# tum-vision/mem

Measured on AMD Instinct MI355X. Metric: pretrain samples/sec (ViT-B, 224^2 event voxels), higher is better.
Workload: dtype bf16; 1 GPU; MEM pretrain ViT-Base/16, 224^2 2-bin event voxels, bf16, batch 256 per GPU (BASELINE configs[1]); step = rasterize 256x30k events + event_norm + masks + ViT fwd/CE/bwd + clip + AdamW; global_batch=256, parallelism=dp1, stochastic_depth=work skipping, optimizer=AdamW as one launch in front of the next forward, last_block_mlp_rows=rows that reach the head

## Files before the change

### include/memhip.h

```cpp
#ifndef MEMHIP_H
#define MEMHIP_H

#include <stddef.h>
#include <stdint.h>

#ifdef __cplusplus
extern "C" {
#endif

#define MEMHIP_ABI_VERSION 10

#define MEMHIP_OK 0
#define MEMHIP_EINVAL (-1)
#define MEMHIP_EWORKSPACE (-2)
#define MEMHIP_ELAUNCH (-3)
#define MEMHIP_EUNSUPPORTED (-4)

typedef void* memhip_stream_t;

int memhip_abi_version(void);
const char* memhip_last_error(void);
const char* memhip_arch(void);
const char* memhip_build_flags(void);
int memhip_set_option(const char* name, int value);
int memhip_get_option(const char* name, int* value);
int memhip_stream_reserve_cus(memhip_stream_t stream, int cus);


typedef struct memhip_event_aug {
  double scale_x, scale_y;
  int32_t time_flip;
  int32_t flip_x;
  int64_t flip_w;
  int32_t shift_x, shift_y;
  int32_t do_filter;
  int32_t filt_w, filt_h;
  int32_t infer;
} memhip_event_aug_t;
#define MEMHIP_AUG_INFER_FLIP_W 1
#define MEMHIP_AUG_INFER_FILT_W 2
#define MEMHIP_AUG_INFER_FILT_H 4

enum { MEMHIP_RASTER_AUTO = 0, MEMHIP_RASTER_SINGLE = 1, MEMHIP_RASTER_BINNED = 2,
       MEMHIP_RASTER_LDS = 3, MEMHIP_RASTER_GLOBAL = 4, MEMHIP_RASTER_GLOBAL_VAR = 5 };
typedef struct memhip_raster_args {
  const double* ev;
  const int64_t* offsets;
  const memhip_event_aug_t* aug;
  const int32_t* dims;
  int32_t B, H, W, time_surface;
  int32_t form;
  int32_t reserved0;
  int64_t n_events;
  uint8_t* out;
  int32_t* status;
  void* workspace;
  size_t workspace_bytes;
} memhip_raster_args_t;
int memhip_rasterize(const memhip_raster_args_t* args, memhip_stream_t stream);

enum { MEMHIP_RASTER_K_COUNT,
       MEMHIP_RASTER_K_FINALIZE,
       MEMHIP_RASTER_K_LDS,
       MEMHIP_RASTER_K_BIN_KEYS,
       MEMHIP_RASTER_K_BIN_ACCUM };
typedef struct memhip_raster_launch {
  int32_t kernel;
  int32_t grid_x, grid_y;
  int32_t block;
  int32_t lds;
} memhip_raster_launch_t;
typedef struct memhip_raster_plan {
  int32_t family;
  int32_t rows_per_band, bands;
  int32_t band_px, nb;
  int32_t bx;
  uint64_t ws_bytes;
  uint64_t off_bins, off_tstat;
  uint64_t off_keys, off_hdr, off_bad_slots;
  uint64_t clear_ws_bytes, clear_status_bytes, clear_out_bytes;
  int32_t count;
  memhip_raster_launch_t l[2];
} memhip_raster_plan_t;
int memhip_rasterize_plan(const memhip_raster_args_t* args, int device_cus, memhip_raster_plan_t* out);

int memhip_aug_resolve(const double* extent, memhip_event_aug_t* aug, int B, int stage, int fixed_h, int fixed_w,
                       int hmax, int wmax, int32_t* dims, int32_t* status, memhip_stream_t stream);

int memhip_events_extent(const double* ev, const int64_t* offsets, const memhip_event_aug_t* aug,
                         int B, double* extent, memhip_stream_t stream);

#define MEMHIP_DT_U8 0
#define MEMHIP_DT_I8 1
#define MEMHIP_DT_U16 2
#define MEMHIP_DT_I16 3
#define MEMHIP_DT_U32 4
#define MEMHIP_DT_I32 5
#define MEMHIP_DT_U64 6
#define MEMHIP_DT_I64 7
#define MEMHIP_DT_F32 8
#define MEMHIP_DT_F64 9
#define MEMHIP_DT_BOOL 10
int memhip_decode_ncaltech101(const uint8_t* raw, int64_t n_bytes, double* ev, memhip_stream_t stream);
int memhip_events_from_columns(const void* x, int x_dtype, const void* y, int y_dtype, const void* t, int t_dtype,
                               const void* p, int p_dtype, int64_t n, double* ev, memhip_stream_t stream);
size_t memhip_events_dsec_workspace(int64_t n);
int memhip_events_dsec(const void* in, int dtype, int64_t n, double y_limit, double* out, int64_t* n_out,
                       void* workspace, size_t workspace_bytes, memhip_stream_t stream);

int memhip_resample_to_f32(const uint8_t* in, const int32_t* dims, int64_t slot_bytes, int fixed_h, int fixed_w, int mode,
                           const int32_t* offs, int B, int OH, int OW, float* out, memhip_stream_t stream);
int memhip_to_uint8(const float* x, int64_t n, uint8_t* y, memhip_stream_t stream);
int memhip_rand_augment_u8(const uint8_t* in, uint8_t* out, const void* ops, int B, int H, int W, memhip_stream_t stream);
int memhip_color_jitter(const void* in, int in_is_u8, int B, int H, int W, const void* params, float* out, int out_chans,
                        memhip_stream_t stream);

#define MEMHIP_EV_RM_TS 1
#define MEMHIP_EV_HOTPIX 2
#define MEMHIP_EV_LOG 4
#define MEMHIP_EV_GAMMA 8
#define MEMHIP_EV_NORMALIZE 16
int memhip_event_norm(const void* in, int in_is_u8, int B, int H, int W, int flags,
                      float num_stds, float gamma, float* out, int out_chans,
                      memhip_stream_t stream);
int memhip_event_norm_topk(const void* in, int in_is_u8, int B, int H, int W, int flags,
                           int num_hot_pixels, float gamma, float* out, int out_chans,
                           uint64_t* hot_keys, memhip_stream_t stream);

int memhip_mt_seed(uint32_t* mt_state, const uint32_t* key, int key_len);
double memhip_mt_random(uint32_t* mt_state);
int memhip_mask_blockwise(uint32_t* mt_state, int H, int W, int num_masking_patches,
                          int min_num_patches, int max_num_patches, double log_aspect_lo,
                          double log_aspect_hi, int n_masks, uint8_t* out);
int memhip_mask_random_location(uint32_t* mt_state, int H, int W, int num_masking_patches,
                                int n_masks, uint8_t* out);

#define MEMHIP_EPI_BIAS_BF16 0
#define MEMHIP_EPI_BIAS_GELU 1
#define MEMHIP_EPI_RESIDUAL 2
#define MEMHIP_EPI_DGELU 3
#define MEMHIP_EPI_F32 4
#define MEMHIP_EPI_PATCH_EMBED 5
#define MEMHIP_EPI_BIAS_GELU_DG 6
#define MEMHIP_EPI_MUL_AUX 7
#define MEMHIP_EPI_RESIDUAL_DROP 8

typedef struct memhip_dropout {
  uint32_t key0, key1;
  uint32_t site;
  uint32_t thr;
  float scale;
  int32_t row0;
} memhip_dropout_t;
int memhip_dropout_mask(const memhip_dropout_t* d, int row0, int rows, int cols, uint8_t* out, memhip_stream_t stream);
int memhip_dropout_rows_f32(const memhip_dropout_t* d, float* x, int64_t ldx, int rows, int D, memhip_stream_t stream);

typedef struct memhip_gemm_args {
  const void* A; const void* B;
  int64_t lda, ldb;
  int32_t M, N, K, epilogue;
  void* out0; int64_t ldo0;
  void* out1; int64_t ldo1;
  const float* bias;
  const float* vec1;
  float* resid; int64_t ldr;
  const void* aux; int64_t ldaux;
  const float* rowmask;
  float keep_prob;
  float colscale; int32_t colscale_n;
  int32_t rows_per_sample;
  int32_t accumulate;
  float* colsum;
  const int32_t* sample_map;
  int32_t colsum_copies;
  int32_t reserved0;
  const memhip_dropout_t* dropout;
} memhip_gemm_args_t;
int memhip_gemm_bf16_nt(const memhip_gemm_args_t* args, memhip_stream_t stream);

#define MEMHIP_NT_128 0
#define MEMHIP_NT_G256 1
#define MEMHIP_NT_P8_256 2
#define MEMHIP_NT_P8_128 3
#define MEMHIP_NT_P8_PAIR 4
typedef struct memhip_nt_launch {
  int32_t kind;
  int32_t row0, rows;
  int32_t tail_rows;
  int32_t guard;
  int32_t copy;
  int32_t grid, tail_grid;
} memhip_nt_launch_t;
typedef struct memhip_nt_plan { int32_t count; memhip_nt_launch_t l[2]; } memhip_nt_plan_t;
int memhip_gemm_bf16_nt_plan(const memhip_gemm_args_t* args, int stream_cus, int device_cus, memhip_nt_plan_t* out);

size_t memhip_gemm_bf16_tn_workspace(int R, int N, int K);
int memhip_gemm_bf16_tn(const void* A, int64_t lda, const void* B, int64_t ldb, int R, int N, int K,
                        float* out, int64_t ldo, int accumulate, void* workspace, size_t workspace_bytes,
                        memhip_stream_t stream);
typedef struct memhip_tn_problem {
  const void* A; int64_t lda;
  const void* B; int64_t ldb;
  float* out; int64_t ldo;
  int32_t R, N, K;
  int32_t reserved0;
} memhip_tn_problem_t;
size_t memhip_gemm_bf16_tn_group_workspace(const memhip_tn_problem_t* problems, int count);
int memhip_gemm_bf16_tn_group(const memhip_tn_problem_t* problems, int count, int accumulate, void* workspace,
                              size_t workspace_bytes, memhip_stream_t stream);

#define MEMHIP_TN_128 0
#define MEMHIP_TN_P8_ATOMIC 1
#define MEMHIP_TN_P8_WS 2
#define MEMHIP_TN_P8_GROUP 3
typedef struct memhip_tn_part {
  int32_t problem;
  int32_t tiles, splits, rows_per_split;
  int32_t wg_begin, quad_begin;
  int64_t ws_offset;
} memhip_tn_part_t;
typedef struct memhip_tn_launch {
  int32_t kind;
  int32_t count;
  int32_t grid, reduce_grid;
  int32_t memset_first;
  int32_t use_atomics;
  int64_t ws_bytes;
  memhip_tn_part_t p[4];
} memhip_tn_launch_t;
typedef struct memhip_tn_plan { int32_t count; int32_t reserved0; memhip_tn_launch_t l[4]; } memhip_tn_plan_t;
int memhip_gemm_bf16_tn_plan(const memhip_tn_problem_t* problems, int count, int accumulate, const void* workspace,
                             size_t workspace_bytes, int stream_cus, memhip_tn_plan_t* out_plan);
size_t memhip_gemm_bf16_tn_plan_workspace(const memhip_tn_problem_t* problems, int count, int device_cus);
int memhip_colsum_bf16(const void* in, int64_t ld, int R, int C, float* out, memhip_stream_t stream);
int memhip_colsum_fold(float* ws, int copies, int N, float* out, memhip_stream_t stream);

int memhip_residual_rows(const float* x, int64_t ldx, const int32_t* rows, const void* y, int64_t ldy, const float* gamma,
                         const float* rowkeep, float keep_prob, int R, int D, float* out, int64_t ldo,
                         memhip_stream_t stream);
int memhip_scatter_rows_f32(const float* src, int64_t lds, const int32_t* rows, int R, int D, float* dst, int64_t ldd,
                            memhip_stream_t stream);

int memhip_layernorm_fwd(const float* x, int64_t ldx, const int32_t* row_idx, int R, int D,
                         const float* gamma, const float* beta, float eps, void* y_bf16, int64_t ldy,
                         float* mean, float* rstd, memhip_stream_t stream);
int memhip_layernorm_bwd(const void* dy_bf16, int64_t lddy, const float* x, int64_t ldx,
                         const int32_t* row_idx, int R, int D, const float* gamma, const float* mean,
                         const float* rstd, float* dres, int64_t lddres, int accumulate, float* dgamma,
                         float* dbeta, memhip_stream_t stream);

int memhip_layerscale_grad(const void* W_bf16, int64_t ldw, const float* dW, int64_t lddw, const float* bias,
                           const float* dbias, const float* gamma, int N, int K, float* dgamma,
                           memhip_stream_t stream);

typedef struct memhip_branch {
  const void* y; int64_t ldy;
  const float* gamma;
  const float* rowmask;
  float keep_prob;
  int32_t rows_per_sample;
  void* dy; int64_t lddy;
  float* dgamma; float* dbias;
  const int32_t* out_map;
  const memhip_dropout_t* dropout;
} memhip_branch_t;
typedef struct memhip_branch_bwd_args {
  const float* dx; int64_t lddx;
  int32_t M, D;
  memhip_branch_t branch;
} memhip_branch_bwd_args_t;
int memhip_branch_bwd(const memhip_branch_bwd_args_t* args, memhip_stream_t stream);
typedef struct memhip_ln_bwd_branch_args {
  const void* dy; int64_t lddy;
  const float* x; int64_t ldx;
  int32_t R, D;
  const float* gamma; const float* mean; const float* rstd;
  float* dres; int64_t lddres;
  float* dgamma; float* dbeta;
  const int32_t* in_map;
  memhip_branch_t branch;
} memhip_ln_bwd_branch_args_t;
int memhip_layernorm_bwd_branch(const memhip_ln_bwd_branch_args_t* args, memhip_stream_t stream);

int memhip_embed_bwd(const float* dx, int64_t lddx, const uint8_t* mask, int B, int L, int D,
                     void* dy_bf16, int64_t lddy, float* dcls, float* dmask_token, memhip_stream_t stream);

int memhip_cross_entropy(void* logits_bf16, int64_t ld, const int64_t* labels, int M, int V,
                         float grad_scale, float* row_loss, int32_t* row_correct, int write_grad,
                         float* out2, memhip_stream_t stream);

int memhip_attn_tokens_padded(int T);
int memhip_relpos_gather(const float* table, const int32_t* index , int T, int TP, int heads,
                         float* bias_pad, float* biasT_pad ,
                         memhip_stream_t stream);
int memhip_attn_fwd(const void* qkv, int64_t ldqkv, int B, int T, int D, int heads, const float* table,
                    int window_h, int window_w, void* out, int64_t ldo, float* lse, memhip_stream_t stream);
int memhip_attn_delta(const void* dout, const void* out, int64_t ldo, int64_t rows, int heads, float* delta,
                      memhip_stream_t stream);
typedef struct memhip_attn_bwd_args {
  const void* qkv; int64_t ldqkv;
  const void* dout; int64_t ldo;
  const void* out; int64_t ldout;
  const float* lse;
  float* delta;
  const float* table;
  int32_t window_h, window_w, B, T, D, heads;
  float scale;
  int32_t reserved0;
  void* dqkv; int64_t lddqkv;
  float* dtable; float* dq_bias; float* dv_bias;
  void* ws; int64_t ws_bytes;
} memhip_attn_bwd_args_t;
int memhip_attn_bwd(const memhip_attn_bwd_args_t* args, memhip_stream_t stream);
int64_t memhip_attn_bwd_workspace(int B, int T, int heads, int window_h, int window_w);

#define MEMHIP_ATTN_16 1
#define MEMHIP_ATTN_SMALL 2
#define MEMHIP_ATTN_WIN 3
#define MEMHIP_ATTN_WIN_DS 4
#define MEMHIP_ATTN_STREAM 5
enum { MEMHIP_ATTN_K_STATS_ZERO, MEMHIP_ATTN_K_DELTA, MEMHIP_ATTN_K_FWD, MEMHIP_ATTN_K_BWD_KV, MEMHIP_ATTN_K_BWD_Q,
       MEMHIP_ATTN_K_FWD16, MEMHIP_ATTN_K_BWD16,
       MEMHIP_ATTN_K_WIN_STATS, MEMHIP_ATTN_K_FWD_WIN, MEMHIP_ATTN_K_BWD_KV_WIN, MEMHIP_ATTN_K_BWD_Q_WIN,
       MEMHIP_ATTN_K_BWD_KVS_WIN, MEMHIP_ATTN_K_BWD_QS_WIN,
       MEMHIP_ATTN_K_FWD_STREAM, MEMHIP_ATTN_K_BWD_KV_STREAM, MEMHIP_ATTN_K_BWD_Q_STREAM };
typedef struct memhip_attn_launch {
  int32_t kernel;
  int32_t grid_x, grid_y, grid_z;
  int32_t block;
  int32_t lds;
} memhip_attn_launch_t;
typedef struct memhip_attn_plan {
  int32_t family;
  int32_t n;
  int32_t ww;
  int32_t vb, dt, fd;
  int32_t spb;
  int32_t nwg;
  int32_t groups;
  int32_t nbz, nbq, nbs;
  int32_t qgroups, qs;
  int32_t stream_spb;
  int32_t lds_over;
  int32_t count;
  memhip_attn_launch_t l[5];
} memhip_attn_plan_t;
int memhip_attn_plan_fwd(int B, int T, int D, int heads, int window_h, int window_w, int stream_cus, memhip_attn_plan_t* out);
int memhip_attn_plan_bwd(int B, int T, int D, int heads, int window_h, int window_w, int has_dtable, int has_dv_bias,
                         int has_out, const void* ws, int64_t ws_bytes, int stream_cus, memhip_attn_plan_t* out);

int memhip_f32_gemm_nt(const memhip_gemm_args_t* args, memhip_stream_t stream);
int memhip_f32_transpose(const float* in, int64_t ldin, int R, int C, float* out, int64_t ldout, memhip_stream_t stream);
int memhip_f32_layernorm_fwd(const float* x, int64_t ldx, const int32_t* row_idx, int R, int D, const float* gamma,
                             const float* beta, float eps, float* y, int64_t ldy, float* mean, float* rstd,
                             memhip_stream_t stream);
int memhip_f32_layernorm_bwd(const float* dy, int64_t lddy, const float* x, int64_t ldx, const int32_t* row_idx, int R, int D,
                             const float* gamma, const float* mean, const float* rstd, float* dres, int64_t lddres,
                             int accumulate, float* dgamma, float* dbeta, memhip_stream_t stream);
int memhip_f32_branch_bwd(const float* dx, int64_t lddx, const float* y, int64_t ldy, const float* gamma, const float* rowmask,
                          float keep_prob, int rows_per_sample, int M, int D, float* dy, int64_t lddy, float* dgamma,
                          float* dbias, memhip_stream_t stream);
int memhip_f32_embed_bwd(const float* dx, int64_t lddx, const uint8_t* mask, int B, int L, int D, float* dy, int64_t lddy,
                         float* dcls, float* dmask_token, memhip_stream_t stream);
int memhip_f32_cross_entropy(float* logits, int64_t ld, const int64_t* labels, int M, int V, float grad_scale,
                             float* row_loss, int32_t* row_correct, int write_grad, float* out2, memhip_stream_t stream);
int memhip_f32_colsum(const float* in, int64_t ld, int R, int C, float* out, memhip_stream_t stream);
int memhip_f32_im2col(const float* x, int B, int C, int H, int W, int ph, int pw, float* out, memhip_stream_t stream);
int memhip_f32_attn_fwd(const float* qkv, int64_t ldqkv, int B, int T, int D, int heads, const float* table,
                        const int32_t* index, float* out, int64_t ldo, float* lse, memhip_stream_t stream);
int memhip_f32_attn_bwd(const float* qkv, int64_t ldqkv, const float* dout, int64_t ldo, int B, int T, int D, int heads,
                        float scale, const float* table, const int32_t* index, float* dqkv, int64_t lddqkv, float* dtable,
                        memhip_stream_t stream);

int memhip_mae_enc_assemble(const float* xe, const float* pos, const float* cls, const int64_t* ids_keep, int B, int L, int K,
                            int D, float* out, memhip_stream_t stream);
int memhip_mae_enc_assemble_bwd(const float* dx, const int64_t* ids_keep, int B, int L, int K, int D, float* dxe, float* dcls,
                                memhip_stream_t stream);
int memhip_mae_dec_assemble(const float* y, const float* mask_token, const float* dpos, const int64_t* ids_restore, int B, int L,
                            int K, int D, float* out, memhip_stream_t stream);
int memhip_mae_dec_assemble_bwd(const float* dxd, const int64_t* ids_restore, int B, int L, int K, int D, float* dy,
                                float* dmask_token, memhip_stream_t stream);
int memhip_mae_loss(const float* pred, const float* img, const float* mask, int B, int C, int H, int W, int patch,
                    int only_masked, float* row_loss, float* dpred, float* scratch2, memhip_stream_t stream);

enum { MEMHIP_CONV_BF16, MEMHIP_CONV_F32, MEMHIP_CONV_F16X2 };
typedef struct memhip_conv_args {
  int32_t mode;
  int32_t reserved0;
  const void* in;
  int64_t in_plane;
  const void* weight;
  int64_t w_plane;
  const float* bias;
  const void* add;
  int64_t add_plane;
  void* out;
  int64_t out_plane;
  int32_t B, H, W, Cin, Cout, ksize, stride, pad;
  int32_t relu;
  int32_t out_padded;
  int32_t out_f32;
  int32_t reserved1;
  const int32_t* n_active;
} memhip_conv_args_t;
int memhip_conv2d_nhwc(const memhip_conv_args_t* args, memhip_stream_t stream);
int memhip_nchw_to_padded_nhwc4(const float* x, int B, int C, int H, int W, const float* mean, const float* stdv, void* out,
                                int64_t out_plane, int mode, memhip_stream_t stream);
int memhip_argmax_rows(const void* logits, int mode, int64_t ld, int M, int N, int64_t* ids, float* top2_gap, float* row_rms,
                       const int32_t* n_samples, int rows_per_sample, memhip_stream_t stream);

int memhip_tok_flag_samples(const float* top2_gap, const float* row_rms, int B, int tokens_per_sample, float kappa,
                            int32_t* list, int32_t* count, int64_t* stats, memhip_stream_t stream);
int memhip_tok_gather_images_f32(const float* x, int C, int H, int W, const float* mean, const float* stdv,
                                 const int32_t* list, const int32_t* count, int offset, int R, float* out, int32_t* n_round,
                                 memhip_stream_t stream);
int memhip_tok_scatter_ids(const int64_t* ids_in, const int32_t* list, const int32_t* n_round, int offset, int R,
                           int tokens_per_sample, int64_t* ids_out, memhip_stream_t stream);

enum { MEMHIP_CONV_K_BF16,
       MEMHIP_CONV_K_F32,
       MEMHIP_CONV_K_F32_M32,
       MEMHIP_CONV_K_F16X2_W4,
       MEMHIP_CONV_K_F16X2_W8,
       MEMHIP_CONV_K_F16X2_WIDE,
       MEMHIP_CONV_K_F16X2_FIRST,
       MEMHIP_CONV_K_BF16_T };
typedef struct memhip_conv_launch {
  int32_t kernel;
  int32_t grid;
  int32_t block;
  int32_t lds;
  int32_t dyn_lo, dyn_hi;
} memhip_conv_launch_t;
typedef struct memhip_conv_plan {
  int32_t Hp, Wp, Ho, Wo;
  int32_t K, off;
  int64_t M;
  int32_t count;
  memhip_conv_launch_t l[2];
} memhip_conv_plan_t;
int memhip_conv_plan(const memhip_conv_args_t* args, int device_cus, memhip_conv_plan_t* out);

int memhip_convt2d_nhwc(const void* in, const void* weight, const float* bias, void* out, int B, int H, int W, int Cin, int Cout,
                        int relu, memhip_stream_t stream);
int memhip_convt_plan(int B, int H, int W, int Cin, int Cout, int device_cus, memhip_conv_plan_t* out);
int memhip_kl_uniform_rows(const void* logits, int mode, int64_t ld, int M, int N, float* row_kl, memhip_stream_t stream);

struct memhip_conv_wgrad_args {
  const void* small;
  const void* big;
  float* grad;
  void* workspace;
  size_t workspace_bytes;
  int32_t B, Hs, Ws;
  int32_t C, N;
  int32_t ksize, stride, pad;
  int32_t small_padded;
  int32_t accumulate;
};
typedef struct memhip_conv_wgrad_args memhip_conv_wgrad_args_t;
struct memhip_conv_wgrad_plan {
  int64_t M;
  int64_t ws_bytes;
  int32_t K;
  int32_t Hbp, Wbp;
  int32_t tiles_n, tiles_k;
  int32_t splits, rows_per_split;
  int32_t grid, block, lds_bytes;
  int32_t fold_grid;
  int32_t reserved;
};
typedef struct memhip_conv_wgrad_plan memhip_conv_wgrad_plan_t;
int memhip_conv_wgrad_nhwc(const memhip_conv_wgrad_args_t* args, memhip_stream_t stream);
int memhip_conv_wgrad_plan(const memhip_conv_wgrad_args_t* args, int device_cus, memhip_conv_wgrad_plan_t* out);
size_t memhip_conv_wgrad_workspace(const memhip_conv_wgrad_args_t* args, int device_cus);
int memhip_relu_bwd_colsum(void* g, const void* y, int padded, int B, int H, int W, int C, float* colsum, int accumulate,
                           void* workspace, size_t workspace_bytes, memhip_stream_t stream);
size_t memhip_relu_bwd_colsum_workspace(int B, int H, int W, int C);

int memhip_cast_f32_bf16(const float* in, void* out_bf16, int64_t n, memhip_stream_t stream);
int memhip_zero(void* p, int64_t bytes, memhip_stream_t stream);
int memhip_zero_ranges(void* base, const int64_t* ranges, int n, int64_t total_bytes, memhip_stream_t stream);
int memhip_copy_samples_f32(const float* src, float* dst, const int32_t* ids, int n, int64_t n_per_sample,
                            memhip_stream_t stream);
int memhip_transpose_cast_f32_bf16(const float* in, int64_t ldin, int R, int Cc, void* out_bf16,
                                   int64_t ldout, memhip_stream_t stream);
int memhip_transpose_cast_batched(const void* desc, const int32_t* tile_prefix, int n, int total_tiles,
                                  memhip_stream_t stream);

int memhip_transpose_bf16(const void* in, int64_t ldin, int R, int Cc, void* out, int64_t ldout, int R_pad,
                          float* colsum0, int c0_begin, int c0_end, float* colsum1, int c1_begin,
                          int c1_end, memhip_stream_t stream);
int memhip_im2col_bf16(const float* x, int B, int C, int H, int W, int ph, int pw, void* out_bf16,
                       memhip_stream_t stream);
int memhip_fill_cls(float* x, int64_t ldx, int B, int T, int D, const float* cls, memhip_stream_t stream);
int memhip_gemv_bf16_acc(const void* W, int64_t ldw, int N, int K, const float* x, float* y, float* x_acc,
                         float* zero, memhip_stream_t stream);

size_t memhip_grad_norm_workspace(void);
int memhip_grad_norm(const float* g, int64_t n, float* norm_out, void* workspace, size_t workspace_bytes,
                     memhip_stream_t stream);
int memhip_adamw(float* p, const float* g, float* m, float* v, int64_t n, const uint8_t* wd_flag_per_chunk,
                 double lr, double beta1, double beta2, double eps, double weight_decay, int step,
                 const float* gnorm, double max_norm, memhip_stream_t stream);

int memhip_adamw_groups(float* p, const float* g, float* m, float* v, int64_t n, const uint8_t* group_of_chunk,
                        const float* group_table, int n_groups, double beta1, double beta2, double eps, int step,
                        const float* gnorm, double max_norm, memhip_stream_t stream);

int memhip_mixup(float* x, int B, int C, int H, int W, const float* lam, const int32_t* box, const float* lam_host,
                 const int32_t* box_host, memhip_stream_t stream);
int memhip_mix_targets(const int64_t* labels, const float* lam, int B, int V, double smoothing, float* t, int64_t ldt,
                       memhip_stream_t stream);
int memhip_ce_soft(const void* logits, int logits_f32, int64_t ld, const float* target, int64_t ldt, const int64_t* labels,
                   float smoothing, int M, int V, float grad_scale, void* dlogits, int64_t lddl, float* row_loss,
                   int32_t* row_correct, int write_grad, float* out2, memhip_stream_t stream);
int memhip_ema_update(float* ema, const float* p, int64_t n, double decay, memhip_stream_t stream);

int memhip_pool_tokens(const float* x, int64_t ldx, int B, int T, int D, float* out, memhip_stream_t stream);
int memhip_pool_tokens_bwd(const float* dout, int B, int T, int D, float* dx, memhip_stream_t stream);

int memhip_tokens_to_maps(const float* x, int64_t ldx, int b0, int b1, int T, int D, float* out, memhip_stream_t stream);
int memhip_maps_to_tokens_add(const float* dmap, int b0, int b1, int T, int D, float* dx, int64_t lddx, memhip_stream_t stream);

int memhip_neck_maps_to_rows(const float* map, int B, int D, int Hp, int Wp, int level, void* rows_bf16, memhip_stream_t stream);
int memhip_neck_rows_to_maps(const void* rows_bf16, int B, int D, int Hp, int Wp, int level, float* map, memhip_stream_t stream);
#define MEMHIP_NECK_GROUPS 128
size_t memhip_neck_sums_workspace(int D);
int memhip_neck_colstats(const void* y_bf16, int64_t R, int D, const float* shift, float* workspace, size_t workspace_bytes,
                         float* out, memhip_stream_t stream);
int memhip_neck_bn_gelu_fwd(const void* y_bf16, int64_t R, int D, const float* mean, const float* rstd, const float* gamma,
                            const float* beta, void* z_bf16, memhip_stream_t stream);
int memhip_neck_bn_gelu_bwd_sums(const void* da_bf16, const void* y_bf16, int64_t R, int D, const float* mean, const float* rstd,
                                 const float* gamma, const float* beta, float* workspace, size_t workspace_bytes, float* out,
                                 memhip_stream_t stream);
int memhip_neck_bn_gelu_bwd_apply(const void* da_bf16, const void* y_bf16, int64_t R, int D, const float* mean, const float* rstd,
                                  const float* gamma, const float* beta, const float* sums, float inv_n, void* dy_bf16,
                                  memhip_stream_t stream);

int memhip_seg_axis_table(int in, int out, int align_corners, int32_t* i0, float* w1, int32_t* lo, int32_t* hi);

struct memhip_seg_args {
  const float* logits;
  int64_t sb, sc, sy, sx;
  const uint8_t* labels;
  int32_t B, C, h, w, H, W;
  int32_t ignore_index;
  int32_t align_corners;
  int32_t avg_non_ignore;
  float loss_weight;
  const int32_t* y_i0; const float* y_w1; const int32_t* y_lo; const int32_t* y_hi;
  const int32_t* x_i0; const float* x_w1; const int32_t* x_lo; const int32_t* x_hi;
  float* dz;
  int64_t db, dc, dy, dx;
  float* loss;
  int64_t* stats;
  void* workspace;
  size_t workspace_bytes;
  int64_t* confusion;
};
typedef struct memhip_seg_args memhip_seg_args_t;

int memhip_seg_ce(const memhip_seg_args_t* args, memhip_stream_t stream);
int memhip_seg_confusion(const memhip_seg_args_t* args, memhip_stream_t stream);

struct memhip_seg_plan {
  int32_t tile_h, tile_w;
  int32_t tiles_y, tiles_x;
  int32_t grid, block;
  int32_t chunk;
  int32_t max_fh, max_fw;
  int32_t tables_in_lds;
  int32_t lds_bytes;
  int32_t slot_bytes;
  int32_t conf_grid, conf_block, conf_lds_bytes;
  int32_t reserved;
  uint64_t ws_bytes;
};
typedef struct memhip_seg_plan memhip_seg_plan_t;
int memhip_seg_plan(const memhip_seg_args_t* args, memhip_seg_plan_t* out);

int memhip_map_to_nhwc_pad(const float* map, int B, int D, int h, int w, void* out_bf16, memhip_stream_t stream);
int memhip_nhwc_pad_to_map(const void* in_bf16, int B, int D, int h, int w, float* map, memhip_stream_t stream);
#define MEMHIP_BN_GROUPS 128
size_t memhip_bn_stats_workspace(int C);
// ... 102 lines not shown
```

### mem_amd/csrc/rowops.hip

```cpp
#include "common.h"
#include "dropout.hpp"

#include <type_traits>

namespace {

using namespace memhip;

typedef __attribute__((ext_vector_type(4))) __bf16 bf16x4;
typedef __attribute__((ext_vector_type(8))) __bf16 bf16x8;

__device__ __forceinline__ float wsum(float v) {
  for (int o = 32; o > 0; o >>= 1) v += __shfl_xor(v, o);
  return v;
}
__device__ __forceinline__ float wmax(float v) {
  for (int o = 32; o > 0; o >>= 1) v = fmaxf(v, __shfl_xor(v, o));
  return v;
}

__device__ __forceinline__ float div_newton(float a, float b, float r) {
  const float q0 = a * r;
  return fmaf(fmaf(-q0, b, a), r, q0);
}

constexpr int kMaxChunks = 8;

template <bool FULL>
__device__ __forceinline__ bool chunk_ok(int i, int nch) {
  if constexpr (FULL) return true;
  else return i < nch;
}

__device__ __forceinline__ int wave_id() { return __builtin_amdgcn_readfirstlane((int)(threadIdx.x >> 6)); }

struct RowWalk {
  int r, smp, off, stride, q, rem, rps;
  __device__ __forceinline__ RowWalk(int r0, int stride_, int rps_) : r(r0), stride(stride_), rps(rps_) {
    smp = r0 / rps; off = r0 - smp * rps;
    q = stride / rps; rem = stride - q * rps;
  }
  __device__ __forceinline__ void next() {
    r += stride; smp += q; off += rem;
    if (off >= rps) { off -= rps; ++smp; }
  }
};

__device__ __forceinline__ void stage_columns(float4* dst, const float* a, const float* b, int nch) {
  for (int i = threadIdx.x; i < nch; i += 256) {
    dst[i] = reinterpret_cast<const float4*>(a)[i];
    dst[nch + i] = b ? reinterpret_cast<const float4*>(b)[i] : float4{1.f, 1.f, 1.f, 1.f};
  }
  __syncthreads();
}

__device__ __forceinline__ int opaque(int v) {
  asm volatile("" : "+v"(v));
  return v;
}

__device__ __forceinline__ float mul_rn(float a, float b) {
#pragma clang fp contract(off)
  return a * b;
}
__device__ __forceinline__ float sub_rn(float a, float b) {
#pragma clang fp contract(off)
  return a - b;
}
__device__ __forceinline__ float ln_dx(float gg, float xh, float m1, float m2) { return __fmaf_rn(-xh, m2, sub_rn(gg, m1)); }
__device__ __forceinline__ float sq2(float a, float b) { return __fmaf_rn(a, a, mul_rn(b, b)); }

template <int NCH, bool FULL>
__global__ __launch_bounds__(256) void ln_fwd_kernel(const float* __restrict__ x, long long ldx,
                                                     const int* __restrict__ row_idx, int R, int D,
                                                     const float* __restrict__ gamma,
                                                     const float* __restrict__ beta, float eps,
                                                     __bf16* __restrict__ y, long long ldy,
                                                     float* __restrict__ mean, float* __restrict__ rstd) {
  extern __shared__ float red[];
  const int lane = threadIdx.x & 63;
  const int r0 = blockIdx.x * 4 + wave_id();
  const bool act = r0 < R;
  const int r = act ? r0 : R - 1;
  const long long src = row_idx ? row_idx[r] : r;
  const float4* xr = reinterpret_cast<const float4*>(x + src * ldx);
  const int nch = D >> 2;
  float4 v[NCH];
#pragma unroll
  for (int c = 0; c < NCH; ++c) {
    const int i = lane + c * 64;
    if (chunk_ok<FULL>(i, nch)) v[c] = xr[i];
  }
  constexpr int NST = (64 * NCH + 255) / 256;
  float4 sg[NST], sb[NST];
#pragma unroll
  for (int k = 0; k < NST; ++k) {
    const int i = min((int)threadIdx.x + k * 256, nch - 1);
    sg[k] = reinterpret_cast<const float4*>(gamma)[i];
    sb[k] = reinterpret_cast<const float4*>(beta)[i];
  }
  __builtin_amdgcn_sched_barrier(0);
  float s = 0.f;
#pragma unroll
  for (int c = 0; c < NCH; ++c)
    if (chunk_ok<FULL>(lane + c * 64, nch)) s += (v[c].x + v[c].y) + (v[c].z + v[c].w);
  const float mu = wsum(s) / (float)D;
  float4* lgb = reinterpret_cast<float4*>(red);
#pragma unroll
  for (int k = 0; k < NST; ++k) {
    const int i = min((int)threadIdx.x + k * 256, nch - 1);
    lgb[i] = sg[k];
    lgb[nch + i] = sb[k];
  }
  float q = 0.f;
#pragma unroll
  for (int c = 0; c < NCH; ++c) {
    if (chunk_ok<FULL>(lane + c * 64, nch)) {
      const float a = v[c].x - mu, b = v[c].y - mu, cc = v[c].z - mu, d = v[c].w - mu;
      q += sq2(a, b) + sq2(cc, d);
    }
  }
  const float var = wsum(q) / (float)D;
  const float rs = 1.0f / sqrtf(var + eps);
  __syncthreads();
  if (!act) return;
  if (lane == 0) { mean[r] = mu; rstd[r] = rs; }
  bf16x4* yr = reinterpret_cast<bf16x4*>(y + (long long)r * ldy);
#pragma unroll
  for (int c = 0; c < NCH; ++c) {
    const int i = lane + c * 64;
    if (chunk_ok<FULL>(i, nch)) {
      const float4 g = lgb[i], b = lgb[nch + i];
      bf16x4 o;
      o[0] = (__bf16)__fmaf_rn(mul_rn(v[c].x - mu, rs), g.x, b.x);
      o[1] = (__bf16)__fmaf_rn(mul_rn(v[c].y - mu, rs), g.y, b.y);
      o[2] = (__bf16)__fmaf_rn(mul_rn(v[c].z - mu, rs), g.z, b.z);
      o[3] = (__bf16)__fmaf_rn(mul_rn(v[c].w - mu, rs), g.w, b.w);
      yr[i] = o;
    }
  }
}

__device__ __forceinline__ void vm_drain() { __builtin_amdgcn_s_waitcnt(0x0F70); }

template <int NCH, bool FULL, bool ACC>
__global__ __launch_bounds__(256) void ln_bwd_kernel(const __bf16* __restrict__ dy, long long lddy,
                                                     const float* __restrict__ x, long long ldx,
                                                     const int* __restrict__ row_idx, int R, int D,
                                                     const float* __restrict__ gamma,
                                                     const float* __restrict__ mean,
                                                     const float* __restrict__ rstd,
                                                     float* __restrict__ dres, long long lddres,
                                                     float* __restrict__ dgamma, float* __restrict__ dbeta) {
  extern __shared__ float red[];
  const int lane = threadIdx.x & 63, wave = wave_id();
  const int nch = D >> 2;
  float4 ag[NCH], ab[NCH];
#pragma unroll
  for (int c = 0; c < NCH; ++c) {
    ag[c] = float4{0, 0, 0, 0};
    ab[c] = float4{0, 0, 0, 0};
  }
  const int rstride = gridDim.x * 4;
  float4 xn[NCH], prev[NCH];
  bf16x4 dn[NCH];
  auto issue = [&](int r, long long src, int lane) {
    const float4* xr = reinterpret_cast<const float4*>(x + src * ldx);
    const bf16x4* dyr = reinterpret_cast<const bf16x4*>(dy + (long long)r * lddy);
#pragma unroll
    for (int c = 0; c < NCH; ++c) {
      const int i = lane + c * 64;
      if (chunk_ok<FULL>(i, nch)) {
        xn[c] = xr[i];
        dn[c] = dyr[i];
      }
    }
  };
  auto issue_prev = [&](long long src, int lane) {
    const float4* o = reinterpret_cast<const float4*>(dres + src * lddres);
#pragma unroll
    for (int c = 0; c < NCH; ++c) {
      const int i = lane + c * 64;
      if (chunk_ok<FULL>(i, nch)) prev[c] = o[i];
    }
  };
  int r = blockIdx.x * 4 + wave;
  long long src = 0;
  float mu = 0.f, rs = 0.f;
  if (r < R) {
    src = row_idx ? row_idx[r] : r;
    issue(r, src, lane);
    if constexpr (ACC) issue_prev(src, lane);
    mu = mean[r]; rs = rstd[r];
  }
  float4* lg = reinterpret_cast<float4*>(red);
  for (int i = threadIdx.x; i < nch; i += 256) lg[i] = reinterpret_cast<const float4*>(gamma)[i];
  __syncthreads();
  int r1 = r + rstride;
  long long src1 = 0;
  if (r1 < R) src1 = row_idx ? row_idx[r1] : r1;
  int r2 = r1 + rstride;
  vm_drain();
  while (r < R) {
    float4 xh[NCH], gg[NCH];
    float s1 = 0.f, s2 = 0.f;
    const int ol = opaque(lane);
    const float4* lgl = lg + ol;
#pragma unroll
    for (int c = 0; c < NCH; ++c) {
      const int i = lane + c * 64;
      if (chunk_ok<FULL>(i, nch)) {
        const float4 xv = xn[c];
        const bf16x4 d4 = dn[c];
        const float4 g = lgl[c * 64];
        const float d0 = (float)d4[0], d1 = (float)d4[1], d2 = (float)d4[2], d3 = (float)d4[3];
        xh[c] = float4{mul_rn(xv.x - mu, rs), mul_rn(xv.y - mu, rs), mul_rn(xv.z - mu, rs), mul_rn(xv.w - mu, rs)};
        gg[c] = float4{mul_rn(d0, g.x), mul_rn(d1, g.y), mul_rn(d2, g.z), mul_rn(d3, g.w)};
        s1 += (gg[c].x + gg[c].y) + (gg[c].z + gg[c].w);
        s2 += (mul_rn(gg[c].x, xh[c].x) + mul_rn(gg[c].y, xh[c].y)) + (mul_rn(gg[c].z, xh[c].z) + mul_rn(gg[c].w, xh[c].w));
        ag[c].x += d0 * xh[c].x; ag[c].y += d1 * xh[c].y; ag[c].z += d2 * xh[c].z; ag[c].w += d3 * xh[c].w;
        ab[c].x += d0; ab[c].y += d1; ab[c].z += d2; ab[c].w += d3;
      }
    }
    float mu1 = 0.f, rs1 = 0.f;
    long long src2 = 0;
    const bool next = r1 < R;
    const int rl = next ? r1 : r;
    const long long srcl = next ? src1 : src;
    issue(rl, srcl, ol);
    if (next) {
      mu1 = mean[r1]; rs1 = rstd[r1];
      if (r2 < R) src2 = row_idx ? row_idx[r2] : r2;
    }
    const float m1 = wsum(s1) / (float)D, m2 = wsum(s2) / (float)D;
    float4* o = reinterpret_cast<float4*>(dres + src * lddres);
#pragma unroll
    for (int c = 0; c < NCH; ++c) {
      const int i = ol + c * 64;
      if (chunk_ok<FULL>(i, nch)) {
        const float4 t{ln_dx(gg[c].x, xh[c].x, m1, m2), ln_dx(gg[c].y, xh[c].y, m1, m2),
                       ln_dx(gg[c].z, xh[c].z, m1, m2), ln_dx(gg[c].w, xh[c].w, m1, m2)};
        float4 d;
        if constexpr (ACC) {
          const float4 p = prev[c];
          d = float4{__fmaf_rn(rs, t.x, p.x), __fmaf_rn(rs, t.y, p.y), __fmaf_rn(rs, t.z, p.z), __fmaf_rn(rs, t.w, p.w)};
        } else {
          d = float4{mul_rn(rs, t.x), mul_rn(rs, t.y), mul_rn(rs, t.z), mul_rn(rs, t.w)};
        }
        o[i] = d;
      }
    }
    if constexpr (ACC) {
      __builtin_amdgcn_sched_barrier(0);
      issue_prev(srcl, ol);
    }
    r = r1; src = src1; mu = mu1; rs = rs1;
    r1 = r2; src1 = src2;
    r2 += rstride;
  }
  __syncthreads();
  float4* rg = reinterpret_cast<float4*>(red + (size_t)wave * 2 * D);
  float4* rb = reinterpret_cast<float4*>(red + (size_t)wave * 2 * D + D);
#pragma unroll
  for (int c = 0; c < NCH; ++c) {
    const int i = lane + c * 64;
    if (chunk_ok<FULL>(i, nch)) { rg[i] = ag[c]; rb[i] = ab[c]; }
  }
  __syncthreads();
  for (int n = threadIdx.x; n < D; n += 256) {
    float a = 0.f, b = 0.f;
#pragma unroll
    for (int w = 0; w < 4; ++w) { a += red[(size_t)w * 2 * D + n]; b += red[(size_t)w * 2 * D + D + n]; }
    atomicAdd(dgamma + n, a);
    atomicAdd(dbeta + n, b);
  }
}

constexpr int kBrMaxChunks = 8;

template <int NCH, bool FULL, bool HAS_Y, class... Drop>
__global__ __launch_bounds__(256) void branch_bwd_kernel(const float* __restrict__ dx, long long lddx,
                                                         const __bf16* __restrict__ y, long long ldy,
                                                         const float* __restrict__ gamma,
                                                         const float* __restrict__ rowmask, float keep,
                                                         int rps, int M, int D, __bf16* __restrict__ dyo,
                                                         long long lddy, float* __restrict__ dgamma,
                                                         float* __restrict__ dbias, const int* __restrict__ out_map,
                                                         Drop... drop) {
  extern __shared__ float red[];
  const int lane = threadIdx.x & 63, wave = wave_id();
  const int nch = D >> 2;
  float4 ag[NCH], ab[NCH];
  const float rk = __frcp_rn(keep);
#pragma unroll
  for (int c = 0; c < NCH; ++c) {
    ag[c] = float4{0, 0, 0, 0};
    ab[c] = float4{0, 0, 0, 0};
  }
  float4 dn[NCH];
  bf16x4 yn[HAS_Y ? NCH : 1];
  auto issue = [&](int m, int lane) {
    const float4* dr = reinterpret_cast<const float4*>(dx + (long long)m * lddx);
#pragma unroll
    for (int c = 0; c < NCH; ++c) {
      const int i = lane + c * 64;
      if (chunk_ok<FULL>(i, nch)) {
        dn[c] = dr[i];
        if constexpr (HAS_Y) yn[c] = reinterpret_cast<const bf16x4*>(y + (long long)m * ldy)[i];
      }
    }
  };
  RowWalk w(blockIdx.x * 4 + wave, gridDim.x * 4, rps);
  auto find = [&](int& m, int& mo, int& smp) {
    for (;;) {
      m = w.r; smp = w.smp; mo = -1;
      if (m >= M) return;
      mo = w.r;
      if (out_map) { const int co = out_map[w.smp]; mo = co < 0 ? -1 : co * w.rps + w.off; }
      w.next();
      if (mo >= 0) return;
    }
  };
  int m, mo, smp;
  float k = 1.f;
  find(m, mo, smp);
  if (m < M) {
    issue(m, lane);
    if (rowmask) k = rowmask[smp];
  }
  float4* lg = reinterpret_cast<float4*>(red);
  for (int i = threadIdx.x; i < nch; i += 256)
    lg[i] = gamma ? reinterpret_cast<const float4*>(gamma)[i] : float4{1.f, 1.f, 1.f, 1.f};
  __syncthreads();
  int m1, mo1, smp1;
  find(m1, mo1, smp1);
  vm_drain();
  while (m < M) {
    const int ol = opaque(lane);
    float4 dv[NCH];
    bf16x4 yv[HAS_Y ? NCH : 1];
#pragma unroll
    for (int c = 0; c < NCH; ++c) {
      if (chunk_ok<FULL>(lane + c * 64, nch)) {
        dv[c] = dn[c];
        if constexpr (HAS_Y) yv[c] = yn[c];
      }
    }
    float k1 = 1.f;
    const bool next = m1 < M;
    issue(next ? m1 : m, ol);
    if (next && rowmask) k1 = rowmask[smp1];
    int m2, mo2, smp2;
    find(m2, mo2, smp2);
    bf16x4* orow = reinterpret_cast<bf16x4*>(dyo + (long long)mo * lddy);
    const float4* lgl = lg + ol;
#pragma unroll
    for (int c = 0; c < NCH; ++c) {
      const int i = ol + c * 64;
      if (chunk_ok<FULL>(i, nch)) {
        float4 d = dv[c];
        if (rowmask || out_map) {
          d.x = div_newton(d.x * k, keep, rk); d.y = div_newton(d.y * k, keep, rk);
          d.z = div_newton(d.z * k, keep, rk); d.w = div_newton(d.w * k, keep, rk);
        }
        if constexpr (sizeof...(Drop) > 0) {
          const DropParams dp = (drop, ...);
          const unsigned kb = dropout_keep8(dp, (unsigned)(dp.row0 + m), (unsigned)(i >> 1)) >> ((i & 1) * 4);
          d.x = __fmul_rn(d.x, dropout_mul(dp, kb, 0)); d.y = __fmul_rn(d.y, dropout_mul(dp, kb, 1));
          d.z = __fmul_rn(d.z, dropout_mul(dp, kb, 2)); d.w = __fmul_rn(d.w, dropout_mul(dp, kb, 3));
        }
        if constexpr (HAS_Y) {
          const bf16x4 yy = yv[c];
          ag[c].x += d.x * (float)yy[0]; ag[c].y += d.y * (float)yy[1];
          ag[c].z += d.z * (float)yy[2]; ag[c].w += d.w * (float)yy[3];
        }
        const float4 g = lgl[c * 64];
        bf16x4 o;
        o[0] = (__bf16)(d.x * g.x); o[1] = (__bf16)(d.y * g.y);
        o[2] = (__bf16)(d.z * g.z); o[3] = (__bf16)(d.w * g.w);
        orow[i] = o;
        ab[c].x += (float)o[0]; ab[c].y += (float)o[1]; ab[c].z += (float)o[2]; ab[c].w += (float)o[3];
      }
    }
    m = m1; mo = mo1; k = k1;
    m1 = m2; mo1 = mo2; smp1 = smp2;
  }
  __syncthreads();
  float4* rg = reinterpret_cast<float4*>(red + (size_t)wave * 2 * D);
  float4* rb = reinterpret_cast<float4*>(red + (size_t)wave * 2 * D + D);
#pragma unroll
  for (int c = 0; c < NCH; ++c) {
    const int i = lane + c * 64;
    if (chunk_ok<FULL>(i, nch)) { rg[i] = ag[c]; rb[i] = ab[c]; }
  }
  __syncthreads();
  for (int n = threadIdx.x; n < D; n += 256) {
    float a = 0.f, b = 0.f;
#pragma unroll
    for (int w2 = 0; w2 < 4; ++w2) { a += red[(size_t)w2 * 2 * D + n]; b += red[(size_t)w2 * 2 * D + D + n]; }
    if (dgamma) atomicAdd(dgamma + n, a);
    if (dbias) atomicAdd(dbias + n, b);
  }
}

template <int NCH, bool FULL, bool HAS_Y, class... Drop>
__global__ __launch_bounds__(256) void ln_bwd_branch_kernel(const __bf16* __restrict__ dy, long long lddy,
                                                            const float* __restrict__ x, long long ldx, int R, int D,
                                                            const float* __restrict__ gamma,
                                                            const float* __restrict__ mean, const float* __restrict__ rstd,
                                                            float* __restrict__ dres, long long lddres,
                                                            float* __restrict__ dgamma, float* __restrict__ dbeta,
                                                            const __bf16* __restrict__ yb, long long ldyb,
                                                            const float* __restrict__ gb, const float* __restrict__ rowmask,
                                                            float keep, int rps, __bf16* __restrict__ dyo, long long lddyo,
                                                            float* __restrict__ dgb, float* __restrict__ dbiasb,
                                                            const int* __restrict__ in_map, const int* __restrict__ out_map,
                                                            Drop... drop) {
  extern __shared__ float red[];
  const int lane = threadIdx.x & 63, wave = wave_id();
  const int nch = D >> 2;
  float4 ag[NCH], ab[NCH], bg[HAS_Y ? NCH : 1], bb[NCH];
  const float rk = __frcp_rn(keep);
#pragma unroll
  for (int c = 0; c < NCH; ++c) {
    ag[c] = ab[c] = bb[c] = float4{0, 0, 0, 0};
    if (HAS_Y) bg[c] = float4{0, 0, 0, 0};
  }
  float4 xn[NCH], prev[NCH];
  bf16x4 dn[NCH], yn[HAS_Y ? NCH : 1];
  auto issue_x = [&](int r, int rin, int lane) {
    const float4* xr = reinterpret_cast<const float4*>(x + (long long)r * ldx);
    const bf16x4* dyr = reinterpret_cast<const bf16x4*>(dy + (long long)rin * lddy);
#pragma unroll
    for (int c = 0; c < NCH; ++c) {
      const int i = lane + c * 64;
      if (chunk_ok<FULL>(i, nch)) {
        xn[c] = xr[i];
        dn[c] = dyr[i];
      }
    }
  };
  auto issue_y = [&](int r, int lane) {
    if constexpr (HAS_Y) {
#pragma unroll
      for (int c = 0; c < NCH; ++c) {
        const int i = lane + c * 64;
        if (chunk_ok<FULL>(i, nch)) yn[c] = reinterpret_cast<const bf16x4*>(yb + (long long)r * ldyb)[i];
      }
    }
  };
  auto issue_prev = [&](int r, int lane) {
    const float4* o = reinterpret_cast<const float4*>(dres + (long long)r * lddres);
#pragma unroll
    for (int c = 0; c < NCH; ++c) {
      const int i = lane + c * 64;
      if (chunk_ok<FULL>(i, nch)) prev[c] = o[i];
    }
  };
  const int row0 = blockIdx.x * 4 + wave, rstride = gridDim.x * 4;
  auto resolve = [&](const RowWalk& t, int& rin, int& rout) {
    rin = rout = t.r;
    if (in_map) { const int ci = in_map[t.smp]; rin = ci < 0 ? -1 : ci * t.rps + t.off; }
    if (out_map) { const int co = out_map[t.smp]; rout = co < 0 ? -1 : co * t.rps + t.off; }
  };
  int r, rin, rout;
  float mu = 0.f, rs = 0.f, km = 1.f;
  float4 xh[NCH], gg[NCH];
  bf16x4 yv[HAS_Y ? NCH : 1];
  float s1, s2;
  float4 *lg = reinterpret_cast<float4*>(red), *lgb = lg + nch;
  auto reduce_row = [&](bool has_in, int ol) {
    s1 = s2 = 0.f;
    const float4* lgl = lg + ol;
    if (has_in) {
#pragma unroll
      for (int c = 0; c < NCH; ++c) {
        if (chunk_ok<FULL>(lane + c * 64, nch)) {
          if constexpr (HAS_Y) yv[c] = yn[c];
          const float4 xv = xn[c];
          const bf16x4 d4 = dn[c];
          const float d0 = (float)d4[0], d1 = (float)d4[1], d2 = (float)d4[2], d3 = (float)d4[3];
          xh[c] = float4{mul_rn(xv.x - mu, rs), mul_rn(xv.y - mu, rs), mul_rn(xv.z - mu, rs), mul_rn(xv.w - mu, rs)};
          const float4 gmc = lgl[c * 64];
          gg[c] = float4{mul_rn(d0, gmc.x), mul_rn(d1, gmc.y), mul_rn(d2, gmc.z), mul_rn(d3, gmc.w)};
          s1 += (gg[c].x + gg[c].y) + (gg[c].z + gg[c].w);
          s2 += (mul_rn(gg[c].x, xh[c].x) + mul_rn(gg[c].y, xh[c].y)) + (mul_rn(gg[c].z, xh[c].z) + mul_rn(gg[c].w, xh[c].w));
          ag[c].x += d0 * xh[c].x; ag[c].y += d1 * xh[c].y; ag[c].z += d2 * xh[c].z; ag[c].w += d3 * xh[c].w;
          ab[c].x += d0; ab[c].y += d1; ab[c].z += d2; ab[c].w += d3;
        }
      }
    } else {
#pragma unroll
      for (int c = 0; c < NCH; ++c) {
        if (chunk_ok<FULL>(lane + c * 64, nch)) {
          if constexpr (HAS_Y) yv[c] = yn[c];
          xh[c] = gg[c] = float4{0.f, 0.f, 0.f, 0.f};
        }
      }
    }
  };
  auto store_row = [&](bool has_in, bool has_out, int ol) {
    const float m1 = wsum(s1) / (float)D, m2 = wsum(s2) / (float)D;
    float4* o = reinterpret_cast<float4*>(dres + (long long)r * lddres);
    bf16x4* orow = reinterpret_cast<bf16x4*>(dyo + (long long)(has_out ? rout : 0) * lddyo);
    const float4* lgbl = lgb + ol;
#pragma unroll
    for (int c = 0; c < NCH; ++c) {
      const int i = ol + c * 64;
      if (chunk_ok<FULL>(i, nch)) {
        float4 d{__fmaf_rn(rs, ln_dx(gg[c].x, xh[c].x, m1, m2), prev[c].x), __fmaf_rn(rs, ln_dx(gg[c].y, xh[c].y, m1, m2), prev[c].y),
                 __fmaf_rn(rs, ln_dx(gg[c].z, xh[c].z, m1, m2), prev[c].z), __fmaf_rn(rs, ln_dx(gg[c].w, xh[c].w, m1, m2), prev[c].w)};
        if (has_in) o[i] = d;
        if (!has_out) continue;
        if (rowmask || out_map) {
          d.x = div_newton(d.x * km, keep, rk); d.y = div_newton(d.y * km, keep, rk);
          d.z = div_newton(d.z * km, keep, rk); d.w = div_newton(d.w * km, keep, rk);
        }
        if constexpr (sizeof...(Drop) > 0) {
          const DropParams dp = (drop, ...);
          const unsigned kb = dropout_keep8(dp, (unsigned)(dp.row0 + r), (unsigned)(i >> 1)) >> ((i & 1) * 4);
          d.x = __fmul_rn(d.x, dropout_mul(dp, kb, 0)); d.y = __fmul_rn(d.y, dropout_mul(dp, kb, 1));
          d.z = __fmul_rn(d.z, dropout_mul(dp, kb, 2)); d.w = __fmul_rn(d.w, dropout_mul(dp, kb, 3));
        }
        if constexpr (HAS_Y) {
          bg[c].x += d.x * (float)yv[c][0]; bg[c].y += d.y * (float)yv[c][1];
          bg[c].z += d.z * (float)yv[c][2]; bg[c].w += d.w * (float)yv[c][3];
        }
        const float4 gbc = lgbl[c * 64];
        bf16x4 q;
        q[0] = (__bf16)(d.x * gbc.x); q[1] = (__bf16)(d.y * gbc.y);
        q[2] = (__bf16)(d.z * gbc.z); q[3] = (__bf16)(d.w * gbc.w);
        orow[i] = q;
        bb[c].x += (float)q[0]; bb[c].y += (float)q[1]; bb[c].z += (float)q[2]; bb[c].w += (float)q[3];
      }
    }
  };
  RowWalk w(row0, rstride, rps);
  auto find = [&](int& fr, int& frin, int& frout, int& fsmp) {
    for (;;) {
      fr = w.r; fsmp = w.smp; frin = frout = -1;
      if (fr >= R) return;
      resolve(w, frin, frout);
      w.next();
      if ((frin | frout) >= 0) return;
    }
  };
  int smp;
  find(r, rin, rout, smp);
  if (r < R) {
    issue_x(r, rin, lane); issue_y(r, lane); issue_prev(r, lane);
    mu = mean[rin]; rs = rstd[rin];
    if (rowmask) km = rowmask[smp];
  }
  stage_columns(lg, gamma, gb, nch);
  int r1, rin1, rout1, smp1;
  find(r1, rin1, rout1, smp1);
  vm_drain();
  while (r < R) {
    const int ol = opaque(lane);
    reduce_row(true, ol);
    float mu1 = 0.f, rs1 = 0.f, km1 = 1.f;
    const bool next = r1 < R;
    const int rl = next ? r1 : r, rinl = next ? rin1 : rin;
    issue_x(rl, rinl, ol); issue_y(rl, ol);
    if (next) {
      mu1 = mean[rin1]; rs1 = rstd[rin1];
      if (rowmask) km1 = rowmask[smp1];
    }
    int r2, rin2, rout2, smp2;
    find(r2, rin2, rout2, smp2);
    store_row(true, true, ol);
    __builtin_amdgcn_sched_barrier(0);
    issue_prev(rl, ol);
    r = r1; rin = rin1; rout = rout1; mu = mu1; rs = rs1; km = km1;
    r1 = r2; rin1 = rin2; rout1 = rout2; smp1 = smp2;
  }
  if (in_map || out_map) {
    for (RowWalk v(row0, rstride, rps); v.r < R; v.next()) {
      resolve(v, rin, rout);
      if ((rin >= 0) == (rout >= 0)) continue;
      r = v.r;
      const int ol = opaque(lane);
      issue_prev(r, ol); issue_y(r, ol);
      mu = rs = 0.f;
      if (rin >= 0) {
        issue_x(r, rin, ol);
        mu = mean[rin]; rs = rstd[rin];
      }
      km = rowmask ? rowmask[v.smp] : 1.f;
      reduce_row(rin >= 0, ol);
      store_row(rin >= 0, rout >= 0, ol);
    }
  }
  __syncthreads();
  float4* r0 = reinterpret_cast<float4*>(red + (size_t)wave * 4 * D);
#pragma unroll
  for (int c = 0; c < NCH; ++c) {
    const int i = lane + c * 64;
    if (chunk_ok<FULL>(i, nch)) { r0[i] = ag[c]; r0[nch + i] = ab[c]; r0[2 * nch + i] = HAS_Y ? bg[HAS_Y ? c : 0] : float4{0, 0, 0, 0}; r0[3 * nch + i] = bb[c]; }
  }
  __syncthreads();
  for (int n = threadIdx.x; n < D; n += 256) {
    float a = 0.f, b = 0.f, c2 = 0.f, d2 = 0.f;
#pragma unroll
    for (int w2 = 0; w2 < 4; ++w2) {
      const float* rw = red + (size_t)w2 * 4 * D;
      a += rw[n]; b += rw[D + n]; c2 += rw[2 * D + n]; d2 += rw[3 * D + n];
    }
    atomicAdd(dgamma + n, a);
    atomicAdd(dbeta + n, b);
    if (dgb) atomicAdd(dgb + n, c2);
    if (dbiasb) atomicAdd(dbiasb + n, d2);
  }
}


__global__ __launch_bounds__(256) void layerscale_grad_kernel(const __bf16* __restrict__ W, long long ldw,
                                                              const float* __restrict__ dW, long long lddw,
                                                              const float* __restrict__ b, const float* __restrict__ db,
                                                              const float* __restrict__ gamma, int N, int K,
                                                              float* __restrict__ dgamma) {
  __shared__ float red[4][4];
  const int lane = threadIdx.x & 63, wave = threadIdx.x >> 6;
  const int n0 = blockIdx.x * 4;
  float s[4] = {0.f, 0.f, 0.f, 0.f};
  for (int k0 = 0; k0 < K; k0 += 4096) {
#pragma unroll
    for (int c = 0; c < 4; ++c) {
      const int n = n0 + c < N ? n0 + c : N - 1;
      const __bf16* wr = W + (long long)n * ldw;
      const float* gr = dW + (long long)n * lddw;
#pragma unroll
      for (int u = 0; u < 4; ++u) {
        const int k = k0 + u * 1024 + (int)threadIdx.x * 4;
        if (k < K) {
          const bf16x4 w = *reinterpret_cast<const bf16x4*>(wr + k);
          const float4 g = *reinterpret_cast<const float4*>(gr + k);
          s[c] += (float)w[0] * g.x + (float)w[1] * g.y + (float)w[2] * g.z + (float)w[3] * g.w;
        }
      }
    }
  }
#pragma unroll
  for (int c = 0; c < 4; ++c) {
    const float t = wsum(s[c]);
    if (lane == 0) red[wave][c] = t;
  }
  __syncthreads();
  if (threadIdx.x < 4 && n0 + (int)threadIdx.x < N) {
    const int n = n0 + threadIdx.x;
    float t = (red[0][threadIdx.x] + red[1][threadIdx.x]) + (red[2][threadIdx.x] + red[3][threadIdx.x]);
    if (b && db) t += b[n] * db[n];
    const float g = gamma[n];
    dgamma[n] = g != 0.f ? t / g : 0.f;
  }
}

__global__ __launch_bounds__(256) void embed_bwd_kernel(const float* __restrict__ dx, long long lddx,
                                                        const unsigned char* __restrict__ mask, int B,
                                                        int L, int D, __bf16* __restrict__ dy,
                                                        long long lddy, float* __restrict__ dcls,
                                                        float* __restrict__ dmask) {
  constexpr int U = 7;
  for (int c = threadIdx.x * 4; c < D; c += 256 * 4) {
    float4 cls{0, 0, 0, 0}, am{0, 0, 0, 0};
    for (int b = blockIdx.x; b < B; b += gridDim.x) {
      const float* row0 = dx + (long long)b * (L + 1) * lddx + c;
      const float4 dc = *reinterpret_cast<const float4*>(row0);
      cls.x += dc.x; cls.y += dc.y; cls.z += dc.z; cls.w += dc.w;
      const unsigned char* mk = mask + (long long)b * L;
      __bf16* out = dy + (long long)b * L * lddy + c;
      int p = 0;
      for (; p + U <= L; p += U) {
        float4 d[U];
#pragma unroll
        for (int u = 0; u < U; ++u) d[u] = *reinterpret_cast<const float4*>(row0 + (long long)(1 + p + u) * lddx);
#pragma unroll
        for (int u = 0; u < U; ++u) {
          const float w = (float)mk[p + u], q = 1.0f - w;
          am.x += d[u].x * w; am.y += d[u].y * w; am.z += d[u].z * w; am.w += d[u].w * w;
          bf16x4 o;
          o[0] = (__bf16)(d[u].x * q); o[1] = (__bf16)(d[u].y * q); o[2] = (__bf16)(d[u].z * q); o[3] = (__bf16)(d[u].w * q);
          *reinterpret_cast<bf16x4*>(out + (long long)(p + u) * lddy) = o;
        }
      }
      for (; p < L; ++p) {
        const float4 d = *reinterpret_cast<const float4*>(row0 + (long long)(1 + p) * lddx);
        const float w = (float)mk[p], q = 1.0f - w;
        am.x += d.x * w; am.y += d.y * w; am.z += d.z * w; am.w += d.w * w;
        bf16x4 o;
        o[0] = (__bf16)(d.x * q); o[1] = (__bf16)(d.y * q); o[2] = (__bf16)(d.z * q); o[3] = (__bf16)(d.w * q);
        *reinterpret_cast<bf16x4*>(out + (long long)p * lddy) = o;
      }
    }
    atomicAdd(dcls + c, cls.x); atomicAdd(dcls + c + 1, cls.y);
    atomicAdd(dcls + c + 2, cls.z); atomicAdd(dcls + c + 3, cls.w);
    atomicAdd(dmask + c, am.x); atomicAdd(dmask + c + 1, am.y);
    atomicAdd(dmask + c + 2, am.z); atomicAdd(dmask + c + 3, am.w);
  }
}

template <int VPT>
__global__ __launch_bounds__(256) void ce_kernel(__bf16* __restrict__ logits, long long ld,
                                                 const long long* __restrict__ labels, int V,
                                                 float grad_scale, float* __restrict__ row_loss,
                                                 int* __restrict__ row_correct, int write_grad) {
  __shared__ float sm[4];
  __shared__ int si[4];
  __shared__ float bc[2];
  const int r = blockIdx.x, tid = threadIdx.x, lane = tid & 63, wave = tid >> 6;
  bf16x8* row = reinterpret_cast<bf16x8*>(logits + (long long)r * ld);
  const int nch = V >> 3;
  float v[VPT][8];
  float mx = -INFINITY;
  int amax = 0x7fffffff;
#pragma unroll
  for (int c = 0; c < VPT; ++c) {
    const int i = tid + c * 256;
    if (i < nch) {
      const bf16x8 t = row[i];
#pragma unroll
      for (int k = 0; k < 8; ++k) {
        v[c][k] = (float)t[k];
        if (v[c][k] > mx) { mx = v[c][k]; amax = i * 8 + k; }
      }
    }
  }
  for (int o = 32; o > 0; o >>= 1) {
    const float om = __shfl_xor(mx, o);
    const int oi = __shfl_xor(amax, o);
    if (om > mx || (om == mx && oi < amax)) { mx = om; amax = oi; }
  }
  if (lane == 0) { sm[wave] = mx; si[wave] = amax; }
  __syncthreads();
  if (tid == 0) {
    float m = sm[0]; int a = si[0];
    for (int w = 1; w < 4; ++w) if (sm[w] > m || (sm[w] == m && si[w] < a)) { m = sm[w]; a = si[w]; }
    bc[0] = m; si[0] = a;
  }
  __syncthreads();
  mx = bc[0];
  amax = si[0];
  float s = 0.f;
#pragma unroll
  for (int c = 0; c < VPT; ++c) {
    const int i = tid + c * 256;
    if (i < nch) {
#pragma unroll
      for (int k = 0; k < 8; ++k) { v[c][k] = __expf(v[c][k] - mx); s += v[c][k]; }
    }
  }
  s = wsum(s);
  __syncthreads();
  if (lane == 0) sm[wave] = s;
  __syncthreads();
  if (tid == 0) bc[1] = (sm[0] + sm[1]) + (sm[2] + sm[3]);
  __syncthreads();
  const float sum = bc[1];
  const long long lab = labels[r];
  if (tid == 0) {
    const bool lab_ok = lab >= 0 && lab < V;
    const float zl = lab_ok ? (float)logits[(long long)r * ld + lab] : __builtin_nanf("");
    row_loss[r] = (mx + __logf(sum)) - zl;
    row_correct[r] = (amax == (int)lab) ? 1 : 0;
  }
  if (write_grad) {
    const float inv = 1.0f / sum;
    __syncthreads();
#pragma unroll
    for (int c = 0; c < VPT; ++c) {
      const int i = tid + c * 256;
      if (i < nch) {
        bf16x8 o;
#pragma unroll
        for (int k = 0; k < 8; ++k) {
          float p = v[c][k] * inv;
          if ((long long)(i * 8 + k) == lab) p -= 1.0f;
          o[k] = (__bf16)(p * grad_scale);
        }
        row[i] = o;
      }
    }
  }
}

__global__ __launch_bounds__(256) void ce_reduce_kernel(const float* __restrict__ row_loss,
                                                        const int* __restrict__ row_correct, int M,
                                                        float* __restrict__ out) {
  __shared__ double sd[4];
  __shared__ int sc[4];
  double s = 0.0;
  int c = 0;
  for (int i = threadIdx.x; i < M; i += 256) { s += (double)row_loss[i]; c += row_correct[i]; }
  for (int o = 32; o > 0; o >>= 1) { s += __shfl_xor(s, o); c += __shfl_xor(c, o); }
  if ((threadIdx.x & 63) == 0) { sd[threadIdx.x >> 6] = s; sc[threadIdx.x >> 6] = c; }
  __syncthreads();
  if (threadIdx.x == 0) {
    const double t = (sd[0] + sd[1]) + (sd[2] + sd[3]);
    const int k = sc[0] + sc[1] + sc[2] + sc[3];
    out[0] = (float)(t / (double)M);
    out[1] = (float)k / (float)M;
  }
}

}

template <int MAXN, class F>
void dispatch_width(int D, F&& f) {
  const int nch = cdiv(D / 4, 64);
  const bool full = D % 256 == 0;
  const auto either = [&](auto N) { if (full) f(N, std::true_type{}); else f(N, std::false_type{}); };
  if (nch <= 1) either(std::integral_constant<int, 1>{});
  else if (nch <= 2) either(std::integral_constant<int, 2>{});
  else if (nch <= 3) either(std::integral_constant<int, 3>{});
  else if (MAXN == 4 || nch <= 4) either(std::integral_constant<int, 4>{});
  else if constexpr (MAXN == 8) {
    if (nch == 5 && full) f(std::integral_constant<int, 5>{}, std::true_type{});
    else if (nch == 8 && full) f(std::integral_constant<int, 8>{}, std::true_type{});
    else f(std::integral_constant<int, 8>{}, std::false_type{});
  }
}

extern "C" int memhip_layernorm_fwd(const float* x, int64_t ldx, const int32_t* row_idx, int R, int D,
                                    const float* gamma, const float* beta, float eps, void* y,
                                    int64_t ldy, float* mean, float* rstd, memhip_stream_t stream) {
  MEMHIP_REQUIRE(R >= 0 && D > 0 && D % 4 == 0 && D <= 64 * 4 * kMaxChunks, "layernorm_fwd: bad R=%d D=%d", R, D);
  if (R == 0) return MEMHIP_OK;
  MEMHIP_REQUIRE(x && gamma && beta && y && mean && rstd, "layernorm_fwd: null pointer");
  MEMHIP_REQUIRE(ldx % 4 == 0 && ldy % 4 == 0, "layernorm_fwd: ld must be a multiple of 4");
  dispatch_width<kMaxChunks>(D, [&](auto N, auto F) {
    hipLaunchKernelGGL((ln_fwd_kernel<decltype(N)::value, decltype(F)::value>), dim3(cdiv(R, 4)), dim3(256), (size_t)2 * D * sizeof(float), as_stream(stream),
                       x, (long long)ldx, row_idx, R, D, gamma, beta, eps, (__bf16*)y, (long long)ldy, mean, rstd);
  });
  return check_launch("layernorm_fwd");
}

extern "C" int memhip_layernorm_bwd(const void* dy, int64_t lddy, const float* x, int64_t ldx,
                                    const int32_t* row_idx, int R, int D, const float* gamma,
                                    const float* mean, const float* rstd, float* dres, int64_t lddres,
                                    int accumulate, float* dgamma, float* dbeta, memhip_stream_t stream) {
  MEMHIP_REQUIRE(R >= 0 && D > 0 && D % 4 == 0 && D <= 64 * 4 * kMaxChunks, "layernorm_bwd: bad R=%d D=%d", R, D);
  if (R == 0) return MEMHIP_OK;
  MEMHIP_REQUIRE(dy && x && gamma && mean && rstd && dres && dgamma && dbeta, "layernorm_bwd: null pointer");
  MEMHIP_REQUIRE(ldx % 4 == 0 && lddy % 4 == 0 && lddres % 4 == 0, "layernorm_bwd: ld must be a multiple of 4");
  int grid = cdiv(R, 4);
  const int cap = opt(OPT_LN_BWD_GRID) * 4 / 3;
  if (grid > cap) grid = cap;
  dispatch_width<kMaxChunks>(D, [&](auto N, auto F) {
    dispatch_bool(accumulate, [&](auto A) {
      hipLaunchKernelGGL((ln_bwd_kernel<decltype(N)::value, decltype(F)::value, decltype(A)::value>), dim3(grid), dim3(256), (size_t)8 * D * sizeof(float), as_stream(stream),
                         (const __bf16*)dy, (long long)lddy, x, (long long)ldx, row_idx, R, D, gamma, mean, rstd, dres,
                         (long long)lddres, dgamma, dbeta);
      return 0;
    });
  });
  return check_launch("layernorm_bwd");
}

template <int NCH, bool FULL, bool HAS_Y, class... Drop>
static void branch_bwd_launch(const memhip_branch_bwd_args_t& a, int grid, memhip_stream_t stream, Drop... drop) {
  const memhip_branch_t& b = a.branch;
  hipLaunchKernelGGL((branch_bwd_kernel<NCH, FULL, HAS_Y, Drop...>), dim3(grid), dim3(256), (size_t)8 * a.D * sizeof(float),
                     as_stream(stream), a.dx, (long long)a.lddx, (const __bf16*)b.y, (long long)b.ldy, b.gamma, b.rowmask,
                     b.keep_prob, b.rows_per_sample > 0 ? b.rows_per_sample : 1, a.M, a.D, (__bf16*)b.dy, (long long)b.lddy,
                     b.dgamma, b.dbias, (const int*)b.out_map, drop...);
}

extern "C" int memhip_branch_bwd(const memhip_branch_bwd_args_t* args, memhip_stream_t stream) {
  MEMHIP_REQUIRE(args, "branch_bwd: null args");
  const memhip_branch_t& b = args->branch;
  const int M = args->M, D = args->D;
  MEMHIP_REQUIRE(M >= 0 && D > 0 && D % 4 == 0, "branch_bwd: bad M=%d D=%d", M, D);
  MEMHIP_REQUIRE(!b.dropout || D % 8 == 0, "branch_bwd_drop: D=%d must be a multiple of 8", D);
  MEMHIP_REQUIRE(!b.out_map || (!b.rowmask && !b.y && b.rows_per_sample > 0), "branch_bwd: out_map excludes rowmask / y");
  if (M == 0) return MEMHIP_OK;
  MEMHIP_REQUIRE(args->dx && b.dy, "branch_bwd: null pointer");
  MEMHIP_REQUIRE(b.y || !b.dgamma, "branch_bwd: dgamma needs y (or use memhip_layerscale_grad)");
  MEMHIP_REQUIRE(args->lddx % 4 == 0 && b.ldy % 4 == 0 && b.lddy % 4 == 0, "branch_bwd: ld must be a multiple of 4");
  MEMHIP_REQUIRE(D <= 64 * 4 * kBrMaxChunks, "branch_bwd: D=%d too large", D);
  int grid = cdiv(M, 4);
  if (grid > 1024) grid = 1024;
  dispatch_width<kBrMaxChunks>(D, [&](auto N, auto F) {
    dispatch_bool(b.y, [&](auto Y) {
      if (b.dropout) branch_bwd_launch<decltype(N)::value, decltype(F)::value, decltype(Y)::value>(*args, grid, stream, drop_params(*b.dropout));
      else branch_bwd_launch<decltype(N)::value, decltype(F)::value, decltype(Y)::value>(*args, grid, stream);
      return 0;
    });
  });
  return check_launch("branch_bwd");
}

extern "C" int memhip_embed_bwd(const float* dx, int64_t lddx, const uint8_t* mask, int B, int L, int D,
                                void* dy, int64_t lddy, float* dcls, float* dmask_token,
                                memhip_stream_t stream) {
  MEMHIP_REQUIRE(B >= 0 && L > 0 && D > 0 && D % 4 == 0, "embed_bwd: bad shape");
  if (B == 0) return MEMHIP_OK;
  MEMHIP_REQUIRE(dx && mask && dy && dcls && dmask_token, "embed_bwd: null pointer");
  hipLaunchKernelGGL(embed_bwd_kernel, dim3(B < 128 ? B : 128), dim3(256), 0, as_stream(stream), dx, (long long)lddx, mask, B,
                     L, D, (__bf16*)dy, (long long)lddy, dcls, dmask_token);
  return check_launch("embed_bwd");
}

extern "C" int memhip_cross_entropy(void* logits, int64_t ld, const int64_t* labels, int M, int V,
                                    float grad_scale, float* row_loss, int32_t* row_correct,
                                    int write_grad, float* out2, memhip_stream_t stream) {
  MEMHIP_REQUIRE(M >= 0 && V > 0 && V % 8 == 0 && V <= 256 * 8 * 8, "cross_entropy: V=%d unsupported", V);
  if (M == 0) return MEMHIP_OK;
  MEMHIP_REQUIRE(logits && labels && row_loss && row_correct && out2, "cross_entropy: null pointer");
  MEMHIP_REQUIRE(ld % 8 == 0, "cross_entropy: ld must be a multiple of 8");
  hipStream_t s = as_stream(stream);
  const int nch = V / 8, vpt = cdiv(nch, 256);
  __bf16* lg = (__bf16*)logits;
  const long long* lab = (const long long*)labels;
#define CE_LAUNCH(N) hipLaunchKernelGGL(ce_kernel<N>, dim3(M), dim3(256), 0, s, lg, (long long)ld, lab, V, \
                                        grad_scale, row_loss, row_correct, write_grad)
  if (vpt <= 1) CE_LAUNCH(1);
  else if (vpt <= 2) CE_LAUNCH(2);
  else if (vpt <= 4) CE_LAUNCH(4);
  else CE_LAUNCH(8);
#undef CE_LAUNCH
  hipLaunchKernelGGL(ce_reduce_kernel, dim3(1), dim3(256), 0, s, row_loss, row_correct, M, out2);
  return check_launch("cross_entropy");
}

template <int NCH, bool FULL, bool HAS_Y, class... Drop>
static void ln_bwd_branch_launch(const memhip_ln_bwd_branch_args_t& a, int grid, memhip_stream_t stream, Drop... drop) {
  const memhip_branch_t& b = a.branch;
  hipLaunchKernelGGL((ln_bwd_branch_kernel<NCH, FULL, HAS_Y, Drop...>), dim3(grid), dim3(256), (size_t)16 * a.D * sizeof(float),
                     as_stream(stream), (const __bf16*)a.dy, (long long)a.lddy, a.x, (long long)a.ldx, a.R, a.D, a.gamma, a.mean,
                     a.rstd, a.dres, (long long)a.lddres, a.dgamma, a.dbeta, (const __bf16*)b.y, (long long)b.ldy, b.gamma,
                     b.rowmask, b.keep_prob, b.rows_per_sample > 0 ? b.rows_per_sample : 1, (__bf16*)b.dy, (long long)b.lddy,
                     b.dgamma, b.dbias, (const int*)a.in_map, (const int*)b.out_map, drop...);
}

extern "C" int memhip_layernorm_bwd_branch(const memhip_ln_bwd_branch_args_t* args, memhip_stream_t stream) {
  MEMHIP_REQUIRE(args, "layernorm_bwd_branch: null args");
  const memhip_ln_bwd_branch_args_t& a = *args;
  const memhip_branch_t& b = a.branch;
  const int R = a.R, D = a.D;
  MEMHIP_REQUIRE(R >= 0 && D > 0 && D % 4 == 0 && D <= 64 * 4 * 4, "layernorm_bwd_branch: D=%d unsupported (<= 1024)", D);
  MEMHIP_REQUIRE(!b.dropout || D % 8 == 0, "layernorm_bwd_branch_drop: D=%d must be a multiple of 8", D);
  MEMHIP_REQUIRE(!(a.in_map || b.out_map) || (!b.rowmask && !b.y && b.rows_per_sample > 0),
                 "layernorm_bwd_branch: sample maps exclude rowmask / y_branch");
  if (R == 0) return MEMHIP_OK;
  MEMHIP_REQUIRE(a.dy && a.x && a.gamma && a.mean && a.rstd && a.dres && a.dgamma && a.dbeta && b.dy,
                 "layernorm_bwd_branch: null pointer");
  MEMHIP_REQUIRE(b.y || !b.dgamma, "layernorm_bwd_branch: dgamma_branch needs y_branch");
  MEMHIP_REQUIRE(a.ldx % 4 == 0 && a.lddy % 4 == 0 && a.lddres % 4 == 0 && b.ldy % 4 == 0 && b.lddy % 4 == 0,
                 "layernorm_bwd_branch: ld must be a multiple of 4");
  int grid = cdiv(R, 4);
  int cap = opt(OPT_LN_BWD_GRID);
  if (D > 768 && cap > 512) cap = 512;
  if (grid > cap) grid = cap;
  dispatch_width<4>(D, [&](auto N, auto F) {
    if (b.dropout)
      dispatch_bool(b.y, [&](auto Y) {
        ln_bwd_branch_launch<decltype(N)::value, decltype(F)::value, decltype(Y)::value>(a, grid, stream, drop_params(*b.dropout));
        return 0;
      });
    else
      dispatch_bool(b.y, [&](auto Y) {
        ln_bwd_branch_launch<decltype(N)::value, decltype(F)::value, decltype(Y)::value>(a, grid, stream);
        return 0;
      });
  });
  return check_launch("layernorm_bwd_branch");
}

extern "C" int memhip_layerscale_grad(const void* W_bf16, int64_t ldw, const float* dW, int64_t lddw, const float* bias,
                                      const float* dbias, const float* gamma, int N, int K, float* dgamma,
                                      memhip_stream_t stream) {
  MEMHIP_REQUIRE(N >= 0 && K > 0 && K % 4 == 0 && ldw % 4 == 0 && lddw % 4 == 0, "layerscale_grad: bad shape");
  if (N == 0) return MEMHIP_OK;
  MEMHIP_REQUIRE(W_bf16 && dW && gamma && dgamma && (!bias == !dbias), "layerscale_grad: null pointer");
  hipLaunchKernelGGL(layerscale_grad_kernel, dim3((N + 3) / 4), dim3(256), 0, as_stream(stream), (const __bf16*)W_bf16,
                     (long long)ldw, dW, (long long)lddw, bias, dbias, gamma, N, K, dgamma);
  return check_launch("layerscale_grad");
}
```

### mem_amd/ops.py

```python
import ctypes as C

import torch

from ._lib import check, declare, f32, f64, i32, i64, lib, ptr, stream_ptr, sz, vp
from .vae_model import pack_convt_weight

EPI_BIAS_BF16, EPI_BIAS_GELU, EPI_RESIDUAL, EPI_DGELU, EPI_F32, EPI_PATCH_EMBED, EPI_BIAS_GELU_DG, EPI_MUL_AUX = range(8)
EPI_RESIDUAL_DROP = 8


class Dropout(C.Structure):
    _fields_ = [("key0", C.c_uint32), ("key1", C.c_uint32), ("site", C.c_uint32), ("thr", C.c_uint32), ("scale", f32),
                ("row0", i32)]


def dropout_params(key0, key1, site, p, row0=0):
    assert 0.0 <= p < 1.0, p
    return Dropout(int(key0) & 0xFFFFFFFF, int(key1) & 0xFFFFFFFF, int(site), int(round(p * 65536)), 1.0 / (1.0 - p), int(row0))


def with_row0(d, row0):
    return None if d is None else Dropout(d.key0, d.key1, d.site, d.thr, d.scale, int(row0))


class GemmArgs(C.Structure):
    _fields_ = [("A", vp), ("B", vp), ("lda", i64), ("ldb", i64),
                ("M", i32), ("N", i32), ("K", i32), ("epilogue", i32),
                ("out0", vp), ("ldo0", i64), ("out1", vp), ("ldo1", i64),
                ("bias", vp), ("vec1", vp), ("resid", vp), ("ldr", i64),
                ("aux", vp), ("ldaux", i64), ("rowmask", vp), ("keep_prob", f32),
                ("colscale", f32), ("colscale_n", i32), ("rows_per_sample", i32), ("accumulate", i32),
                ("colsum", vp), ("sample_map", vp), ("colsum_copies", i32), ("reserved0", i32),
                ("dropout", vp)]


class Branch(C.Structure):
    _fields_ = [("y", vp), ("ldy", i64), ("gamma", vp), ("rowmask", vp), ("keep_prob", f32), ("rows_per_sample", i32),
                ("dy", vp), ("lddy", i64), ("dgamma", vp), ("dbias", vp), ("out_map", vp), ("dropout", vp)]


class BranchBwdArgs(C.Structure):
    _fields_ = [("dx", vp), ("lddx", i64), ("M", i32), ("D", i32), ("branch", Branch)]


class LnBwdBranchArgs(C.Structure):
    _fields_ = [("dy", vp), ("lddy", i64), ("x", vp), ("ldx", i64), ("R", i32), ("D", i32), ("gamma", vp), ("mean", vp),
                ("rstd", vp), ("dres", vp), ("lddres", i64), ("dgamma", vp), ("dbeta", vp), ("in_map", vp), ("branch", Branch)]


class AttnBwdArgs(C.Structure):
    _fields_ = [("qkv", vp), ("ldqkv", i64), ("dout", vp), ("ldo", i64), ("out", vp), ("ldout", i64), ("lse", vp), ("delta", vp),
                ("table", vp), ("window_h", i32), ("window_w", i32), ("B", i32), ("T", i32), ("D", i32), ("heads", i32),
                ("scale", f32), ("reserved0", i32), ("dqkv", vp), ("lddqkv", i64), ("dtable", vp), ("dq_bias", vp),
                ("dv_bias", vp), ("ws", vp), ("ws_bytes", i64)]


class NtLaunch(C.Structure):
    _fields_ = [(n, i32) for n in ("kind", "row0", "rows", "tail_rows", "guard", "copy", "grid", "tail_grid")]


class NtPlan(C.Structure):
    _fields_ = [("count", i32), ("l", NtLaunch * 2)]


declare({"memhip_gemm_bf16_nt": (i32, [C.POINTER(GemmArgs), vp]),
         "memhip_branch_bwd": (i32, [C.POINTER(BranchBwdArgs), vp]),
         "memhip_layernorm_bwd_branch": (i32, [C.POINTER(LnBwdBranchArgs), vp]),
         "memhip_attn_bwd": (i32, [C.POINTER(AttnBwdArgs), vp]),
         "memhip_gemm_bf16_nt_plan": (i32, [C.POINTER(GemmArgs), i32, i32, C.POINTER(NtPlan)])})


def _p(t):
    return None if t is None else t.data_ptr()


GEMM_TIMER = None
GEMM_EVENT_POOL = []


def _timer_event():
    return GEMM_EVENT_POOL.pop() if GEMM_EVENT_POOL else torch.cuda.Event(enable_timing=True)


def _timed(code, flops, fn):
    if GEMM_TIMER is None:
        fn()
        return
    e0, e1 = _timer_event(), _timer_event()
    e0.record()
    fn()
    e1.record()
    GEMM_TIMER.append((e0, e1, flops, code))


def gemm_args(A, B, M, N, K, epi, out0=None, out1=None, bias=None, vec1=None, resid=None, aux=None,
              rowmask=None, keep_prob=1.0, colscale=1.0, colscale_n=0, rows_per_sample=1, accumulate=False, colsum=None,
              lda=None, ldb=None, ldo0=None, ldo1=None, ldr=None, ldaux=None, sample_map=None, colsum_copies=0, dropout=None):
    a = GemmArgs()
    a.A, a.B = _p(A), _p(B)
    a.lda = A.stride(0) if lda is None else lda
    a.ldb = B.stride(0) if ldb is None else ldb
    a.M, a.N, a.K, a.epilogue = M, N, K, epi
    a.out0 = _p(out0)
    a.ldo0 = (out0.stride(0) if out0 is not None else 0) if ldo0 is None else ldo0
    a.out1 = _p(out1)
    a.ldo1 = (out1.stride(0) if out1 is not None else 0) if ldo1 is None else ldo1
    a.bias, a.vec1, a.resid = _p(bias), _p(vec1), _p(resid)
    a.ldr = (resid.stride(0) if resid is not None else 0) if ldr is None else ldr
    a.aux = _p(aux)
    a.ldaux = (aux.stride(0) if (aux is not None and aux.dim() > 1) else 0) if ldaux is None else ldaux
    a.rowmask = _p(rowmask)
    a.keep_prob, a.colscale, a.colscale_n = keep_prob, colscale, colscale_n
    a.rows_per_sample, a.accumulate = rows_per_sample, int(accumulate)
    a.colsum = _p(colsum)
    a.sample_map = _p(sample_map)
    a.colsum_copies = colsum_copies
    a.dropout = None if dropout is None else C.addressof(dropout)
    return a


def gemm_nt(A, B, M, N, K, epi, *args, **kw):
    a = gemm_args(A, B, M, N, K, epi, *args, **kw)
    _timed(epi, 2.0 * M * N * K, lambda: check(lib.memhip_gemm_bf16_nt(C.byref(a), stream_ptr()), "gemm_bf16_nt"))


NT_128, NT_G256, NT_P8_256, NT_P8_128, NT_P8_PAIR = range(5)


def gemm_nt_plan(a, stream_cus=None, device_cus=None):
    if stream_cus is None or device_cus is None:
        cus = torch.cuda.get_device_properties(torch.cuda.current_device()).multi_processor_count
        stream_cus = cus if stream_cus is None else stream_cus
        device_cus = cus if device_cus is None else device_cus
    plan = NtPlan()
    check(lib.memhip_gemm_bf16_nt_plan(C.byref(a), stream_cus, device_cus, C.byref(plan)), "gemm_bf16_nt_plan")
    return [plan.l[i] for i in range(plan.count)]


declare({
    "memhip_layernorm_fwd": (i32, [vp, i64, vp, i32, i32, vp, vp, f32, vp, i64, vp, vp, vp]),
    "memhip_layernorm_bwd": (i32, [vp, i64, vp, i64, vp, i32, i32, vp, vp, vp, vp, i64, i32, vp, vp, vp]),
    "memhip_layerscale_grad": (i32, [vp, i64, vp, i64, vp, vp, vp, i32, i32, vp, vp]),
    "memhip_embed_bwd": (i32, [vp, i64, vp, i32, i32, i32, vp, i64, vp, vp, vp]),
    "memhip_cross_entropy": (i32, [vp, i64, vp, i32, i32, f32, vp, vp, i32, vp, vp]),
    "memhip_attn_tokens_padded": (i32, [i32]),
    "memhip_relpos_gather": (i32, [vp, vp, i32, i32, i32, vp, vp, vp]),
    "memhip_attn_fwd": (i32, [vp, i64, i32, i32, i32, i32, vp, i32, i32, vp, i64, vp, vp]),
    "memhip_attn_delta": (i32, [vp, vp, i64, i64, i32, vp, vp]),
    "memhip_attn_bwd_workspace": (i64, [i32, i32, i32, i32, i32]),
    "memhip_cast_f32_bf16": (i32, [vp, vp, i64, vp]),
    "memhip_copy_samples_f32": (i32, [vp, vp, vp, i32, i64, vp]),
    "memhip_zero": (i32, [vp, i64, vp]),
    "memhip_stream_reserve_cus": (i32, [vp, i32]),
    "memhip_zero_ranges": (i32, [vp, vp, i32, i64, vp]),
    "memhip_transpose_cast_f32_bf16": (i32, [vp, i64, i32, i32, vp, i64, vp]),
    "memhip_transpose_bf16": (i32, [vp, i64, i32, i32, vp, i64, i32, vp, i32, i32, vp, i32, i32, vp]),
    "memhip_im2col_bf16": (i32, [vp, i32, i32, i32, i32, i32, i32, vp, vp]),
    "memhip_fill_cls": (i32, [vp, i64, i32, i32, i32, vp, vp]),
    "memhip_gemv_bf16_acc": (i32, [vp, i64, i32, i32, vp, vp, vp, vp, vp]),
    "memhip_nchw_to_padded_nhwc4": (i32, [vp, i32, i32, i32, i32, vp, vp, vp, i64, i32, vp]),
    "memhip_argmax_rows": (i32, [vp, i32, i64, i32, i32, vp, vp, vp, vp, i32, vp]),
    "memhip_tok_flag_samples": (i32, [vp, vp, i32, i32, f32, vp, vp, vp, vp]),
    "memhip_tok_gather_images_f32": (i32, [vp, i32, i32, i32, vp, vp, vp, vp, i32, i32, vp, vp, vp]),
    "memhip_tok_scatter_ids": (i32, [vp, vp, vp, i32, i32, i32, vp, vp]),
    "memhip_grad_norm_workspace": (sz, []),
    "memhip_grad_norm": (i32, [vp, i64, vp, vp, sz, vp]),
    "memhip_adamw": (i32, [vp, vp, vp, vp, i64, vp, f64, f64, f64, f64, f64, i32, vp, f64, vp]),
    "memhip_transpose_cast_batched": (i32, [vp, vp, i32, i32, vp]),
    "memhip_adamw_groups": (i32, [vp, vp, vp, vp, i64, vp, vp, i32, f64, f64, f64, i32, vp, f64, vp]),
    "memhip_dropout_mask": (i32, [C.POINTER(Dropout), i32, i32, i32, vp, vp]),
    "memhip_dropout_rows_f32": (i32, [C.POINTER(Dropout), vp, i64, i32, i32, vp]),
})


def dropout_mask(d, row0, rows, cols, out):
    check(lib.memhip_dropout_mask(C.byref(d), row0, rows, cols, ptr(out), stream_ptr()), "dropout_mask")


def dropout_rows(d, x, rows, D):
    check(lib.memhip_dropout_rows_f32(C.byref(d), ptr(x), x.stride(0), rows, D, stream_ptr()), "dropout_rows_f32")


def layernorm_fwd(x, gamma, beta, y, mean, rstd, R, D, eps=1e-6, row_idx=None):
    check(lib.memhip_layernorm_fwd(ptr(x), x.stride(0), ptr(row_idx), R, D, ptr(gamma), ptr(beta), eps,
                                   ptr(y), y.stride(0), ptr(mean), ptr(rstd), stream_ptr()), "layernorm_fwd")


def layernorm_bwd(dy, x, gamma, mean, rstd, dres, dgamma, dbeta, R, D, accumulate=True, row_idx=None):
    check(lib.memhip_layernorm_bwd(ptr(dy), dy.stride(0), ptr(x), x.stride(0), ptr(row_idx), R, D, ptr(gamma),
                                   ptr(mean), ptr(rstd), ptr(dres), dres.stride(0), int(accumulate),
                                   ptr(dgamma), ptr(dbeta), stream_ptr()), "layernorm_bwd")


def _branch(y, gamma, rowmask, keep_prob, rows_per_sample, dy, dgamma, dbias, out_map, dropout):
    return Branch(_p(y), y.stride(0) if y is not None else 0, _p(gamma), _p(rowmask), keep_prob, rows_per_sample, _p(dy),
                  dy.stride(0), _p(dgamma), _p(dbias), _p(out_map), None if dropout is None else C.addressof(dropout))


def layernorm_bwd_branch(dy, x, gamma, mean, rstd, dres, dgamma, dbeta, R, D, y_b, gamma_b, dy_b, dgamma_b, dbias_b,
                         rowmask=None, keep_prob=1.0, rows_per_sample=1, in_map=None, out_map=None, dropout=None):
    a = LnBwdBranchArgs(_p(dy), dy.stride(0), _p(x), x.stride(0), R, D, _p(gamma), _p(mean), _p(rstd), _p(dres), dres.stride(0),
                        _p(dgamma), _p(dbeta), _p(in_map),
                        _branch(y_b, gamma_b, rowmask, keep_prob, rows_per_sample, dy_b, dgamma_b, dbias_b, out_map, dropout))
    check(lib.memhip_layernorm_bwd_branch(C.byref(a), stream_ptr()), "layernorm_bwd_branch")


def layerscale_grad(W16, dW, bias, dbias, gamma, N, K, dgamma):
    check(lib.memhip_layerscale_grad(ptr(W16), W16.stride(0), ptr(dW), dW.stride(0), ptr(bias), ptr(dbias), ptr(gamma),
                                     N, K, ptr(dgamma), stream_ptr()), "layerscale_grad")


def branch_bwd(dx, y, gamma, dy, dgamma, dbias, M, D, rowmask=None, keep_prob=1.0, rows_per_sample=1, out_map=None, dropout=None):
    a = BranchBwdArgs(_p(dx), dx.stride(0), M, D,
                      _branch(y, gamma, rowmask, keep_prob, rows_per_sample, dy, dgamma, dbias, out_map, dropout))
    check(lib.memhip_branch_bwd(C.byref(a), stream_ptr()), "branch_bwd")


def gemv_acc(W, N, K, x, y, x_acc=None, zero=None):
    check(lib.memhip_gemv_bf16_acc(ptr(W), W.stride(0), N, K, ptr(x), ptr(y), ptr(x_acc), ptr(zero), stream_ptr()),
          "gemv_bf16_acc")


CONV_MODES = ("bf16", "fp32", "fp16x2")
_CONV_MODE = {torch.bfloat16: 0, torch.float32: 1, torch.float16: 2}
_F16X2 = 2


class ConvArgs(C.Structure):
    _fields_ = [("mode", i32), ("reserved0", i32), ("in", vp), ("in_plane", i64), ("weight", vp), ("w_plane", i64),
                ("bias", vp), ("add", vp), ("add_plane", i64), ("out", vp), ("out_plane", i64)] + \
               [(n, i32) for n in ("B", "H", "W", "Cin", "Cout", "ksize", "stride", "pad", "relu", "out_padded", "out_f32",
                                   "reserved1")] + [("n_active", vp)]


declare({"memhip_conv2d_nhwc": (i32, [C.POINTER(ConvArgs), vp])})


def conv_args(mode, B, H, W, Cin, Cout, ksize, stride, pad, x=None, weight=None, bias=None, out=None, relu=False, add=None,
              out_padded=True, out_f32=False, n_active=None, planes=(0, 0, 0, 0)):
    return ConvArgs(mode, 0, x, planes[0], weight, planes[1], bias, add, planes[2], out, planes[3], B, H, W, Cin, Cout, ksize,
                    stride, pad, int(relu), int(out_padded), int(out_f32), 0, n_active)


def conv2d_nhwc(x_pad, weight, bias, out, B, H, W, Cin, Cout, ksize, stride, pad, relu=False, add=None, out_padded=True,
                n_active=None):
    mode = _CONV_MODE[x_pad.dtype]
    out_f32 = mode == _F16X2 and out.dtype == torch.float32
    assert weight.dtype == x_pad.dtype and (out_f32 or out.dtype == x_pad.dtype) and (add is None or add.dtype == x_pad.dtype)
    planes = (0, 0, 0, 0) if mode != _F16X2 else (x_pad.stride(0), weight.stride(0), 0 if add is None else add.stride(0),
                                             0 if out_f32 else out.stride(0))
    a = conv_args(mode, B, H, W, Cin, Cout, ksize, stride, pad, _p(x_pad), _p(weight), _p(bias), _p(out), relu, _p(add),
                  out_padded and not out_f32, out_f32, _p(n_active), planes)
    check(lib.memhip_conv2d_nhwc(C.byref(a), stream_ptr()), "conv2d_nhwc")


def nchw_to_padded_nhwc4(x, out, mean=None, std=None):
    B, Cc, H, W = x.shape
    mode = _CONV_MODE[out.dtype]
    check(lib.memhip_nchw_to_padded_nhwc4(ptr(x), B, Cc, H, W, ptr(mean), ptr(std), ptr(out), out.stride(0) if mode == _F16X2 else 0,
                                          mode, stream_ptr()), "nchw_to_padded_nhwc4")


def argmax_rows(logits, M, N, ids, gap=None, rms=None, n_samples=None, rows_per_sample=0):
    check(lib.memhip_argmax_rows(ptr(logits), _CONV_MODE[logits.dtype], logits.stride(0), M, N, ptr(ids), ptr(gap), ptr(rms),
                                 ptr(n_samples), rows_per_sample, stream_ptr()), "argmax_rows")


declare({
    "memhip_convt2d_nhwc": (i32, [vp, vp, vp, vp, i32, i32, i32, i32, i32, i32, vp]),
    "memhip_kl_uniform_rows": (i32, [vp, i32, i64, i32, i32, vp, vp]),
})


def convt2d_nhwc(x_pad, weight, bias, out, B, H, W, Cin, Cout, relu=False):
    assert x_pad.dtype == torch.bfloat16 and weight.dtype == torch.bfloat16 and out.dtype == torch.bfloat16
    assert B == 0 or (x_pad.numel() >= B * (H + 2) * (W + 2) * Cin and weight.numel() == 16 * Cin * Cout and
                      out.numel() >= B * (2 * H + 2) * (2 * W + 2) * Cout and (bias is None or bias.numel() == Cout))
    check(lib.memhip_convt2d_nhwc(_p(x_pad), _p(weight), _p(bias), _p(out), B, H, W, Cin, Cout, int(relu), stream_ptr()),
          "convt2d_nhwc")


def kl_uniform_rows(logits, M, N, out=None):
    assert logits.dim() == 2 and logits.stride(1) == 1 and logits.shape[0] >= M and logits.shape[1] >= N
    if out is None:
        out = torch.empty((M,), dtype=torch.float32, device=logits.device)
    assert out.dtype == torch.float32 and out.numel() >= M
    check(lib.memhip_kl_uniform_rows(ptr(logits), _CONV_MODE[logits.dtype], logits.stride(0), M, N, ptr(out), stream_ptr()),
          "kl_uniform_rows")
    return out[:M]


def tok_flag_samples(gap, rms, B, hw, kappa, lst, count, stats=None):
    check(lib.memhip_tok_flag_samples(ptr(gap), ptr(rms), B, hw, float(kappa), ptr(lst), ptr(count), ptr(stats), stream_ptr()),
          "tok_flag_samples")


def tok_gather_images(x, mean, std, lst, count, offset, R, out, n_round):
    _, Cc, H, W = x.shape
    check(lib.memhip_tok_gather_images_f32(ptr(x), Cc, H, W, ptr(mean), ptr(std), ptr(lst), ptr(count), offset, R, ptr(out),
                                           ptr(n_round), stream_ptr()), "tok_gather_images_f32")


def tok_scatter_ids(ids_in, lst, n_round, offset, R, hw, ids_out):
    check(lib.memhip_tok_scatter_ids(ptr(ids_in), ptr(lst), ptr(n_round), offset, R, hw, ptr(ids_out), stream_ptr()),
          "tok_scatter_ids")


def embed_bwd(dx, mask_u8, B, L, D, dy, dcls, dmask_token):
    check(lib.memhip_embed_bwd(ptr(dx), dx.stride(0), ptr(mask_u8), B, L, D, ptr(dy), dy.stride(0), ptr(dcls),
                               ptr(dmask_token), stream_ptr()), "embed_bwd")


def cross_entropy(logits, labels, M, V, grad_scale, row_loss, row_correct, out2, write_grad=True):
    check(lib.memhip_cross_entropy(ptr(logits), logits.stride(0), ptr(labels), M, V, grad_scale, ptr(row_loss),
                                   ptr(row_correct), int(write_grad), ptr(out2), stream_ptr()), "cross_entropy")


def attn_tokens_padded(T):
    return lib.memhip_attn_tokens_padded(T)


def relpos_gather(table, index_i32, T, TP, heads, bias_pad, biasT_pad=None):
    check(lib.memhip_relpos_gather(ptr(table), ptr(index_i32), T, TP, heads, ptr(bias_pad), ptr(biasT_pad),
                                   stream_ptr()), "relpos_gather")


def attn_fwd(qkv, B, T, D, heads, table, window, out, lse):
    _timed(200, 4.0 * B * T * T * D, lambda: check(
        lib.memhip_attn_fwd(ptr(qkv), qkv.stride(0), B, T, D, heads, ptr(table), window[0], window[1], ptr(out),
                            out.stride(0), ptr(lse), stream_ptr()), "attn_fwd"))


def attn_delta(dout, out, rows, heads, delta):
    check(lib.memhip_attn_delta(ptr(dout), ptr(out), out.stride(0), rows, heads, ptr(delta), stream_ptr()),
          "attn_delta")


def attn_bwd_workspace(B, T, heads, window):
    return int(lib.memhip_attn_bwd_workspace(B, T, heads, window[0], window[1]))


ATTN_16, ATTN_SMALL, ATTN_WIN, ATTN_WIN_DS, ATTN_STREAM = range(1, 6)
ATTN_KERNELS = ("attn_stats_zero_kernel", "attn_delta_kernel", "attn_fwd_kernel", "attn_bwd_kv_kernel", "attn_bwd_q_kernel",
                "attn16_fwd_kernel", "attn16_bwd_kernel", "attn_win_stats_kernel", "attn_fwd_win_kernel", "attn_bwd_kv_win_kernel",
                "attn_bwd_q_win_kernel", "attn_bwd_kvs_win_kernel", "attn_bwd_qs_win_kernel", "attn_fwd_stream_kernel",
                "attn_bwd_kv_stream_kernel", "attn_bwd_q_stream_kernel")


class AttnLaunch(C.Structure):
    _fields_ = [(n, i32) for n in ("kernel", "grid_x", "grid_y", "grid_z", "block", "lds")]


class AttnPlan(C.Structure):
    _fields_ = [(n, i32) for n in ("family", "n", "ww", "vb", "dt", "fd", "spb", "nwg", "groups", "nbz", "nbq", "nbs", "qgroups",
                                   "qs", "stream_spb", "lds_over", "count")] + [("l", AttnLaunch * 5)]

    @property
    def launches(self):
        return [(ATTN_KERNELS[l.kernel], (l.grid_x, l.grid_y, l.grid_z), l.block, l.lds) for l in self.l[:self.count]]


declare({"memhip_attn_plan_fwd": (i32, [i32, i32, i32, i32, i32, i32, i32, C.POINTER(AttnPlan)]),
         "memhip_attn_plan_bwd": (i32, [i32, i32, i32, i32, i32, i32, i32, i32, i32, vp, i64, i32, C.POINTER(AttnPlan)])})


def attn_plan(B, T, heads, window, backward=False, dtable=True, dv_bias=False, out=False, ws=None, ws_bytes=0, stream_cus=None):
    if stream_cus is None:
        stream_cus = torch.cuda.get_device_properties(torch.cuda.current_device()).multi_processor_count
    plan = AttnPlan()
    if not backward:
        check(lib.memhip_attn_plan_fwd(B, T, 64 * heads, heads, window[0], window[1], stream_cus, C.byref(plan)), "attn_plan_fwd")
        return plan
    if ws is not None and not isinstance(ws, int):
        ws, ws_bytes = ptr(ws), ws.numel() * ws.element_size()
    check(lib.memhip_attn_plan_bwd(B, T, 64 * heads, heads, window[0], window[1], int(dtable), int(dv_bias), int(out), ws, ws_bytes,
                                   stream_cus, C.byref(plan)), "attn_plan_bwd")
    return plan


def attn_bwd(qkv, dout, lse, delta, table, window, B, T, D, heads, scale, dqkv, dtable, dq_bias=None, dv_bias=None, out=None, ws=None):
    a = AttnBwdArgs(_p(qkv), qkv.stride(0), _p(dout), dout.stride(0), _p(out), out.stride(0) if out is not None else 0, _p(lse),
                    _p(delta), _p(table), window[0], window[1], B, T, D, heads, scale, 0, _p(dqkv), dqkv.stride(0), _p(dtable),
                    _p(dq_bias), _p(dv_bias), _p(ws), ws.numel() * ws.element_size() if ws is not None else 0)
    _timed(201, 10.0 * B * T * T * D, lambda: check(lib.memhip_attn_bwd(C.byref(a), stream_ptr()), "attn_bwd"))


def residual_rows(x, rows_i32, y, gamma, rowkeep, keep_prob, R, D, out):
    check(lib.memhip_residual_rows(ptr(x), x.stride(0), ptr(rows_i32), ptr(y), y.stride(0), ptr(gamma), ptr(rowkeep), keep_prob,
                                   R, D, ptr(out), out.stride(0), stream_ptr()), "residual_rows")


def scatter_rows(src, rows_i32, R, D, dst):
    check(lib.memhip_scatter_rows_f32(ptr(src), src.stride(0), ptr(rows_i32), R, D, ptr(dst), dst.stride(0), stream_ptr()),
          "scatter_rows")


def copy_samples(src, dst, ids_i32, n, n_per_sample):
    check(lib.memhip_copy_samples_f32(ptr(src), ptr(dst), ptr(ids_i32), n, n_per_sample, stream_ptr()), "copy_samples")


def stream_reserve_cus(stream, cus):
    check(lib.memhip_stream_reserve_cus(C.c_void_p(stream.cuda_stream), int(cus)), "stream_reserve_cus")


def zero_(t):
    nb = t.numel() * t.element_size()
    assert t.is_contiguous() and nb % 16 == 0
    check(lib.memhip_zero(ptr(t), nb, stream_ptr()), "zero")


def zero_ranges(base, ranges_dev, n, total_bytes):
    check(lib.memhip_zero_ranges(ptr(base), ptr(ranges_dev), n, total_bytes, stream_ptr()), "zero_ranges")


def cast_f32_bf16(src, dst, n):
    check(lib.memhip_cast_f32_bf16(ptr(src), ptr(dst), n, stream_ptr()), "cast")


def transpose_cast(src_f32, R, Cc, dst_bf16, ldout=None):
    check(lib.memhip_transpose_cast_f32_bf16(ptr(src_f32), src_f32.stride(0), R, Cc, ptr(dst_bf16),
                                             dst_bf16.stride(0) if ldout is None else ldout, stream_ptr()),
          "transpose_cast")


def transpose_cast_batched(desc_dev, prefix_dev, n, total_tiles):
    check(lib.memhip_transpose_cast_batched(ptr(desc_dev), ptr(prefix_dev), n, total_tiles, stream_ptr()),
          "transpose_cast_batched")


def transpose_bf16(src, R, Cc, dst, R_pad, colsum0=None, c0=(0, 0), colsum1=None, c1=(0, 0)):
    check(lib.memhip_transpose_bf16(ptr(src), src.stride(0), R, Cc, ptr(dst), dst.stride(0), R_pad, ptr(colsum0),
                                    c0[0], c0[1], ptr(colsum1), c1[0], c1[1], stream_ptr()), "transpose_bf16")


def im2col(x, B, Cc, H, W, ph, pw, out):
    check(lib.memhip_im2col_bf16(ptr(x), B, Cc, H, W, ph, pw, ptr(out), stream_ptr()), "im2col")


def fill_cls(x, B, T, D, cls):
    check(lib.memhip_fill_cls(ptr(x), x.stride(0), B, T, D, ptr(cls), stream_ptr()), "fill_cls")


def grad_norm(g, n, norm_out, ws):
    check(lib.memhip_grad_norm(ptr(g), n, ptr(norm_out), ptr(ws), ws.numel() * ws.element_size(), stream_ptr()),
          "grad_norm")


def adamw(p, g, m, v, n, wd_flags, lr, beta1, beta2, eps, wd, step, gnorm=None, max_norm=0.0):
    check(lib.memhip_adamw(ptr(p), ptr(g), ptr(m), ptr(v), n, ptr(wd_flags), lr, beta1, beta2, eps, wd, step,
                           ptr(gnorm), max_norm if max_norm else 0.0, stream_ptr()), "adamw")


def adamw_groups(p, g, m, v, n, group_of_chunk, group_table, n_groups, beta1, beta2, eps, step, gnorm=None, max_norm=0.0):
    check(lib.memhip_adamw_groups(ptr(p), ptr(g), ptr(m), ptr(v), n, ptr(group_of_chunk), ptr(group_table), n_groups, beta1,
                                  beta2, eps, step, ptr(gnorm), max_norm if max_norm else 0.0, stream_ptr()), "adamw_groups")


declare({
    "memhip_gemm_bf16_tn": (i32, [vp, i64, vp, i64, i32, i32, i32, vp, i64, i32, vp, sz, vp]),
    "memhip_gemm_bf16_tn_workspace": (sz, [i32, i32, i32]),
    "memhip_gemm_bf16_tn_group_workspace": (sz, [vp, i32]),
    "memhip_gemm_bf16_tn_group": (i32, [vp, i32, i32, vp, sz, vp]),
    "memhip_colsum_bf16": (i32, [vp, i64, i32, i32, vp, vp]),
    "memhip_colsum_fold": (i32, [vp, i32, i32, vp, vp]),
    "memhip_residual_rows": (i32, [vp, i64, vp, vp, i64, vp, vp, f32, i32, i32, vp, i64, vp]),
    "memhip_scatter_rows_f32": (i32, [vp, i64, vp, i32, i32, vp, i64, vp]),
})


_TN_WS_CACHE = {}


def gemm_tn_workspace(R, N, K):
    key = (R, N, K)
    v = _TN_WS_CACHE.get(key)
    if v is None:
        v = _TN_WS_CACHE[key] = int(lib.memhip_gemm_bf16_tn_workspace(R, N, K))
    return v


def _ws_arg(workspace):
    return (None, 0) if workspace is None else (ptr(workspace), workspace.numel() * workspace.element_size())


def gemm_tn(A, B, R, N, K, out, accumulate=True, workspace=None):
    ws, wsb = _ws_arg(workspace)
    _timed(100, 2.0 * R * N * K, lambda: check(
        lib.memhip_gemm_bf16_tn(ptr(A), A.stride(0), ptr(B), B.stride(0), R, N, K, ptr(out), out.stride(0),
                                int(accumulate), ws, wsb, stream_ptr()), "gemm_bf16_tn"))


class TnProblem(C.Structure):
    _fields_ = [("A", C.c_void_p), ("lda", C.c_int64), ("B", C.c_void_p), ("ldb", C.c_int64), ("out", C.c_void_p),
                ("ldo", C.c_int64), ("R", C.c_int32), ("N", C.c_int32), ("K", C.c_int32), ("reserved0", C.c_int32)]


def _tn_problems(problems):
    arr = (TnProblem * len(problems))()
    for q, (A, B, R, N, K, out) in zip(arr, problems):
        q.A, q.lda, q.B, q.ldb, q.out, q.ldo = A.data_ptr(), A.stride(0), B.data_ptr(), B.stride(0), out.data_ptr(), out.stride(0)
        q.R, q.N, q.K, q.reserved0 = R, N, K, 0
    return arr


def _tn_shapes(shapes):
    arr = (TnProblem * len(shapes))()
    for q, (R, N, K) in zip(arr, shapes):
# ... 835 lines not shown
```

### mem_amd/vit_engine.py

```python
import math
from collections import namedtuple

import torch

from . import ops

ALIGN = 1024

Branch = namedtuple("Branch", "n rows gemm_rows ridx smap cmap rowmask keep_prob")


def _pad(n, a):
    return (n + a - 1) // a * a


def flat_layout(shapes, skip, order, aliases=()):
    decays = lambda n: not (len(shapes[n]) == 1 or n.endswith(".bias") or n in skip)
    segs, buckets, flags, off = {}, [], [], 0
    for bname, entries in order:
        b0 = off
        for e in entries:
            if isinstance(e, tuple):
                (n, k), flag = e, 0
            elif e in shapes:
                n, k, flag = e, math.prod(shapes[e]), int(decays(e))
            else:
                continue
            segs[n] = (off, k)
            size = _pad(k, ALIGN)
            flags += [flag] * (size // ALIGN)
            off += size
        buckets.append((bname, b0, off))
    for alias, seg, o, k in aliases:
        segs[alias] = (segs[seg][0] + o, k)
    missing = [n for n in shapes if n not in segs]
    assert not missing, f"parameters not placed in the flat buffer: {missing}"
    return segs, buckets, off, flags, [n for n in shapes if decays(n)]


def check_export(export, depth, what="export"):
    if export is None:
        return ()
    export = tuple(int(i) for i in export)
    for k, i in enumerate(export):
        if not 0 <= i < depth:
            raise ValueError(f"{what}: block index {i} outside [0, {depth})")
        if i in export[:k]:
            raise ValueError(f"{what}: block index {i} given twice")
        if k and i < export[k - 1]:
            raise ValueError(f"{what}: block indices must ascend, {i} follows {export[k - 1]}")
    return export


class FlatParams:

    def _pack_flat(self, named, skip, order, aliases=()):
        self.segs, self.buckets, self.nflat, flags, self.decay_names = flat_layout(
            {n: tuple(p.shape) for n, p in named.items()}, skip, order, aliases)
        self.flat_p = torch.zeros(self.nflat, dtype=torch.float32, device=self.dev)
        self.flat_g = torch.zeros(self.nflat, dtype=torch.float32, device=self.dev)
        self.wd_flags = torch.tensor(flags, dtype=torch.uint8, device=self.dev)
        self.named = named
        for n, p in named.items():
            o, k = self.segs[n]
            view = self.flat_p[o:o + k].view(p.shape)
            view.copy_(p.data)
            p.data = view
        self.attach_grads()

    def attach_grads(self):
        for n, p in self.named.items():
            o, k = self.segs[n]
            g = p.grad
            if g is None or g.data_ptr() != self.flat_g.data_ptr() + 4 * o:
                p.grad = self.flat_g[o:o + k].view(p.shape)

    def P(self, name):
        o, k = self.segs[name]
        return self.flat_p[o:o + k]

    def G(self, name):
        o, k = self.segs[name]
        return self.flat_g[o:o + k]


class ViTEngine(FlatParams):
    def __init__(self, model):
        self.model = model
        p0 = next(model.parameters())
        assert p0.is_cuda, "mem_amd runs on the GPU only: move the model to cuda first (no CPU fallback)"
        self.dev = p0.device
        pe = model.patch_embed
        self.C = pe.proj.weight.shape[1]
        self.ph, self.pw = pe.patch_size
        self.H, self.W = pe.img_size
        self.L = pe.num_patches
        self.T = self.L + 1
        self.D = model.embed_dim
        self.depth = len(model.blocks)
        self.heads = model.blocks[0].attn.num_heads
        self.scale = float(model.blocks[0].attn.scale)
        self.hidden = model.blocks[0].mlp.fc1.weight.shape[0]
        self.head_kind = "mlm" if hasattr(model, "lm_head") else "cls"
        self.V = model.lm_head.weight.shape[0] if self.head_kind == "mlm" else 0
        self.Kpe = self.C * self.ph * self.pw
        assert self.D % 64 == 0 and self.hidden % 64 == 0 and self.Kpe % 64 == 0, "GEMM K dims must be multiples of 64"
        self.has_pos = model.pos_embed is not None
        self.drop_rate = float(getattr(model, "drop_rate", 0.0))
        self.window = tuple(pe.patch_shape)
        self.nrd = (2 * self.window[0] - 1) * (2 * self.window[1] - 1) + 3
        if model.rel_pos_bias is not None:
            self.rel = "shared"
        elif getattr(model.blocks[0].attn, "relative_position_bias_table", None) is not None:
            self.rel = "block"
        else:
            self.rel = "none"
        self.TP = ops.attn_tokens_padded(self.T)
        self._pack_parameters()
        self._build_static()
        if hasattr(model, "register_state_dict_pre_hook"):
            model.register_state_dict_pre_hook(lambda *_a, **_k: self.wait_optimizer())
        self.B = 0
        self.Mm_cap = 0
        self.cur = None
        self.B_stash = 0
        self.step_masks = None
        self.weights_dirty = True
        self.w16_version = 0
        self._zero_plans = {}
        self.grad_hook = None
        self.hook_on_side = True
        self.accumulate_grads = False
        self.overlap_optimizer = False
        self._opt_stream = None
        self._opt_ev = None
        self._opt_done = None
        self.wgrad_side_stream = True
        self.wgrad_group = 2
        self.fwd_two_streams = False
        self._side = None
        self._ev_pool, self._ev_i = [], 0
        self.dp_skip = True
        self.tail_rows = True
        self._dp_stage = None

    def _pack_parameters(self):
        m, D = self.model, self.D
        order, aliases = [], []
        head = ["lm_head.weight", "lm_head.bias", "head.weight", "head.bias", "fc_norm.weight", "fc_norm.bias", "norm.weight",
                "norm.bias"]
        head += [n for n, _ in m.named_parameters() if n.startswith(tuple(getattr(m, "_TAIL_PREFIXES", ()))) and n not in head]
        order.append(("head", head))
        for i in reversed(range(self.depth)):
            pre = f"blocks.{i}."
            qkvb = pre + "attn.qkvbias3"
            aliases += [(pre + "attn.q_bias", qkvb, 0, D), (pre + "attn.v_bias", qkvb, 2 * D, D)]
            names = [pre + n for n in ("mlp.fc2.weight", "mlp.fc2.bias", "gamma_2", "mlp.fc1.weight", "mlp.fc1.bias",
                                       "norm2.weight", "norm2.bias", "attn.proj.weight", "attn.proj.bias", "gamma_1",
                                       "attn.qkv.weight")]
            names += [(qkvb, 3 * D)] + [pre + n for n in ("attn.relative_position_bias_table", "norm1.weight", "norm1.bias")]
            order.append((f"block{i}", names))
        order.append(("embed", ["rel_pos_bias.relative_position_bias_table", "patch_embed.proj.weight",
                                "patch_embed.proj.bias", "mask_token", "cls_token", "pos_embed"]))
        self._pack_flat(dict(m.named_parameters()), m.no_weight_decay(), order, aliases)
        self.flat_w16 = torch.zeros(self.nflat, dtype=torch.bfloat16, device=self.dev)
        self.no_decay_names = [n for n in self.named if n not in set(self.decay_names)]

    def W16(self, name, rows, cols):
        o, k = self.segs[name]
        return self.flat_w16[o:o + k].view(rows, cols)

    def _build_static(self):
        D, Hd, V, dev = self.D, self.hidden, self.V, self.dev
        bf = torch.bfloat16
        self.wT = {}
        for i in range(self.depth):
            self.wT[i] = dict(qkv=torch.empty((D, 3 * D), dtype=bf, device=dev),
                              proj=torch.empty((D, D), dtype=bf, device=dev),
                              fc1=torch.empty((D, Hd), dtype=bf, device=dev),
                              fc2=torch.empty((Hd, D), dtype=bf, device=dev))
        self.wT_lm = torch.empty((D, V), dtype=bf, device=dev) if self.head_kind == "mlm" else None
        self.zero_table = torch.zeros((self.nrd, self.heads), dtype=torch.float32, device=dev)
        self.zero_vec = torch.zeros(D, dtype=torch.float32, device=dev)
        self.head_end = self.buckets[0][2]
        self._tdesc = None
        self.set_gelu_dg(True)
        self.fuse_ln_branch = True
        self.gn_ws = torch.zeros(1024, dtype=torch.float64, device=dev)
        self.gnorm = torch.zeros(1, dtype=torch.float32, device=dev)
        self.loss_acc = torch.zeros(2, dtype=torch.float32, device=dev)

    def _matrix_grad_names(self):
        names = [f"blocks.{i}.{n}" for i in range(self.depth) for n in ("attn.qkv.weight", "attn.proj.weight", "mlp.fc1.weight",
                                                                       "mlp.fc2.weight")]
        names.append("patch_embed.proj.weight")
        if self.head_kind == "mlm":
            names.append("lm_head.weight")
        return names

    def _zero_small_grads(self, start=0):
        key = ("zr", start)
        if key not in self._zero_plans:
            import numpy as np
            mats = sorted(self.segs[n] for n in self._matrix_grad_names())
            ranges, pos = [], start
            for o, k in mats:
                end = o + _pad(k, ALIGN)
                if end <= start:
                    continue
                if o > pos:
                    ranges.append((pos * 4, (o - pos) * 4))
                pos = max(pos, end)
            if pos < self.nflat:
                ranges.append((pos * 4, (self.nflat - pos) * 4))
            arr = np.asarray(ranges, dtype=np.int64).reshape(-1, 2)
            self._zero_plans[key] = (torch.from_numpy(arr).to(self.dev), len(ranges), int(arr[:, 1].sum()) if len(ranges) else 0)
        dev, n, total = self._zero_plans[key]
        ops.zero_ranges(self.flat_g, dev, n, total)

    def _zero_grad_of(self, name):
        o, k = self.segs[name]
        ops.zero_(self.flat_g[o:o + _pad(k, ALIGN)])

    def set_gelu_dg(self, on):
        self.epi_gelu, self.epi_dgelu = (ops.EPI_BIAS_GELU_DG, ops.EPI_MUL_AUX) if on else (ops.EPI_BIAS_GELU, ops.EPI_DGELU)

    def ensure_batch(self, B, Mm_max, keep=True):
        if B > self.B:
            self._alloc_forward(B)
        if keep and self.B_stash < self.B:
            self._alloc_stash()
        if Mm_max > self.Mm_cap or (self.head_kind == "mlm" and not hasattr(self, "hN")):
            self._alloc_head(min(self.B * self.L, _pad(Mm_max + Mm_max // 16 + 1, 256)))

    def _alloc_head(self, Mm_cap):
        dev, bf, f32 = self.dev, torch.bfloat16, torch.float32
        D, V = self.D, self.V
        e = lambda *s, dt=bf: torch.empty(s, dtype=dt, device=dev)
        if self.head_kind == "mlm":
            self.hN = e(Mm_cap, D)
            self.meanN, self.rstdN = e(Mm_cap, dt=f32), e(Mm_cap, dt=f32)
            self.logits = e(Mm_cap, V)
            self.row_loss, self.row_ok = e(Mm_cap, dt=f32), torch.empty(Mm_cap, dtype=torch.int32, device=dev)
            self.dhN = e(Mm_cap, D)
            self.x_tail, self.dxc = e(max(Mm_cap, 1), D, dt=f32), e(max(Mm_cap, 1), D, dt=f32)
            self.y_tail = torch.zeros((_pad(max(Mm_cap, 1), 256), D), dtype=bf, device=dev)
        self.Mm_cap = Mm_cap

    def _act_set(self, B):
        dev, bf, f32 = self.dev, torch.bfloat16, torch.float32
        D, Hd, M = self.D, self.hidden, B * self.T
        Ma = M + 256
        e = lambda *s, dt=bf: torch.empty(s, dtype=dt, device=dev)
        z = lambda *s, dt=bf: torch.zeros(s, dtype=dt, device=dev)
        return dict(h1=z(Ma, D), qkv=z(Ma, 3 * D), ao=z(Ma, D), h2=z(Ma, D), hpre=z(Ma, Hd),
                    a=z(Ma, Hd), lse=e(B, self.heads, self.TP, dt=f32),
                    mean1=e(M, dt=f32), rstd1=e(M, dt=f32), mean2=e(M, dt=f32), rstd2=e(M, dt=f32))

    def _alloc_forward(self, B):
        dev, f32 = self.dev, torch.float32
        D, T = self.D, self.T
        M = B * T
        self.patches = torch.empty((B * self.L, self.Kpe), dtype=torch.bfloat16, device=dev)
        self.x = [torch.zeros((M + T, D), dtype=f32, device=dev) for _ in range(3)]
        self.act = [self._act_set(B)]
        if self.head_kind != "mlm":
            self.zero_mask = torch.zeros(B * self.L, dtype=torch.uint8, device=dev)
        for name in ("dx", "dY", "dh_small", "dY2", "dbig", "dqkv", "dao", "delta_ws", "_tn_ws", "bias_scr", "cs_ws", "dYpe"):
            if hasattr(self, name):
                delattr(self, name)
        self._maps = []
        self.B, self.B_stash = B, 0

    def _map_buffers(self, n, B):
        D, L = self.D, self.L
        while len(self._maps) < n:
            self._maps.append(torch.empty(self.B * D * L, dtype=torch.float32, device=self.dev))
        return [m[: B * D * L].view(B, D, *self.window) for m in self._maps[:n]]

    def _alloc_stash(self):
        dev, bf, f32 = self.dev, torch.bfloat16, torch.float32
        D, Hd, T, B = self.D, self.hidden, self.T, self.B
        M = B * T
        Ma = M + 256
        e = lambda *s, dt=bf: torch.empty(s, dtype=dt, device=dev)
        z = lambda *s, dt=bf: torch.zeros(s, dtype=dt, device=dev)
        self.x += [torch.zeros((M + T, D), dtype=f32, device=dev) for _ in range(2 * self.depth + 1 - len(self.x))]
        self.act += [self._act_set(B) for _ in range(self.depth - len(self.act))]
        self.dx = torch.zeros((M, D), dtype=f32, device=dev)
        self.dY, self.dh_small = z(Ma, D), z(Ma, D)
        self.dY2 = z(Ma, D)
        self.dbig = z(Ma, Hd)
        self.dqkv = z(Ma, 3 * D)
        self.dao = z(Ma, D)
        self.delta_ws = e(2 * M + 4, self.heads, dt=f32)
        self._tn_ws = torch.empty(0, dtype=torch.uint8, device=dev)
        self.bias_scr = torch.zeros(2, D, dtype=f32, device=dev)
        self.cs_ws = torch.zeros(self.CS_COPIES, self.hidden, dtype=f32, device=dev)
        self.dYpe = e(B * self.L, D)
        self.B_stash = B

    def sync_weights(self):
        self.wait_optimizer()
        ops.cast_f32_bf16(self.flat_p, self.flat_w16, self.nflat)
        if self._tdesc is None:
            self._build_transpose_descs()
        ops.transpose_cast_batched(self._tdesc, self._tprefix, self._tn, self._ttiles)
        self.weights_dirty = False
        self.w16_version += 1

    def _build_transpose_descs(self):
        import numpy as np
        D, Hd = self.D, self.hidden
        items = []
        for i in range(self.depth):
            pre = f"blocks.{i}."
            items += [(self.P(pre + "attn.qkv.weight"), 3 * D, D, self.wT[i]["qkv"]),
                      (self.P(pre + "attn.proj.weight"), D, D, self.wT[i]["proj"]),
                      (self.P(pre + "mlp.fc1.weight"), Hd, D, self.wT[i]["fc1"]),
                      (self.P(pre + "mlp.fc2.weight"), D, Hd, self.wT[i]["fc2"])]
        if self.head_kind == "mlm":
            items.append((self.P("lm_head.weight"), self.V, D, self.wT_lm))
        desc = np.zeros((len(items), 6), dtype=np.int64)
        prefix = np.zeros(len(items) + 1, dtype=np.int32)
        for k, (src, R, Cc, dst) in enumerate(items):
            desc[k] = (src.data_ptr(), Cc, R, Cc, dst.data_ptr(), dst.stride(0))
            prefix[k + 1] = prefix[k] + ((R + 63) // 64) * ((Cc + 63) // 64)
        self._tdesc = torch.from_numpy(desc).to(self.dev)
        self._tprefix = torch.from_numpy(prefix).to(self.dev)
        self._tn, self._ttiles = len(items), int(prefix[-1])
        self._tbucket = {}
        locs = []
        for i in range(self.depth):
            locs.append((f"block{i}", 4 * i, 4))
        if self.head_kind == "mlm":
            locs.append(("head", 4 * self.depth, 1))
        loc_prefix = []
        for name, k0, n in locs:
            pl = (prefix[k0:k0 + n + 1] - prefix[k0]).astype(np.int32)
            self._tbucket[name] = (k0, n, len(loc_prefix), int(pl[-1]))
            loc_prefix += list(pl)
        self._tprefix_loc = torch.from_numpy(np.asarray(loc_prefix, dtype=np.int32)).to(self.dev)

    def table(self, i):
        if self.rel == "shared":
            return self.P("rel_pos_bias.relative_position_bias_table")
        if self.rel == "block":
            return self.P(f"blocks.{i}.attn.relative_position_bias_table")
        return self.zero_table

    def dtable(self, i):
        if self.rel == "shared":
            return self.G("rel_pos_bias.relative_position_bias_table")
        if self.rel == "block":
            return self.G(f"blocks.{i}.attn.relative_position_bias_table")
        return None

    CS_COPIES = 8

    def _dp_plan(self, dp_masks, B):
        import numpy as np
        if dp_masks is None or not self.dp_skip:
            return None
        probs = [float(b.drop_prob) for b in self.model.blocks for _ in range(2)]
        if max(probs) == 0.0:
            return None
        mk = dp_masks.detach().cpu().numpy() if isinstance(dp_masks, torch.Tensor) else np.asarray(dp_masks)
        mk = mk.reshape(2 * self.depth, B) != 0
        J, T = 2 * self.depth, self.T
        W = 3 * B + 256
        host = np.zeros((J, W), dtype=np.int32)
        host[:, B + 256:2 * B + 256] = -1
        kept_n = []
        for j in range(J):
            if probs[j] == 0.0:
                kept_n.append(None)
                continue
            k = np.flatnonzero(mk[j]).astype(np.int32)
            d = np.flatnonzero(~mk[j]).astype(np.int32)
            host[j, :len(k)] = k
            host[j, len(k):B + 256] = B
            host[j, B + 256 + k] = np.arange(len(k), dtype=np.int32)
            host[j, 2 * B + 256:2 * B + 256 + len(d)] = d
            kept_n.append(len(k))
        if self._dp_stage is None or self._dp_stage_w != J * W:
            from .utils import HostStager
            self._dp_stage, self._dp_stage_w = HostStager(J * W * 4, self.dev), J * W
            self._dp_ar = torch.arange(T, dtype=torch.int32, device=self.dev)
        dev = self._dp_stage.put(host).view(torch.int32).view(J, W)
        ridx = (dev[:, :B, None] * T + self._dp_ar[None, None, :]).view(J, B * T)
        return dict(n=kept_n, kidx=dev[:, :B + 256], cmap=dev[:, B + 256:2 * B + 256], drop=dev[:, 2 * B + 256:], ridx=ridx, B=B)

    def _branches(self, B, plan, dp_masks):
        T, out = self.T, []
        for j in range(2 * self.depth):
            drop_prob = self.model.blocks[j // 2].drop_prob
            if plan is not None and plan["n"][j] is not None:
                n = plan["n"][j]
                out.append(Branch(n, n * T, _pad(n * T, 256), plan["ridx"][j], plan["kidx"][j], plan["cmap"][j], None,
                                  1.0 - drop_prob))
            else:
                rowmask = dp_masks[j] if (dp_masks is not None and drop_prob > 0.0) else None
                out.append(Branch(B, B * T, B * T, None, None, None, rowmask, 1.0 - drop_prob))
        return out

    def _drop(self, site, row0=0):
        key = self.cur["drop_key"] if self.cur else None
        if key is None:
            return None
        return ops.dropout_params(key[0], key[1], site, self.drop_rate, row0)

    def _copy_dropped(self, plan, j, src, dst, B):
        nd = B - plan["n"][j]
        if nd > 0:
            ops.copy_samples(src, dst, plan["drop"][j], nd, self.T * self.D)

    def forward(self, x, mask_u8, rows_idx, labels=None, dp_masks=None, all_tokens=False, labels_event=None):
        assert x.is_cuda and x.dtype == torch.float32 and x.is_contiguous()
        B = x.shape[0]
        assert tuple(x.shape[1:]) == (self.C, self.H, self.W), \
            f"Input image size ({x.shape[2]}*{x.shape[3]}) doesn't match model ({self.H}*{self.W})."
        Mm = rows_idx.numel()
        self.ensure_batch(B, Mm)
        use_tail = (self.tail_rows and not all_tokens and self.depth >= 1 and 0 < Mm and 4 * Mm <= 3 * B * self.T)
        xl = self.forward_trunk(x, mask_u8, dp_masks, tail_rows=rows_idx if use_tail else None)
        D, Hd, T, L, V = self.D, self.hidden, self.T, self.L, self.V
        M = B * T
        self.cur.update(Mm=Mm, rows=rows_idx, labels=labels)
        self._wait_params("head")
        if self.cur.get("tail") is not None:
            ops.layernorm_fwd(self.x_tail, self.P("norm.weight"), self.P("norm.bias"), self.hN, self.meanN, self.rstdN, Mm, D)
        else:
            ops.layernorm_fwd(xl, self.P("norm.weight"), self.P("norm.bias"), self.hN, self.meanN, self.rstdN, Mm, D,
                              row_idx=rows_idx)
        ops.gemm_nt(self.hN, self.W16("lm_head.weight", V, D), Mm, V, D, ops.EPI_BIAS_BF16, out0=self.logits,
                    bias=self.P("lm_head.bias"))
        if labels is not None:
            if labels_event is not None:
                torch.cuda.current_stream().wait_event(labels_event)
            ops.cross_entropy(self.logits, labels, Mm, V, 1.0 / Mm, self.row_loss, self.row_ok, self.loss_acc,
                              write_grad=True)
        return self.logits[:Mm]

    def _split_point(self, B, num_cu=256):
        ntn = max(1, self.D // 256)
        tile_rows = -(-B * self.T // 256)
        rounds = tile_rows * ntn // num_cu
        if rounds < 1:
            return 0
        bs = (rounds * num_cu // ntn) * 256 // self.T
        return bs if 0 < bs < B and (B - bs) * self.T >= 4096 else 0

    def _branch(self, j, b0, b1):
        br = self.cur["branch"][j]
        if b0 == 0 and b1 == self.cur["B"]:
            return br
        assert br.smap is None, "stochastic-depth work skipping runs the whole batch on one stream"
        rows = (b1 - b0) * self.T
        return br._replace(n=b1 - b0, rows=rows, gemm_rows=rows, rowmask=None if br.rowmask is None else br.rowmask[b0:b1])

    def _block_fwd(self, i, b0, b1):
        D, Hd, T = self.D, self.hidden, self.T
        r0, r1 = b0 * T, b1 * T
        pre = f"blocks.{i}."
        xs = self.cur["x"]
        a = self.cur["act"][i]
        B, plan = self.cur["B"], self.cur["plan"]
        ba, bm = self._branch(2 * i, b0, b1), self._branch(2 * i + 1, b0, b1)
        xin, xmid, xout = xs[2 * i][r0:r1], xs[2 * i + 1][r0:r1], xs[2 * i + 2][r0:r1]
        g1 = self.P(pre + "gamma_1") if (pre + "gamma_1") in self.segs else None
        g2 = self.P(pre + "gamma_2") if (pre + "gamma_2") in self.segs else None
        tail = self.cur["tail"] if (i == self.depth - 1 and b0 == 0 and b1 == B) else None
        if ba.smap is not None:
            self._copy_dropped(plan, 2 * i, xin, xmid, B)
        if ba.n > 0:
            rs = slice(r0, r1) if ba.smap is None else slice(None)
            h1, qkv, ao = a["h1"][rs], a["qkv"][rs], a["ao"][rs]
            ops.layernorm_fwd(xin, self.P(pre + "norm1.weight"), self.P(pre + "norm1.bias"), h1, a["mean1"][r0:r1],
                              a["rstd1"][r0:r1], ba.rows, D, row_idx=ba.ridx)
            ops.gemm_nt(h1, self.W16(pre + "attn.qkv.weight", 3 * D, D), ba.gemm_rows, 3 * D, D, ops.EPI_BIAS_BF16,
                        out0=qkv, bias=self.P(pre + "attn.qkvbias3"), colscale=self.scale, colscale_n=D)
            ops.attn_fwd(qkv, ba.n, T, D, self.heads, self.table(i), self.window, ao, a["lse"][b0:b1])
            da = self._drop(2 * i, r0)
            ops.gemm_nt(ao, self.W16(pre + "attn.proj.weight", D, D), ba.gemm_rows, D, D,
                        ops.EPI_RESIDUAL if da is None else ops.EPI_RESIDUAL_DROP, out0=None,
                        bias=self.P(pre + "attn.proj.bias"), vec1=g1, resid=xmid, aux=xin, ldaux=D, rowmask=ba.rowmask,
                        keep_prob=ba.keep_prob, rows_per_sample=T, sample_map=ba.smap, dropout=da)
        if tail is not None:
            self._mlp_fwd_tail(i, a, xs[2 * i + 1], g2, bm.keep_prob, tail)
            return
        if bm.smap is not None:
            self._copy_dropped(plan, 2 * i + 1, xmid, xout, B)
        if bm.n > 0:
            rs = slice(r0, r1) if bm.smap is None else slice(None)
            h2, hpre, aa = a["h2"][rs], a["hpre"][rs], a["a"][rs]
            ops.layernorm_fwd(xmid, self.P(pre + "norm2.weight"), self.P(pre + "norm2.bias"), h2, a["mean2"][r0:r1],
                              a["rstd2"][r0:r1], bm.rows, D, row_idx=bm.ridx)
            ops.gemm_nt(h2, self.W16(pre + "mlp.fc1.weight", Hd, D), bm.gemm_rows, Hd, D, self.epi_gelu, out0=hpre,
                        out1=aa, bias=self.P(pre + "mlp.fc1.bias"))
            dm = self._drop(2 * i + 1, r0)
            ops.gemm_nt(aa, self.W16(pre + "mlp.fc2.weight", D, Hd), bm.gemm_rows, D, Hd,
                        ops.EPI_RESIDUAL if dm is None else ops.EPI_RESIDUAL_DROP, out0=None,
                        bias=self.P(pre + "mlp.fc2.bias"), vec1=g2, resid=xout, aux=xmid, ldaux=D, rowmask=bm.rowmask,
                        keep_prob=bm.keep_prob, rows_per_sample=T, sample_map=bm.smap, dropout=dm)

    def _mlp_fwd_tail(self, i, a, xmid, g2, keep, tail):
        D, Hd = self.D, self.hidden
        pre = f"blocks.{i}."
        rows, Mm = tail["rows"], tail["Mm"]
        Mp = _pad(Mm, 256)
        assert self._drop(0) is None, "the tail-row form of the last block is pretraining-only: no element-wise dropout"
        ops.layernorm_fwd(xmid, self.P(pre + "norm2.weight"), self.P(pre + "norm2.bias"), a["h2"], a["mean2"], a["rstd2"],
                          Mm, D, row_idx=rows)
        ops.gemm_nt(a["h2"], self.W16(pre + "mlp.fc1.weight", Hd, D), Mp, Hd, D, self.epi_gelu, out0=a["hpre"],
                    out1=a["a"], bias=self.P(pre + "mlp.fc1.bias"))
        ops.gemm_nt(a["a"], self.W16(pre + "mlp.fc2.weight", D, Hd), Mp, D, Hd, ops.EPI_BIAS_BF16, out0=self.y_tail,
                    bias=self.P(pre + "mlp.fc2.bias"))
        ops.residual_rows(xmid, rows, self.y_tail, g2, tail["rowkeep"], keep, Mm, D, self.x_tail)

    def forward_trunk(self, x, mask_u8=None, dp_masks=None, tail_rows=None, drop_key=None, keep=True, export=None,
                      streams=None):
        export = check_export(export, self.depth)
        assert (not export and streams is None) or (self.head_kind == "cls" and tail_rows is None), \
            "per-block exports serve the finetuning trunk: no mlm head, no tail-row form"
        assert drop_key is None or (self.drop_rate > 0.0 and tail_rows is None), "dropout: finetuning trunk only"
        assert keep or (self.head_kind == "cls" and tail_rows is None), \
            "forward-only mode (keep=False) serves the finetuning trunk: no mlm head, no tail-row form"
        assert x.is_cuda and x.dtype == torch.float32 and x.is_contiguous()
        B = x.shape[0]
        assert tuple(x.shape[1:]) == (self.C, self.H, self.W), \
            f"Input image size ({x.shape[2]}*{x.shape[3]}) doesn't match model ({self.H}*{self.W})."
        self.ensure_batch(B, self.Mm_cap, keep=keep)
        if self.weights_dirty:
            self.sync_weights()
        if self.fwd_two_streams:
            self.wait_optimizer()
        self._wait_params("embed")
        if mask_u8 is None:
            mask_u8 = self.zero_mask[: B * self.L]
        D, Hd, T, L = self.D, self.hidden, self.T, self.L
        M = B * T
        plan = self._dp_plan(dp_masks, B)
        if plan is not None:
            dp_masks = None
        nx = 2 * self.depth + 1
        self.cur = dict(B=B, M=M, Mm=0, mask=mask_u8, rows=None, dp=dp_masks, labels=None, plan=plan, tail=None, drop_key=drop_key,
                        keep=bool(keep), x=self.x if keep else [self.x[j % 3] for j in range(nx)],
                        act=self.act if keep else [self.act[0]] * self.depth, branch=self._branches(B, plan, dp_masks),
                        maps=dict(zip(export, self._map_buffers(len(export), B))) if export else None, streams=streams, dmaps=None)
        if tail_rows is not None and not self.fwd_two_streams:
            jm, lastb = 2 * self.depth - 1, self.model.blocks[self.depth - 1]
            keepvec = None
            if lastb.drop_prob > 0.0:
                if plan is not None and plan["n"][jm] is not None:
                    keepvec = (plan["cmap"][jm] >= 0).to(torch.float32)
                elif dp_masks is not None:
                    keepvec = dp_masks[jm]
            rowkeep = None
            if keepvec is not None:
                rowkeep = keepvec.index_select(0, torch.div(tail_rows, T, rounding_mode="floor").long()).contiguous()
            self.cur["tail"] = dict(rows=tail_rows, Mm=tail_rows.numel(), rowkeep=rowkeep)
        if self.head_kind == "cls" and not self.accumulate_grads and self.head_end:
            ops.zero_(self.flat_g[: self.head_end])
        ops.im2col(x, B, self.C, self.H, self.W, self.ph, self.pw, self.patches)
        x0 = self.x[0]
        if not keep and plan is not None:
            ops.zero_(x0[M:M + T])
        ops.fill_cls(x0, B, T, D, self.P("cls_token"))
        ops.gemm_nt(self.patches, self.W16("patch_embed.proj.weight", D, self.Kpe), B * L, D, self.Kpe,
                    ops.EPI_PATCH_EMBED, bias=self.P("patch_embed.proj.bias"),
                    vec1=self.P("mask_token") if "mask_token" in self.segs else self.zero_vec,
                    resid=x0, aux=mask_u8, rows_per_sample=L, ldaux=0)
        if self.has_pos:
            x0[:M].view(B, T, D).add_(self.P("pos_embed").view(1, T, D))
        dpos = self._drop(2 * self.depth)
        if dpos is not None:
            ops.dropout_rows(dpos, x0, M, D)
        bs = self._split_point(B) if (self.fwd_two_streams and ops.GEMM_TIMER is None and plan is None) else 0
        split = 0 < bs < B
        if split:
            if self._side is None:
                self._side = torch.cuda.Stream(device=self.dev)
            e0 = torch.cuda.Event()
            e0.record()
            self._side.wait_event(e0)
            for i in range(self.depth):
                self._block_fwd(i, 0, bs)
                self._export_block(i, 0, bs)
                with torch.cuda.stream(self._side):
                    self._block_fwd(i, bs, B)
                    self._export_block(i, bs, B)
            e1 = torch.cuda.Event()
            e1.record(self._side)
            torch.cuda.current_stream().wait_event(e1)
        else:
            for i in range(self.depth):
                self._wait_params(f"block{i}")
                self._block_fwd(i, 0, B)
                self._export_block(i, 0, B)
        return self.cur["x"][2 * self.depth][:M]

    def _export_block(self, i, b0, b1):
        c = self.cur
        if c["maps"] is None and c["streams"] is None:
            return
        xout, T = c["x"][2 * i + 2], self.T
        if c["maps"] is not None and i in c["maps"]:
            ops.tokens_to_maps(xout, c["B"], T, out=c["maps"][i], b0=b0, b1=b1)
        if c["streams"] is not None:
            c["streams"][i][b0 * T:b1 * T].copy_(xout[b0 * T:b1 * T])

    def _tn_ws_at_least(self, need):
        if need > self._tn_ws.numel():
            self._tn_ws = torch.empty(need, dtype=torch.uint8, device=self.dev)

    def _wgrad(self, dY, X, R, n_out, n_in, gname, bias_grads=()):
        self._tn_ws_at_least(ops.gemm_tn_workspace(R, n_out, n_in))
        ops.gemm_tn(dY, X, R, n_out, n_in, self.G(gname).view(n_out, n_in), accumulate=self.accumulate_grads,
                    workspace=self._tn_ws)
        for gv, c0, c1 in bias_grads:
            ops.colsum_bf16(dY[:, c0:c1], R, c1 - c0, gv)

    def _wg_mlp(self, pre, a, has_g, R, dY):
        D, Hd = self.D, self.hidden
        both = int(self.wgrad_group) >= 2
        if both:
            self._wgrad_group([(dY, a["a"], R, D, Hd, pre + "mlp.fc2.weight"), (self.dbig, a["h2"], R, Hd, D, pre + "mlp.fc1.weight")])
        else:
            self._wgrad(dY, a["a"], R, D, Hd, pre + "mlp.fc2.weight")
        self._side_read_done("dY")
        if has_g:
            ops.layerscale_grad(self.W16(pre + "mlp.fc2.weight", D, Hd), self.G(pre + "mlp.fc2.weight").view(D, Hd),
                                self.P(pre + "mlp.fc2.bias"), self.G(pre + "mlp.fc2.bias"),
                                self.P(pre + "gamma_2"), D, Hd, self.G(pre + "gamma_2"))
        if not both:
            self._wgrad(self.dbig, a["h2"], R, Hd, D, pre + "mlp.fc1.weight")
        self._side_read_done("dbig")

    def _wgrad_group(self, items):
        self._tn_ws_at_least(ops.gemm_tn_group_workspace([(R, n_out, n_in) for _, _, R, n_out, n_in, _ in items]))
        ops.gemm_tn_group([(dY, X, R, n_out, n_in, self.G(gname).view(n_out, n_in)) for dY, X, R, n_out, n_in, gname in items],
                          accumulate=self.accumulate_grads, workspace=self._tn_ws)

    def _event(self):
        if self._ev_i == len(self._ev_pool):
            self._ev_pool.append(torch.cuda.Event())
        e = self._ev_pool[self._ev_i]
        self._ev_i += 1
        return e

    def _side_begin(self):
        self._use_side = bool(self.wgrad_side_stream) and ops.GEMM_TIMER is None
        self._ev_i = 0
        self._side_reads = {}
        if self._use_side and self._side is None:
            self._side = torch.cuda.Stream(device=self.dev)
        if self._use_side and getattr(self, "_ws_for", None) != (self.B, self.Mm_cap):
            self._ws_for = (self.B, self.Mm_cap)
            D, Hd = self.D, self.hidden
            M = self.B * self.T
            self._tn_ws_at_least(max(
                ops.gemm_tn_group_workspace([(M, D, D), (M, 3 * D, D)]), ops.gemm_tn_group_workspace([(M, D, Hd), (M, Hd, D)]),
                ops.gemm_tn_workspace(M, 3 * D, D), ops.gemm_tn_workspace(M, Hd, D), ops.gemm_tn_workspace(M, D, Hd),
                ops.gemm_tn_workspace(M, D, D), ops.gemm_tn_workspace(self.Mm_cap or M, max(self.V, 1), D),
                ops.gemm_tn_workspace(self.B * self.L, D, self.Kpe)))

    def _on_side(self, fn):
        if not self._use_side:
            fn()
            return
        e = self._event()
        e.record()
        with torch.cuda.stream(self._side):
            self._side.wait_event(e)
            fn()

    def _side_read_done(self, name):
        if self._use_side:
            e = self._event()
            e.record(self._side)
            self._side_reads[name] = e

    def _before_overwrite(self, name):
        if self._use_side:
            e = self._side_reads.pop(name, None)
            if e is not None:
                torch.cuda.current_stream().wait_event(e)

    def _side_join(self):
        if not self._use_side:
            return
        e = self._event()
        e.record(self._side)
        torch.cuda.current_stream().wait_event(e)

    def _bucket_ready(self, k):
        if not self.grad_hook:
            return
        if not self._use_side:
            self.grad_hook(k)
            return
        if not self.hook_on_side:
            self._side_join()
            self.grad_hook(k)
            return
        e = self._event()
        e.record()
        with torch.cuda.stream(self._side):
            self._side.wait_event(e)
            self.grad_hook(k)

    attn_ds_workspace = True

    def _attn_ws(self, nb):
        if not self.attn_ds_workspace:
            return None
        need = ops.attn_bwd_workspace(nb, self.T, self.heads, self.window)
        if need == 0:
            return None
        ws = getattr(self, "_attn_ws_buf", None)
        if ws is None or ws.numel() < need:
            ws = self._attn_ws_buf = torch.empty(ops.attn_bwd_workspace(self.cur["B"], self.T, self.heads, self.window),
                                                 dtype=torch.uint8, device=self.dev)
        return ws

    def backward(self, dlogits=None):
        c = self.cur
        B, M, Mm = c["B"], c["M"], c["Mm"]
        D, Hd, T, L, V = self.D, self.hidden, self.T, self.L, self.V
        dp_masks = c["dp"]
        self.wait_optimizer()
        if dlogits is not None:
            self.logits[:Mm].copy_(dlogits)
        if not self.accumulate_grads:
            self._zero_small_grads()
        dx = self.dx
        ops.zero_(dx[:M])
        dl = self.logits
        self._side_begin()
        ops.gemm_nt(dl, self.wT_lm, Mm, D, V, ops.EPI_BIAS_BF16, out0=self.dhN)
        self._on_side(lambda: self._wgrad(dl, self.hN, Mm, V, D, "lm_head.weight", bias_grads=((self.G("lm_head.bias"), 0, V),)))
        if c.get("tail") is not None:
            ops.layernorm_bwd(self.dhN, self.x_tail, self.P("norm.weight"), self.meanN, self.rstdN, self.dxc,
                              self.G("norm.weight"), self.G("norm.bias"), Mm, D, accumulate=False)
            ops.scatter_rows(self.dxc, c["rows"], Mm, D, dx)
        else:
            ops.layernorm_bwd(self.dhN, self.x[2 * self.depth], self.P("norm.weight"), self.meanN, self.rstdN, dx,
                              self.G("norm.weight"), self.G("norm.bias"), Mm, D, accumulate=False, row_idx=c["rows"])
        self._backward_trunk()

    def backward_trunk(self, dxl, dmaps=None):
        c = self.cur
        if not c.get("keep", True):
            raise RuntimeError("backward_trunk after forward_trunk(keep=False): a forward-only pass keeps no activations "
                               "(the blocks shared one buffer set); run the forward with keep=True to train the trunk")
        M, D = c["M"], self.D
        if not self.accumulate_grads:
            self._zero_small_grads(self.head_end)
        if dxl is None:
            ops.zero_(self.dx[:M])
        else:
            self.dx[:M].copy_(dxl.reshape(M, D))
        if dmaps is not None:
            B, n = c["B"], c["B"] * D * self.L
            for i, g in dmaps.items():
                if not 0 <= i < self.depth:
                    raise ValueError(f"dmaps: block index {i} outside [0, {self.depth})")
                assert g.is_cuda and g.dtype == torch.float32 and g.is_contiguous() and g.numel() == n, \
                    f"dmaps[{i}]: contiguous fp32 [{B}, {D}, {self.window[0]}, {self.window[1]}]"
        c["dmaps"] = dmaps or None
        self._side_begin()
        self._backward_trunk()

    def _inject_dmap(self, i):
        dm = self.cur.get("dmaps")
        if dm is not None and i in dm:
            ops.maps_to_tokens_add(dm[i], self.dx, self.cur["B"], self.T)

    def _attn_branch_bwd(self, i, scr):
        pre = f"blocks.{i}."
        ba = self.cur["branch"][2 * i]
        self._before_overwrite("dY2")
        ops.branch_bwd(self.dx, None, self.P(pre + "gamma_1") if (pre + "gamma_1") in self.segs else None, self.dY2, None, scr,
                       self.cur["M"], self.D, rowmask=ba.rowmask, keep_prob=ba.keep_prob, rows_per_sample=self.T,
                       out_map=ba.cmap, dropout=self._drop(2 * i))

    def _mlp_bwd_tail(self, i, a, pre, has_g, keep, tail, scr):
        D, Hd = self.D, self.hidden
        rows, Mm, rk = tail["rows"], tail["Mm"], tail["rowkeep"]
        Mp = _pad(Mm, 256)
        assert self._drop(0) is None, "the tail-row form of the last block is pretraining-only: no element-wise dropout"
        dx, dY = self.dx, self.dY
        self._before_overwrite("dY")
        ops.branch_bwd(self.dxc, None, self.P(pre + "gamma_2") if has_g else None, dY, None, self.G(pre + "mlp.fc2.bias"),
                       Mm, D, rowmask=rk, keep_prob=keep, rows_per_sample=1)
        if Mp > Mm:
            ops.zero_(dY[Mm:Mp])
        self._before_overwrite("dbig")
        ops.gemm_nt(dY, self.wT[i]["fc2"], Mp, Hd, D, self.epi_dgelu, out0=self.dbig, aux=a["hpre"],
                    colsum=self.cs_ws, colsum_copies=self.CS_COPIES)
        ops.colsum_fold(self.cs_ws, self.CS_COPIES, Hd, self.G(pre + "mlp.fc1.bias"))
        self._on_side(lambda: self._wg_mlp(pre, a, has_g, Mm, dY))
        ops.gemm_nt(self.dbig, self.wT[i]["fc1"], Mp, D, Hd, ops.EPI_BIAS_BF16, out0=self.dh_small)
        ops.layernorm_bwd(self.dh_small, self.x[2 * i + 1], self.P(pre + "norm2.weight"), a["mean2"], a["rstd2"], dx,
                          self.G(pre + "norm2.weight"), self.G(pre + "norm2.bias"), Mm, D, accumulate=True, row_idx=rows)
        self._attn_branch_bwd(i, scr)

    def _backward_trunk(self):
        c = self.cur
        B, M, br = c["B"], c["M"], c["branch"]
        D, Hd, T = self.D, self.hidden, self.T
        dx, dY, dY2 = self.dx, self.dY, self.dY2
        self._bucket_ready(0)
        ops.zero_(self.bias_scr)
        fuse = D <= 1024 and self.fuse_ln_branch
        self._inject_dmap(self.depth - 1)
        for i in reversed(range(self.depth)):
            pre = f"blocks.{i}."
            a = self.act[i]
            ba, bm = br[2 * i], br[2 * i + 1]
            xin, xmid = self.x[2 * i], self.x[2 * i + 1]
            has_g = (pre + "gamma_1") in self.segs
            table, dtable = self.table(i), self.dtable(i)
            scr = self.bias_scr[i & 1]
            tail = c["tail"] if i == self.depth - 1 else None
            if tail is not None:
                self._mlp_bwd_tail(i, a, pre, has_g, bm.keep_prob, tail, scr)
            else:
                if i == self.depth - 1 or not fuse:
                    self._before_overwrite("dY")
                    ops.branch_bwd(dx, None, self.P(pre + "gamma_2") if has_g else None, dY, None, self.G(pre + "mlp.fc2.bias"),
                                   M, D, rowmask=bm.rowmask, keep_prob=bm.keep_prob, rows_per_sample=T, out_map=bm.cmap,
                                   dropout=self._drop(2 * i + 1))
                if bm.n == 0 and not self.accumulate_grads:
                    self._zero_grad_of(pre + "mlp.fc1.weight")
                    self._zero_grad_of(pre + "mlp.fc2.weight")
                if bm.n > 0:
                    self._before_overwrite("dbig")
                    if bm.gemm_rows > bm.rows:
                        ops.zero_(dY[bm.rows:bm.gemm_rows])
                    ops.gemm_nt(dY, self.wT[i]["fc2"], bm.gemm_rows, Hd, D, self.epi_dgelu, out0=self.dbig, aux=a["hpre"],
                                colsum=self.cs_ws, colsum_copies=self.CS_COPIES)
                    ops.colsum_fold(self.cs_ws, self.CS_COPIES, Hd, self.G(pre + "mlp.fc1.bias"))
                    self._on_side(lambda: self._wg_mlp(pre, a, has_g, bm.rows, dY))
                    ops.gemm_nt(self.dbig, self.wT[i]["fc1"], bm.gemm_rows, D, Hd, ops.EPI_BIAS_BF16, out0=self.dh_small)
                if fuse:
                    self._before_overwrite("dY2")
                    ops.layernorm_bwd_branch(self.dh_small, xmid, self.P(pre + "norm2.weight"), a["mean2"], a["rstd2"], dx,
                                             self.G(pre + "norm2.weight"), self.G(pre + "norm2.bias"), M, D, None,
                                             self.P(pre + "gamma_1") if has_g else None, dY2, None, scr,
                                             rowmask=ba.rowmask, keep_prob=ba.keep_prob, rows_per_sample=T,
                                             in_map=bm.cmap, out_map=ba.cmap, dropout=self._drop(2 * i))
                else:
                    if bm.n > 0:
                        ops.layernorm_bwd(self.dh_small, xmid, self.P(pre + "norm2.weight"), a["mean2"], a["rstd2"], dx,
                                          self.G(pre + "norm2.weight"), self.G(pre + "norm2.bias"), bm.rows, D, accumulate=True,
                                          row_idx=bm.ridx)
                    self._attn_branch_bwd(i, scr)
            if ba.n == 0 and not self.accumulate_grads:
                self._zero_grad_of(pre + "attn.proj.weight")
                self._zero_grad_of(pre + "attn.qkv.weight")
            if ba.n > 0:
                ops.gemm_nt(dY2, self.wT[i]["proj"], ba.gemm_rows, D, D, ops.EPI_BIAS_BF16, out0=self.dao)
            ops.gemv_acc(self.wT[i]["proj"], D, D, scr, self.G(pre + "attn.v_bias"),
                         x_acc=self.G(pre + "attn.proj.bias"), zero=self.bias_scr[(i & 1) ^ 1])
            if ba.n > 0:
                def wg_proj(grouped=False):
                    if not grouped:
                        self._wgrad(dY2, a["ao"], ba.rows, D, D, pre + "attn.proj.weight")
                    self._side_read_done("dY2")
                    if has_g:
                        ops.layerscale_grad(self.W16(pre + "attn.proj.weight", D, D), self.G(pre + "attn.proj.weight").view(D, D),
                                            self.P(pre + "attn.proj.bias"), self.G(pre + "attn.proj.bias"),
                                            self.P(pre + "gamma_1"), D, D, self.G(pre + "gamma_1"))
                if not self.wgrad_group:
                    self._on_side(wg_proj)
                self._before_overwrite("dqkv")
                ops.attn_bwd(a["qkv"], self.dao, a["lse"], self.delta_ws, table, self.window, ba.n, T, D, self.heads,
                             self.scale, self.dqkv, dtable, dq_bias=self.G(pre + "attn.q_bias"), out=a["ao"],
                             ws=self._attn_ws(ba.n))

                def wg_qkv():
                    if self.wgrad_group:
                        self._wgrad_group([(dY2, a["ao"], ba.rows, D, D, pre + "attn.proj.weight"),
                                           (self.dqkv, a["h1"], ba.rows, 3 * D, D, pre + "attn.qkv.weight")])
                        wg_proj(grouped=True)
                    else:
                        self._wgrad(self.dqkv, a["h1"], ba.rows, 3 * D, D, pre + "attn.qkv.weight")
                    self._side_read_done("dqkv")
                self._on_side(wg_qkv)
                ops.gemm_nt(self.dqkv, self.wT[i]["qkv"], ba.gemm_rows, D, 3 * D, ops.EPI_BIAS_BF16, out0=self.dh_small)
            if i > 0:
                self._inject_dmap(i - 1)
            if fuse and i > 0:
                pb, bb = f"blocks.{i - 1}.", br[2 * i - 1]
                self._before_overwrite("dY")
                ops.layernorm_bwd_branch(self.dh_small, xin, self.P(pre + "norm1.weight"), a["mean1"], a["rstd1"], dx,
                                         self.G(pre + "norm1.weight"), self.G(pre + "norm1.bias"), M, D, None,
                                         self.P(pb + "gamma_2") if (pb + "gamma_2") in self.segs else None, dY, None,
                                         self.G(pb + "mlp.fc2.bias"), rowmask=bb.rowmask, keep_prob=bb.keep_prob,
                                         rows_per_sample=T, in_map=ba.cmap, out_map=bb.cmap, dropout=self._drop(2 * i - 1))
            elif ba.n > 0:
                ops.layernorm_bwd(self.dh_small, xin, self.P(pre + "norm1.weight"), a["mean1"], a["rstd1"], dx,
                                  self.G(pre + "norm1.weight"), self.G(pre + "norm1.bias"), ba.rows, D, accumulate=True,
                                  row_idx=ba.ridx)
            self._bucket_ready(self.depth - i)
        self._backward_embed(c, B, M)

    def _backward_embed(self, c, B, M):
        D, T, L = self.D, self.T, self.L
        dx = self.dx
        dpos = self._drop(2 * self.depth)
        if dpos is not None:
            ops.dropout_rows(dpos, dx, M, D)
        if self.has_pos:
            if self.accumulate_grads:
                self.G("pos_embed").view(T, D).add_(dx[:M].view(B, T, D).sum(0))
            else:
                self.G("pos_embed").view(T, D).copy_(dx[:M].view(B, T, D).sum(0))
        ops.embed_bwd(dx, c["mask"], B, L, D, self.dYpe, self.G("cls_token"),
                      self.G("mask_token") if "mask_token" in self.segs else self.zero_vec)
        self._on_side(lambda: self._wgrad(self.dYpe, self.patches, B * L, D, self.Kpe, "patch_embed.proj.weight",
                                          bias_grads=((self.G("patch_embed.proj.bias"), 0, D),)))
        self._side_join()
        if self.grad_hook:
            self.grad_hook(self.depth + 1)

    def grad_norm(self, end=None):
        n = self.nflat if end is None else end
        ops.grad_norm(self.flat_g[:n], n, self.gnorm, self.gn_ws)
        return self.gnorm

    def weights_updated(self, end=None):
        if end is None or end >= self.nflat:
            self.weights_dirty = True
        elif not self.weights_dirty:
            assert end <= self.head_end, "partial weight update: the head bucket only (no transposed copies to refresh)"
            ops.cast_f32_bf16(self.flat_p[:end], self.flat_w16[:end], end)
            self.w16_version += 1

    def adamw_step(self, m, v, lr, wd, step, betas=(0.9, 0.95), eps=1e-8, max_norm=0.0):
        if not (self.overlap_optimizer and self.head_kind == "mlm" and not self.fwd_two_streams):
            self.wait_optimizer()
            ops.adamw(self.flat_p, self.flat_g, m, v, self.nflat, self.wd_flags, lr, betas[0], betas[1], eps, wd, step,
                      gnorm=self.gnorm, max_norm=max_norm or 0.0)
            self.weights_dirty = True
            return
        self.wait_optimizer()
        if self._tdesc is None:
            self._build_transpose_descs()
        if self._opt_stream is None:
            self._opt_stream = torch.cuda.Stream(device=self.dev)
            self._opt_events = {b[0]: torch.cuda.Event() for b in self.buckets}
            self._opt_events["__done__"] = torch.cuda.Event()
            self._opt_start = torch.cuda.Event()
        main, st = torch.cuda.current_stream(), self._opt_stream
        self._opt_start.record(main)
        with torch.cuda.stream(st):
            st.wait_event(self._opt_start)
            for name, b0, b1 in reversed(self.buckets):
                if b1 == b0:
                    self._opt_events[name].record(st)
                    continue
                ops.adamw(self.flat_p[b0:b1], self.flat_g[b0:b1], m[b0:b1], v[b0:b1], b1 - b0,
                          self.wd_flags[b0 // ALIGN: b1 // ALIGN], lr, betas[0], betas[1], eps, wd, step,
                          gnorm=self.gnorm, max_norm=max_norm or 0.0)
                ops.cast_f32_bf16(self.flat_p[b0:b1], self.flat_w16[b0:b1], b1 - b0)
                self._opt_events[name].record(st)
            for name, (k0, n, p0, tiles) in self._tbucket.items():
                ops.transpose_cast_batched(self._tdesc[k0:k0 + n], self._tprefix_loc[p0:p0 + n + 1], n, tiles)
            self._opt_events["__done__"].record(st)
        self._opt_ev = self._opt_events
        self._opt_done = self._opt_events["__done__"]
        self.weights_dirty = False
        self.w16_version += 1

    def _wait_params(self, bucket):
        if self._opt_ev is not None:
            torch.cuda.current_stream().wait_event(self._opt_ev[bucket])

    def wait_optimizer(self):
        if self._opt_done is not None:
            torch.cuda.current_stream().wait_event(self._opt_done)
            self._opt_ev = None
            self._opt_done = None
```

Baseline: 7730 samples/sec.

## Fold dropped-sample copies into LN forward and colsum fold into LN backward

```diff
diff --git a/include/memhip.h b/include/memhip.h
--- a/include/memhip.h
+++ b/include/memhip.h
@@ -248,6 +248,15 @@
                          const int32_t* row_idx, int R, int D, const float* gamma, const float* mean,
                          const float* rstd, float* dres, int64_t lddres, int accumulate, float* dgamma,
                          float* dbeta, memhip_stream_t stream);
+int memhip_layernorm_fwd_copy(const float* x, int64_t ldx, const int32_t* row_idx, int R, int D,
+                              const float* gamma, const float* beta, float eps, void* y_bf16, int64_t ldy,
+                              float* mean, float* rstd, const int32_t* dropped, int n_dropped, int rows_per_sample,
+                              float* x_out, int64_t ldxo, memhip_stream_t stream);
+int memhip_layernorm_bwd_fold(const void* dy_bf16, int64_t lddy, const float* x, int64_t ldx,
+                              const int32_t* row_idx, int R, int D, const float* gamma, const float* mean,
+                              const float* rstd, float* dres, int64_t lddres, int accumulate, float* dgamma,
+                              float* dbeta, float* fold_ws, int fold_copies, int fold_n, float* fold_dst,
+                              memhip_stream_t stream);
 
 int memhip_layerscale_grad(const void* W_bf16, int64_t ldw, const float* dW, int64_t lddw, const float* bias,
                            const float* dbias, const float* gamma, int N, int K, float* dgamma,
@@ -281,6 +290,8 @@
   memhip_branch_t branch;
 } memhip_ln_bwd_branch_args_t;
 int memhip_layernorm_bwd_branch(const memhip_ln_bwd_branch_args_t* args, memhip_stream_t stream);
+int memhip_layernorm_bwd_branch_fold(const memhip_ln_bwd_branch_args_t* args, float* fold_ws, int fold_copies, int fold_n,
+                                     float* fold_dst, memhip_stream_t stream);
 
 int memhip_embed_bwd(const float* dx, int64_t lddx, const uint8_t* mask, int B, int L, int D,
                      void* dy_bf16, int64_t lddy, float* dcls, float* dmask_token, memhip_stream_t stream);
diff --git a/mem_amd/csrc/rowops.hip b/mem_amd/csrc/rowops.hip
--- a/mem_amd/csrc/rowops.hip
+++ b/mem_amd/csrc/rowops.hip
@@ -70,13 +70,21 @@
 __device__ __forceinline__ float ln_dx(float gg, float xh, float m1, float m2) { return __fmaf_rn(-xh, m2, sub_rn(gg, m1)); }
 __device__ __forceinline__ float sq2(float a, float b) { return __fmaf_rn(a, a, mul_rn(b, b)); }
 
-template <int NCH, bool FULL>
-__global__ __launch_bounds__(256) void ln_fwd_kernel(const float* __restrict__ x, long long ldx,
-                                                     const int* __restrict__ row_idx, int R, int D,
-                                                     const float* __restrict__ gamma,
-                                                     const float* __restrict__ beta, float eps,
-                                                     __bf16* __restrict__ y, long long ldy,
-                                                     float* __restrict__ mean, float* __restrict__ rstd) {
+struct NoFold {};
+struct DroppedCopy {
+  const int* ids;
+  int n, rps;
+  float* out;
+  long long ldo;
+};
+
+template <int NCH, bool FULL, class Copy>
+__device__ __forceinline__ void ln_fwd_body(const float* __restrict__ x, long long ldx,
+                                            const int* __restrict__ row_idx, int R, int D,
+                                            const float* __restrict__ gamma,
+                                            const float* __restrict__ beta, float eps,
+                                            __bf16* __restrict__ y, long long ldy,
+                                            float* __restrict__ mean, float* __restrict__ rstd, Copy cp) {
   extern __shared__ float red[];
   const int lane = threadIdx.x & 63;
   const int r0 = blockIdx.x * 4 + wave_id();
@@ -123,36 +131,93 @@
   const float var = wsum(q) / (float)D;
   const float rs = 1.0f / sqrtf(var + eps);
   __syncthreads();
-  if (!act) return;
-  if (lane == 0) { mean[r] = mu; rstd[r] = rs; }
-  bf16x4* yr = reinterpret_cast<bf16x4*>(y + (long long)r * ldy);
-#pragma unroll
-  for (int c = 0; c < NCH; ++c) {
-    const int i = lane + c * 64;
-    if (chunk_ok<FULL>(i, nch)) {
-      const float4 g = lgb[i], b = lgb[nch + i];
-      bf16x4 o;
-      o[0] = (__bf16)__fmaf_rn(mul_rn(v[c].x - mu, rs), g.x, b.x);
-      o[1] = (__bf16)__fmaf_rn(mul_rn(v[c].y - mu, rs), g.y, b.y);
-      o[2] = (__bf16)__fmaf_rn(mul_rn(v[c].z - mu, rs), g.z, b.z);
-      o[3] = (__bf16)__fmaf_rn(mul_rn(v[c].w - mu, rs), g.w, b.w);
-      yr[i] = o;
-    }
-  }
-}
-
-__device__ __forceinline__ void vm_drain() { __builtin_amdgcn_s_waitcnt(0x0F70); }
-
-template <int NCH, bool FULL, bool ACC>
-__global__ __launch_bounds__(256) void ln_bwd_kernel(const __bf16* __restrict__ dy, long long lddy,
-                                                     const float* __restrict__ x, long long ldx,
+  const auto store = [&]() {
+    if (lane == 0) { mean[r] = mu; rstd[r] = rs; }
+    bf16x4* yr = reinterpret_cast<bf16x4*>(y + (long long)r * ldy);
+#pragma unroll
+    for (int c = 0; c < NCH; ++c) {
+      const int i = lane + c * 64;
+      if (chunk_ok<FULL>(i, nch)) {
+        const float4 g = lgb[i], b = lgb[nch + i];
+        bf16x4 o;
+        o[0] = (__bf16)__fmaf_rn(mul_rn(v[c].x - mu, rs), g.x, b.x);
+        o[1] = (__bf16)__fmaf_rn(mul_rn(v[c].y - mu, rs), g.y, b.y);
+        o[2] = (__bf16)__fmaf_rn(mul_rn(v[c].z - mu, rs), g.z, b.z);
+        o[3] = (__bf16)__fmaf_rn(mul_rn(v[c].w - mu, rs), g.w, b.w);
+        yr[i] = o;
+      }
+    }
+  };
+  if constexpr (std::is_same_v<Copy, NoFold>) {
+    if (!act) return;
+    store();
+  } else {
+    if (act) store();
+    const int total = cp.n * cp.rps;
+    RowWalk w(r0, gridDim.x * 4, cp.rps);
+    for (; w.r < total; w.next()) {
+      const long long row = (long long)cp.ids[w.smp] * cp.rps + w.off;
+      const float4* sr = reinterpret_cast<const float4*>(x + row * ldx);
+      float4* dr = reinterpret_cast<float4*>(cp.out + row * cp.ldo);
+      float4 t[NCH];
+#pragma unroll
+      for (int c = 0; c < NCH; ++c)
+        if (chunk_ok<FULL>(lane + c * 64, nch)) t[c] = sr[lane + c * 64];
+#pragma unroll
+      for (int c = 0; c < NCH; ++c)
+        if (chunk_ok<FULL>(lane + c * 64, nch)) dr[lane + c * 64] = t[c];
+    }
+  }
+}
+
+template <int NCH, bool FULL>
+__global__ __launch_bounds__(256) void ln_fwd_kernel(const float* __restrict__ x, long long ldx,
                                                      const int* __restrict__ row_idx, int R, int D,
                                                      const float* __restrict__ gamma,
-                                                     const float* __restrict__ mean,
-                                                     const float* __restrict__ rstd,
-                                                     float* __restrict__ dres, long long lddres,
-                                                     float* __restrict__ dgamma, float* __restrict__ dbeta) {
+                                                     const float* __restrict__ beta, float eps,
+                                                     __bf16* __restrict__ y, long long ldy,
+                                                     float* __restrict__ mean, float* __restrict__ rstd) {
+  ln_fwd_body<NCH, FULL>(x, ldx, row_idx, R, D, gamma, beta, eps, y, ldy, mean, rstd, NoFold{});
+}
+
+template <int NCH, bool FULL>
+__global__ __launch_bounds__(256) void ln_fwd_copy_kernel(const float* __restrict__ x, long long ldx,
+                                                          const int* __restrict__ row_idx, int R, int D,
+                                                          const float* __restrict__ gamma,
+                                                          const float* __restrict__ beta, float eps,
+                                                          __bf16* __restrict__ y, long long ldy,
+                                                          float* __restrict__ mean, float* __restrict__ rstd,
+                                                          DroppedCopy cp) {
+  ln_fwd_body<NCH, FULL>(x, ldx, row_idx, R, D, gamma, beta, eps, y, ldy, mean, rstd, cp);
+}
+
+__device__ __forceinline__ void vm_drain() { __builtin_amdgcn_s_waitcnt(0x0F70); }
+
+struct ColFold { float* ws; int copies, n; float* dst; };
+
+__device__ __forceinline__ void fold_columns(const ColFold& f) {
+  if (!f.ws) return;
+  for (int c = blockIdx.x * 256 + threadIdx.x; c < f.n; c += gridDim.x * 256) {
+    float s = 0.f;
+    for (int k = 0; k < f.copies; ++k) {
+      s += f.ws[(long long)k * f.n + c];
+      f.ws[(long long)k * f.n + c] = 0.f;
+    }
+    f.dst[c] += s;
+  }
+}
+
+template <int NCH, bool FULL, bool ACC, class Fold>
+__device__ __forceinline__ void ln_bwd_body(const __bf16* __restrict__ dy, long long lddy,
+                                            const float* __restrict__ x, long long ldx,
+                                            const int* __restrict__ row_idx, int R, int D,
+                                            const float* __restrict__ gamma,
+                                            const float* __restrict__ mean,
+                                            const float* __restrict__ rstd,
+                                            float* __restrict__ dres, long long lddres,
+                                            float* __restrict__ dgamma, float* __restrict__ dbeta, Fold fold) {
   extern __shared__ float red[];
+  if constexpr (!std::is_same_v<Fold, NoFold>) fold_columns(fold);
   const int lane = threadIdx.x & 63, wave = wave_id();
   const int nch = D >> 2;
   float4 ag[NCH], ab[NCH];
@@ -274,6 +339,31 @@
     atomicAdd(dgamma + n, a);
     atomicAdd(dbeta + n, b);
   }
+}
+
+template <int NCH, bool FULL, bool ACC>
+__global__ __launch_bounds__(256) void ln_bwd_kernel(const __bf16* __restrict__ dy, long long lddy,
+                                                     const float* __restrict__ x, long long ldx,
+                                                     const int* __restrict__ row_idx, int R, int D,
+                                                     const float* __restrict__ gamma,
+                                                     const float* __restrict__ mean,
+                                                     const float* __restrict__ rstd,
+                                                     float* __restrict__ dres, long long lddres,
+                                                     float* __restrict__ dgamma, float* __restrict__ dbeta) {
+  ln_bwd_body<NCH, FULL, ACC>(dy, lddy, x, ldx, row_idx, R, D, gamma, mean, rstd, dres, lddres, dgamma, dbeta, NoFold{});
+}
+
+template <int NCH, bool FULL, bool ACC>
+__global__ __launch_bounds__(256) void ln_bwd_fold_kernel(const __bf16* __restrict__ dy, long long lddy,
+                                                          const float* __restrict__ x, long long ldx,
+                                                          const int* __restrict__ row_idx, int R, int D,
+                                                          const float* __restrict__ gamma,
+                                                          const float* __restrict__ mean,
+                                                          const float* __restrict__ rstd,
+                                                          float* __restrict__ dres, long long lddres,
+                                                          float* __restrict__ dgamma, float* __restrict__ dbeta,
+                                                          ColFold fold) {
+  ln_bwd_body<NCH, FULL, ACC>(dy, lddy, x, ldx, row_idx, R, D, gamma, mean, rstd, dres, lddres, dgamma, dbeta, fold);
 }
 
 constexpr int kBrMaxChunks = 8;
@@ -403,20 +493,21 @@
   }
 }
 
-template <int NCH, bool FULL, bool HAS_Y, class... Drop>
-__global__ __launch_bounds__(256) void ln_bwd_branch_kernel(const __bf16* __restrict__ dy, long long lddy,
-                                                            const float* __restrict__ x, long long ldx, int R, int D,
-                                                            const float* __restrict__ gamma,
-                                                            const float* __restrict__ mean, const float* __restrict__ rstd,
-                                                            float* __restrict__ dres, long long lddres,
-                                                            float* __restrict__ dgamma, float* __restrict__ dbeta,
-                                                            const __bf16* __restrict__ yb, long long ldyb,
-                                                            const float* __restrict__ gb, const float* __restrict__ rowmask,
-                                                            float keep, int rps, __bf16* __restrict__ dyo, long long lddyo,
-                                                            float* __restrict__ dgb, float* __restrict__ dbiasb,
-                                                            const int* __restrict__ in_map, const int* __restrict__ out_map,
-                                                            Drop... drop) {
+template <int NCH, bool FULL, bool HAS_Y, class Fold, class... Drop>
+__device__ __forceinline__ void ln_bwd_branch_body(const __bf16* __restrict__ dy, long long lddy,
+                                                   const float* __restrict__ x, long long ldx, int R, int D,
+                                                   const float* __restrict__ gamma,
+                                                   const float* __restrict__ mean, const float* __restrict__ rstd,
+                                                   float* __restrict__ dres, long long lddres,
+                                                   float* __restrict__ dgamma, float* __restrict__ dbeta,
+                                                   const __bf16* __restrict__ yb, long long ldyb,
+                                                   const float* __restrict__ gb, const float* __restrict__ rowmask,
+                                                   float keep, int rps, __bf16* __restrict__ dyo, long long lddyo,
+                                                   float* __restrict__ dgb, float* __restrict__ dbiasb,
+                                                   const int* __restrict__ in_map, const int* __restrict__ out_map,
+                                                   Fold fold, Drop... drop) {
   extern __shared__ float red[];
+  if constexpr (!std::is_same_v<Fold, NoFold>) fold_columns(fold);
   const int lane = threadIdx.x & 63, wave = wave_id();
   const int nch = D >> 2;
   float4 ag[NCH], ab[NCH], bg[HAS_Y ? NCH : 1], bb[NCH];
@@ -614,6 +705,39 @@
   }
 }
 
+template <int NCH, bool FULL, bool HAS_Y, class... Drop>
+__global__ __launch_bounds__(256) void ln_bwd_branch_kernel(const __bf16* __restrict__ dy, long long lddy,
+                                                            const float* __restrict__ x, long long ldx, int R, int D,
+                                                            const float* __restrict__ gamma,
+                                                            const float* __restrict__ mean, const float* __restrict__ rstd,
+                                                            float* __restrict__ dres, long long lddres,
+                                                            float* __restrict__ dgamma, float* __restrict__ dbeta,
+                                                            const __bf16* __restrict__ yb, long long ldyb,
+                                                            const float* __restrict__ gb, const float* __restrict__ rowmask,
+                                                            float keep, int rps, __bf16* __restrict__ dyo, long long lddyo,
+                                                            float* __restrict__ dgb, float* __restrict__ dbiasb,
+                                                            const int* __restrict__ in_map, const int* __restrict__ out_map,
+                                                            Drop... drop) {
+  ln_bwd_branch_body<NCH, FULL, HAS_Y>(dy, lddy, x, ldx, R, D, gamma, mean, rstd, dres, lddres, dgamma, dbeta, yb, ldyb, gb,
+                                       rowmask, keep, rps, dyo, lddyo, dgb, dbiasb, in_map, out_map, NoFold{}, drop...);
+}
+
+template <int NCH, bool FULL, class... Drop>
+__global__ __launch_bounds__(256) void ln_bwd_branch_fold_kernel(const __bf16* __restrict__ dy, long long lddy,
+                                                                 const float* __restrict__ x, long long ldx, int R, int D,
+                                                                 const float* __restrict__ gamma,
+                                                                 const float* __restrict__ mean, const float* __restrict__ rstd,
+                                                                 float* __restrict__ dres, long long lddres,
+                                                                 float* __restrict__ dgamma, float* __restrict__ dbeta,
+                                                                 const float* __restrict__ gb, const float* __restrict__ rowmask,
+                                                                 float keep, int rps, __bf16* __restrict__ dyo, long long lddyo,
+                                                                 float* __restrict__ dbiasb,
+                                                                 const int* __restrict__ in_map, const int* __restrict__ out_map,
+                                                                 ColFold fold, Drop... drop) {
+  ln_bwd_branch_body<NCH, FULL, false>(dy, lddy, x, ldx, R, D, gamma, mean, rstd, dres, lddres, dgamma, dbeta, nullptr, 0, gb,
+                                       rowmask, keep, rps, dyo, lddyo, nullptr, dbiasb, in_map, out_map, fold, drop...);
+}
+
 
 __global__ __launch_bounds__(256) void layerscale_grad_kernel(const __bf16* __restrict__ W, long long ldw,
                                                               const float* __restrict__ dW, long long lddw,
@@ -833,6 +957,24 @@
                        x, (long long)ldx, row_idx, R, D, gamma, beta, eps, (__bf16*)y, (long long)ldy, mean, rstd);
   });
   return check_launch("layernorm_fwd");
+}
+
+extern "C" int memhip_layernorm_fwd_copy(const float* x, int64_t ldx, const int32_t* row_idx, int R, int D,
+                                         const float* gamma, const float* beta, float eps, void* y,
+                                         int64_t ldy, float* mean, float* rstd, const int32_t* dropped, int n_dropped,
+                                         int rows_per_sample, float* x_out, int64_t ldxo, memhip_stream_t stream) {
+  if (n_dropped == 0) return memhip_layernorm_fwd(x, ldx, row_idx, R, D, gamma, beta, eps, y, ldy, mean, rstd, stream);
+  MEMHIP_REQUIRE(R > 0 && D > 0 && D % 4 == 0 && D <= 64 * 4 * kMaxChunks, "layernorm_fwd_copy: bad R=%d D=%d (the copy rides on a LayerNorm launch)", R, D);
+  MEMHIP_REQUIRE(n_dropped > 0 && rows_per_sample > 0 && (long long)n_dropped * rows_per_sample <= INT32_MAX,
+                 "layernorm_fwd_copy: bad n_dropped=%d rows_per_sample=%d", n_dropped, rows_per_sample);
+  MEMHIP_REQUIRE(x && gamma && beta && y && mean && rstd && dropped && x_out, "layernorm_fwd_copy: null pointer");
+  MEMHIP_REQUIRE(ldx % 4 == 0 && ldy % 4 == 0 && ldxo % 4 == 0, "layernorm_fwd_copy: ld must be a multiple of 4");
+  const DroppedCopy cp{(const int*)dropped, n_dropped, rows_per_sample, x_out, (long long)ldxo};
+  dispatch_width<kMaxChunks>(D, [&](auto N, auto F) {
+    hipLaunchKernelGGL((ln_fwd_copy_kernel<decltype(N)::value, decltype(F)::value>), dim3(cdiv(R, 4)), dim3(256), (size_t)2 * D * sizeof(float), as_stream(stream),
+                       x, (long long)ldx, row_idx, R, D, gamma, beta, eps, (__bf16*)y, (long long)ldy, mean, rstd, cp);
+  });
+  return check_launch("layernorm_fwd_copy");
 }
 
 extern "C" int memhip_layernorm_bwd(const void* dy, int64_t lddy, const float* x, int64_t ldx,
@@ -855,6 +997,32 @@
     });
   });
   return check_launch("layernorm_bwd");
+}
+
+extern "C" int memhip_layernorm_bwd_fold(const void* dy, int64_t lddy, const float* x, int64_t ldx,
+                                         const int32_t* row_idx, int R, int D, const float* gamma,
+                                         const float* mean, const float* rstd, float* dres, int64_t lddres,
+                                         int accumulate, float* dgamma, float* dbeta, float* fold_ws, int fold_copies,
+                                         int fold_n, float* fold_dst, memhip_stream_t stream) {
+  if (!fold_ws)
+    return memhip_layernorm_bwd(dy, lddy, x, ldx, row_idx, R, D, gamma, mean, rstd, dres, lddres, accumulate, dgamma, dbeta, stream);
+  MEMHIP_REQUIRE(R > 0 && D > 0 && D % 4 == 0 && D <= 64 * 4 * kMaxChunks, "layernorm_bwd_fold: bad R=%d D=%d (the fold rides on a LayerNorm launch)", R, D);
+  MEMHIP_REQUIRE(fold_copies >= 1 && fold_n > 0 && fold_dst, "layernorm_bwd_fold: bad fold copies=%d n=%d", fold_copies, fold_n);
+  MEMHIP_REQUIRE(dy && x && gamma && mean && rstd && dres && dgamma && dbeta, "layernorm_bwd_fold: null pointer");
+  MEMHIP_REQUIRE(ldx % 4 == 0 && lddy % 4 == 0 && lddres % 4 == 0, "layernorm_bwd_fold: ld must be a multiple of 4");
+  int grid = cdiv(R, 4);
+  const int cap = opt(OPT_LN_BWD_GRID) * 4 / 3;
+  if (grid > cap) grid = cap;
+  const ColFold fold{fold_ws, fold_copies, fold_n, fold_dst};
+  dispatch_width<kMaxChunks>(D, [&](auto N, auto F) {
+    dispatch_bool(accumulate, [&](auto A) {
+      hipLaunchKernelGGL((ln_bwd_fold_kernel<decltype(N)::value, decltype(F)::value, decltype(A)::value>), dim3(grid), dim3(256), (size_t)8 * D * sizeof(float), as_stream(stream),
+                         (const __bf16*)dy, (long long)lddy, x, (long long)ldx, row_idx, R, D, gamma, mean, rstd, dres,
+                         (long long)lddres, dgamma, dbeta, fold);
+      return 0;
+    });
+  });
+  return check_launch("layernorm_bwd_fold");
 }
 
 template <int NCH, bool FULL, bool HAS_Y, class... Drop>
@@ -933,7 +1101,32 @@
                      b.dgamma, b.dbias, (const int*)a.in_map, (const int*)b.out_map, drop...);
 }
 
+template <int NCH, bool FULL, class... Drop>
+static void ln_bwd_branch_fold_launch(const memhip_ln_bwd_branch_args_t& a, ColFold fold, int grid, memhip_stream_t stream,
+                                      Drop... drop) {
+  const memhip_branch_t& b = a.branch;
+  hipLaunchKernelGGL((ln_bwd_branch_fold_kernel<NCH, FULL, Drop...>), dim3(grid), dim3(256), (size_t)16 * a.D * sizeof(float),
+                     as_stream(stream), (const __bf16*)a.dy, (long long)a.lddy, a.x, (long long)a.ldx, a.R, a.D, a.gamma, a.mean,
+                     a.rstd, a.dres, (long long)a.lddres, a.dgamma, a.dbeta, b.gamma, b.rowmask, b.keep_prob,
+                     b.rows_per_sample > 0 ? b.rows_per_sample : 1, (__bf16*)b.dy, (long long)b.lddy, b.dbias,
+                     (const int*)a.in_map, (const int*)b.out_map, fold, drop...);
+}
+
+static int ln_bwd_branch_impl(const memhip_ln_bwd_branch_args_t* args, const ColFold* fold, memhip_stream_t stream);
+
 extern "C" int memhip_layernorm_bwd_branch(const memhip_ln_bwd_branch_args_t* args, memhip_stream_t stream) {
+  return ln_bwd_branch_impl(args, nullptr, stream);
+}
+
+extern "C" int memhip_layernorm_bwd_branch_fold(const memhip_ln_bwd_branch_args_t* args, float* fold_ws, int fold_copies,
+                                                int fold_n, float* fold_dst, memhip_stream_t stream) {
+  if (!fold_ws) return ln_bwd_branch_impl(args, nullptr, stream);
+  MEMHIP_REQUIRE(fold_copies >= 1 && fold_n > 0 && fold_dst, "layernorm_bwd_branch_fold: bad fold copies=%d n=%d", fold_copies, fold_n);
+  const ColFold fold{fold_ws, fold_copies, fold_n, fold_dst};
+  return ln_bwd_branch_impl(args, &fold, stream);
+}
+
+static int ln_bwd_branch_impl(const memhip_ln_bwd_branch_args_t* args, const ColFold* fold, memhip_stream_t stream) {
   MEMHIP_REQUIRE(args, "layernorm_bwd_branch: null args");
   const memhip_ln_bwd_branch_args_t& a = *args;
   const memhip_branch_t& b = a.branch;
@@ -942,6 +1135,7 @@
   MEMHIP_REQUIRE(!b.dropout || D % 8 == 0, "layernorm_bwd_branch_drop: D=%d must be a multiple of 8", D);
   MEMHIP_REQUIRE(!(a.in_map || b.out_map) || (!b.rowmask && !b.y && b.rows_per_sample > 0),
                  "layernorm_bwd_branch: sample maps exclude rowmask / y_branch");
+  MEMHIP_REQUIRE(!fold || (R > 0 && !b.y), "layernorm_bwd_branch_fold: the fold rides on a launch without y_branch (R=%d)", R);
   if (R == 0) return MEMHIP_OK;
   MEMHIP_REQUIRE(a.dy && a.x && a.gamma && a.mean && a.rstd && a.dres && a.dgamma && a.dbeta && b.dy,
                  "layernorm_bwd_branch: null pointer");
@@ -952,6 +1146,13 @@
   int cap = opt(OPT_LN_BWD_GRID);
   if (D > 768 && cap > 512) cap = 512;
   if (grid > cap) grid = cap;
+  if (fold) {
+    dispatch_width<4>(D, [&](auto N, auto F) {
+      if (b.dropout) ln_bwd_branch_fold_launch<decltype(N)::value, decltype(F)::value>(a, *fold, grid, stream, drop_params(*b.dropout));
+      else ln_bwd_branch_fold_launch<decltype(N)::value, decltype(F)::value>(a, *fold, grid, stream);
+    });
+    return check_launch("layernorm_bwd_branch_fold");
+  }
   dispatch_width<4>(D, [&](auto N, auto F) {
     if (b.dropout)
       dispatch_bool(b.y, [&](auto Y) {
diff --git a/mem_amd/ops.py b/mem_amd/ops.py
--- a/mem_amd/ops.py
+++ b/mem_amd/ops.py
@@ -140,6 +140,9 @@
 declare({
     "memhip_layernorm_fwd": (i32, [vp, i64, vp, i32, i32, vp, vp, f32, vp, i64, vp, vp, vp]),
     "memhip_layernorm_bwd": (i32, [vp, i64, vp, i64, vp, i32, i32, vp, vp, vp, vp, i64, i32, vp, vp, vp]),
+    "memhip_layernorm_fwd_copy": (i32, [vp, i64, vp, i32, i32, vp, vp, f32, vp, i64, vp, vp, vp, i32, i32, vp, i64, vp]),
+    "memhip_layernorm_bwd_fold": (i32, [vp, i64, vp, i64, vp, i32, i32, vp, vp, vp, vp, i64, i32, vp, vp, vp, i32, i32, vp, vp]),
+    "memhip_layernorm_bwd_branch_fold": (i32, [C.POINTER(LnBwdBranchArgs), vp, i32, i32, vp, vp]),
     "memhip_layerscale_grad": (i32, [vp, i64, vp, i64, vp, vp, vp, i32, i32, vp, vp]),
     "memhip_embed_bwd": (i32, [vp, i64, vp, i32, i32, i32, vp, i64, vp, vp, vp]),
     "memhip_cross_entropy": (i32, [vp, i64, vp, i32, i32, f32, vp, vp, i32, vp, vp]),
@@ -181,15 +184,27 @@
     check(lib.memhip_dropout_rows_f32(C.byref(d), ptr(x), x.stride(0), rows, D, stream_ptr()), "dropout_rows_f32")
 
 
-def layernorm_fwd(x, gamma, beta, y, mean, rstd, R, D, eps=1e-6, row_idx=None):
-    check(lib.memhip_layernorm_fwd(ptr(x), x.stride(0), ptr(row_idx), R, D, ptr(gamma), ptr(beta), eps,
-                                   ptr(y), y.stride(0), ptr(mean), ptr(rstd), stream_ptr()), "layernorm_fwd")
-
-
-def layernorm_bwd(dy, x, gamma, mean, rstd, dres, dgamma, dbeta, R, D, accumulate=True, row_idx=None):
-    check(lib.memhip_layernorm_bwd(ptr(dy), dy.stride(0), ptr(x), x.stride(0), ptr(row_idx), R, D, ptr(gamma),
-                                   ptr(mean), ptr(rstd), ptr(dres), dres.stride(0), int(accumulate),
-                                   ptr(dgamma), ptr(dbeta), stream_ptr()), "layernorm_bwd")
+def layernorm_fwd(x, gamma, beta, y, mean, rstd, R, D, eps=1e-6, row_idx=None, dropped=None):
+    if dropped is None:
+        check(lib.memhip_layernorm_fwd(ptr(x), x.stride(0), ptr(row_idx), R, D, ptr(gamma), ptr(beta), eps,
+                                       ptr(y), y.stride(0), ptr(mean), ptr(rstd), stream_ptr()), "layernorm_fwd")
+        return
+    ids, n, rps, x_out = dropped
+    check(lib.memhip_layernorm_fwd_copy(ptr(x), x.stride(0), ptr(row_idx), R, D, ptr(gamma), ptr(beta), eps, ptr(y), y.stride(0),
+                                        ptr(mean), ptr(rstd), ptr(ids), n, rps, ptr(x_out), x_out.stride(0), stream_ptr()),
+          "layernorm_fwd_copy")
+
+
+def layernorm_bwd(dy, x, gamma, mean, rstd, dres, dgamma, dbeta, R, D, accumulate=True, row_idx=None, fold=None):
+    if fold is None:
+        check(lib.memhip_layernorm_bwd(ptr(dy), dy.stride(0), ptr(x), x.stride(0), ptr(row_idx), R, D, ptr(gamma),
+                                       ptr(mean), ptr(rstd), ptr(dres), dres.stride(0), int(accumulate),
+                                       ptr(dgamma), ptr(dbeta), stream_ptr()), "layernorm_bwd")
+        return
+    ws, copies, n, dst = fold
+    check(lib.memhip_layernorm_bwd_fold(ptr(dy), dy.stride(0), ptr(x), x.stride(0), ptr(row_idx), R, D, ptr(gamma),
+                                        ptr(mean), ptr(rstd), ptr(dres), dres.stride(0), int(accumulate),
+                                        ptr(dgamma), ptr(dbeta), ptr(ws), copies, n, ptr(dst), stream_ptr()), "layernorm_bwd_fold")
 
 
 def _branch(y, gamma, rowmask, keep_prob, rows_per_sample, dy, dgamma, dbias, out_map, dropout):
@@ -198,11 +213,15 @@
 
 
 def layernorm_bwd_branch(dy, x, gamma, mean, rstd, dres, dgamma, dbeta, R, D, y_b, gamma_b, dy_b, dgamma_b, dbias_b,
-                         rowmask=None, keep_prob=1.0, rows_per_sample=1, in_map=None, out_map=None, dropout=None):
+                         rowmask=None, keep_prob=1.0, rows_per_sample=1, in_map=None, out_map=None, dropout=None, fold=None):
     a = LnBwdBranchArgs(_p(dy), dy.stride(0), _p(x), x.stride(0), R, D, _p(gamma), _p(mean), _p(rstd), _p(dres), dres.stride(0),
                         _p(dgamma), _p(dbeta), _p(in_map),
                         _branch(y_b, gamma_b, rowmask, keep_prob, rows_per_sample, dy_b, dgamma_b, dbias_b, out_map, dropout))
-    check(lib.memhip_layernorm_bwd_branch(C.byref(a), stream_ptr()), "layernorm_bwd_branch")
+    if fold is None:
+        check(lib.memhip_layernorm_bwd_branch(C.byref(a), stream_ptr()), "layernorm_bwd_branch")
+        return
+    ws, copies, n, dst = fold
+    check(lib.memhip_layernorm_bwd_branch_fold(C.byref(a), ptr(ws), copies, n, ptr(dst), stream_ptr()), "layernorm_bwd_branch_fold")
 
 
 def layerscale_grad(W16, dW, bias, dbias, gamma, N, K, dgamma):
diff --git a/mem_amd/vit_engine.py b/mem_amd/vit_engine.py
--- a/mem_amd/vit_engine.py
+++ b/mem_amd/vit_engine.py
@@ -186,6 +186,7 @@
         self._tdesc = None
         self.set_gelu_dg(True)
         self.fuse_ln_branch = True
+        self.block_folds = True
         self.gn_ws = torch.zeros(1024, dtype=torch.float64, device=dev)
         self.gnorm = torch.zeros(1, dtype=torch.float32, device=dev)
         self.loss_acc = torch.zeros(2, dtype=torch.float32, device=dev)
@@ -296,7 +297,7 @@
         self.delta_ws = e(2 * M + 4, self.heads, dt=f32)
         self._tn_ws = torch.empty(0, dtype=torch.uint8, device=dev)
         self.bias_scr = torch.zeros(2, D, dtype=f32, device=dev)
-        self.cs_ws = torch.zeros(self.CS_COPIES, self.hidden, dtype=f32, device=dev)
+        self.cs_ws = torch.zeros(2, self.CS_COPIES, self.hidden, dtype=f32, device=dev)
         self.dYpe = e(B * self.L, D)
         self.B_stash = B
 
@@ -415,6 +416,16 @@
         if nd > 0:
             ops.copy_samples(src, dst, plan["drop"][j], nd, self.T * self.D)
 
+    FOLD_COPY, FOLD_COLSUM = 2, 4
+
+    def _rides(self, what):
+        f = self.block_folds
+        return bool(f) if isinstance(f, bool) else bool(int(f) & what)
+
+    def _dropped(self, plan, j, dst, B):
+        nd = B - plan["n"][j]
+        return (plan["drop"][j], nd, self.T, dst) if nd > 0 else None
+
     def forward(self, x, mask_u8, rows_idx, labels=None, dp_masks=None, all_tokens=False, labels_event=None):
         assert x.is_cuda and x.dtype == torch.float32 and x.is_contiguous()
         B = x.shape[0]
@@ -471,13 +482,15 @@
         g1 = self.P(pre + "gamma_1") if (pre + "gamma_1") in self.segs else None
         g2 = self.P(pre + "gamma_2") if (pre + "gamma_2") in self.segs else None
         tail = self.cur["tail"] if (i == self.depth - 1 and b0 == 0 and b1 == B) else None
-        if ba.smap is not None:
+        ride = self._rides(self.FOLD_COPY)
+        if ba.smap is not None and not (ride and ba.n > 0):
             self._copy_dropped(plan, 2 * i, xin, xmid, B)
         if ba.n > 0:
             rs = slice(r0, r1) if ba.smap is None else slice(None)
             h1, qkv, ao = a["h1"][rs], a["qkv"][rs], a["ao"][rs]
             ops.layernorm_fwd(xin, self.P(pre + "norm1.weight"), self.P(pre + "norm1.bias"), h1, a["mean1"][r0:r1],
-                              a["rstd1"][r0:r1], ba.rows, D, row_idx=ba.ridx)
+                              a["rstd1"][r0:r1], ba.rows, D, row_idx=ba.ridx,
+                              dropped=self._dropped(plan, 2 * i, xmid, B) if (ride and ba.smap is not None) else None)
             ops.gemm_nt(h1, self.W16(pre + "attn.qkv.weight", 3 * D, D), ba.gemm_rows, 3 * D, D, ops.EPI_BIAS_BF16,
                         out0=qkv, bias=self.P(pre + "attn.qkvbias3"), colscale=self.scale, colscale_n=D)
             ops.attn_fwd(qkv, ba.n, T, D, self.heads, self.table(i), self.window, ao, a["lse"][b0:b1])
@@ -489,13 +502,14 @@
         if tail is not None:
             self._mlp_fwd_tail(i, a, xs[2 * i + 1], g2, bm.keep_prob, tail)
             return
-        if bm.smap is not None:
+        if bm.smap is not None and not (ride and bm.n > 0):
             self._copy_dropped(plan, 2 * i + 1, xmid, xout, B)
         if bm.n > 0:
             rs = slice(r0, r1) if bm.smap is None else slice(None)
             h2, hpre, aa = a["h2"][rs], a["hpre"][rs], a["a"][rs]
             ops.layernorm_fwd(xmid, self.P(pre + "norm2.weight"), self.P(pre + "norm2.bias"), h2, a["mean2"][r0:r1],
-                              a["rstd2"][r0:r1], bm.rows, D, row_idx=bm.ridx)
+                              a["rstd2"][r0:r1], bm.rows, D, row_idx=bm.ridx,
+                              dropped=self._dropped(plan, 2 * i + 1, xout, B) if (ride and bm.smap is not None) else None)
             ops.gemm_nt(h2, self.W16(pre + "mlp.fc1.weight", Hd, D), bm.gemm_rows, Hd, D, self.epi_gelu, out0=hpre,
                         out1=aa, bias=self.P(pre + "mlp.fc1.bias"))
             dm = self._drop(2 * i + 1, r0)
@@ -791,6 +805,8 @@
         Mp = _pad(Mm, 256)
         assert self._drop(0) is None, "the tail-row form of the last block is pretraining-only: no element-wise dropout"
         dx, dY = self.dx, self.dY
+        ride_cs, cs = self._rides(self.FOLD_COLSUM), self.cs_ws[i & 1]
+        fold = (cs, self.CS_COPIES, Hd, self.G(pre + "mlp.fc1.bias"))
         self._before_overwrite("dY")
         ops.branch_bwd(self.dxc, None, self.P(pre + "gamma_2") if has_g else None, dY, None, self.G(pre + "mlp.fc2.bias"),
                        Mm, D, rowmask=rk, keep_prob=keep, rows_per_sample=1)
@@ -798,12 +814,14 @@
             ops.zero_(dY[Mm:Mp])
         self._before_overwrite("dbig")
         ops.gemm_nt(dY, self.wT[i]["fc2"], Mp, Hd, D, self.epi_dgelu, out0=self.dbig, aux=a["hpre"],
-                    colsum=self.cs_ws, colsum_copies=self.CS_COPIES)
-        ops.colsum_fold(self.cs_ws, self.CS_COPIES, Hd, self.G(pre + "mlp.fc1.bias"))
+                    colsum=cs, colsum_copies=self.CS_COPIES)
+        if not ride_cs:
+            ops.colsum_fold(*fold)
         self._on_side(lambda: self._wg_mlp(pre, a, has_g, Mm, dY))
         ops.gemm_nt(self.dbig, self.wT[i]["fc1"], Mp, D, Hd, ops.EPI_BIAS_BF16, out0=self.dh_small)
         ops.layernorm_bwd(self.dh_small, self.x[2 * i + 1], self.P(pre + "norm2.weight"), a["mean2"], a["rstd2"], dx,
-                          self.G(pre + "norm2.weight"), self.G(pre + "norm2.bias"), Mm, D, accumulate=True, row_idx=rows)
+                          self.G(pre + "norm2.weight"), self.G(pre + "norm2.bias"), Mm, D, accumulate=True, row_idx=rows,
+                          fold=fold if ride_cs else None)
         self._attn_branch_bwd(i, scr)
 
     def _backward_trunk(self):
@@ -814,6 +832,7 @@
         self._bucket_ready(0)
         ops.zero_(self.bias_scr)
         fuse = D <= 1024 and self.fuse_ln_branch
+        ride_cs = self._rides(self.FOLD_COLSUM)
         self._inject_dmap(self.depth - 1)
         for i in reversed(range(self.depth)):
             pre = f"blocks.{i}."
@@ -835,13 +854,18 @@
                 if bm.n == 0 and not self.accumulate_grads:
                     self._zero_grad_of(pre + "mlp.fc1.weight")
                     self._zero_grad_of(pre + "mlp.fc2.weight")
+                fold = None
                 if bm.n > 0:
                     self._before_overwrite("dbig")
                     if bm.gemm_rows > bm.rows:
                         ops.zero_(dY[bm.rows:bm.gemm_rows])
+                    cs = self.cs_ws[i & 1]
                     ops.gemm_nt(dY, self.wT[i]["fc2"], bm.gemm_rows, Hd, D, self.epi_dgelu, out0=self.dbig, aux=a["hpre"],
-                                colsum=self.cs_ws, colsum_copies=self.CS_COPIES)
-                    ops.colsum_fold(self.cs_ws, self.CS_COPIES, Hd, self.G(pre + "mlp.fc1.bias"))
+                                colsum=cs, colsum_copies=self.CS_COPIES)
+                    fold = (cs, self.CS_COPIES, Hd, self.G(pre + "mlp.fc1.bias"))
+                    if not ride_cs:
+                        ops.colsum_fold(*fold)
+                        fold = None
                     self._on_side(lambda: self._wg_mlp(pre, a, has_g, bm.rows, dY))
                     ops.gemm_nt(self.dbig, self.wT[i]["fc1"], bm.gemm_rows, D, Hd, ops.EPI_BIAS_BF16, out0=self.dh_small)
                 if fuse:
@@ -850,12 +874,12 @@
                                              self.G(pre + "norm2.weight"), self.G(pre + "norm2.bias"), M, D, None,
                                              self.P(pre + "gamma_1") if has_g else None, dY2, None, scr,
                                              rowmask=ba.rowmask, keep_prob=ba.keep_prob, rows_per_sample=T,
-                                             in_map=bm.cmap, out_map=ba.cmap, dropout=self._drop(2 * i))
+                                             in_map=bm.cmap, out_map=ba.cmap, dropout=self._drop(2 * i), fold=fold)
                 else:
                     if bm.n > 0:
                         ops.layernorm_bwd(self.dh_small, xmid, self.P(pre + "norm2.weight"), a["mean2"], a["rstd2"], dx,
                                           self.G(pre + "norm2.weight"), self.G(pre + "norm2.bias"), bm.rows, D, accumulate=True,
-                                          row_idx=bm.ridx)
+                                          row_idx=bm.ridx, fold=fold)
                     self._attn_branch_bwd(i, scr)
             if ba.n == 0 and not self.accumulate_grads:
                 self._zero_grad_of(pre + "attn.proj.weight")
```

After: 7764 samples/sec (median of 4 runs). No clear change (+0.4%).
